# zixunh/vipe

Hardware: AMD Instinct MI355X
Metric: dense-BA+flow update iters/s, 512x384 48-KF graph (higher is better)
Workload: dtype f16 (correlation, GRU; fp32 accumulate) + f32 geometry/BA (fp64 reduced system)

## Files before the change

include/vipe_amd.h:

```cpp
#ifndef VIPE_AMD_H
#define VIPE_AMD_H

#include <stdint.h>

#ifdef __cplusplus
extern "C" {
#endif

#define VIPE_F16 0
#define VIPE_F32 1
#define VIPE_F64 2
#define VIPE_U8 3

#define VIPE_OK 0
#define VIPE_EINVAL (-1)
#define VIPE_ENOSPACE (-2)
#define VIPE_EUNSUPPORTED (-3)

#define VIPE_PYRAMID_REFERENCE 0
#define VIPE_PYRAMID_BLOCKED 1

#define VIPE_CAM_PINHOLE 0
#define VIPE_CAM_MEI 1
#define VIPE_CAM_PANORAMA 2

const char* vipe_amd_version(void);
int vipe_amd_abi_version(void);


int vipe_corr_index_forward(const void* d_volume, const float* d_coords, void* d_corr, int B, int h1, int w1,
                            int h2, int w2, int radius, int dtype, void* stream);

int vipe_corr_index_backward(const float* d_coords, const void* d_corr_grad, void* d_volume_grad, int B, int h1,
                             int w1, int h2, int w2, int radius, int dtype, void* stream);

int vipe_corr_pyramid_lookup(const void* const* h_levels, const float* d_coords, void* d_out, int B, int h1, int w1,
                             int h2, int w2, int num_levels, int radius, int dtype, void* stream);

int vipe_corr_pyramid_lookup_nhwc(const void* const* h_levels, const float* d_coords, void* d_out, int B, int h1,
                                  int w1, int h2, int w2, int num_levels, int radius, int dtype, int channel_stride,
                                  void* stream);

int vipe_corr_lookup_conv1x1(const void* const* h_levels, const float* d_coords, const void* d_w_packed,
                             const float* d_bias, void* d_out, int out_ctot, int out_coff, int B, int h1, int w1,
                             int h2, int w2, int Cout, int act, const int* d_slots, int layout, void* stream);

int vipe_corr_lookup_conv1x1_ex(const void* const* h_levels, const float* d_coords, const void* d_w_packed,
                                const float* d_bias, void* d_out, int out_ctot, int out_coff, int B, int h1, int w1,
                                int h2, int w2, int Cout, int act, const int* d_slots, int layout, void* stream,
                                int max_workgroups, int share_cu);

int vipe_corr_pyramid_build(const void* d_fmap1, const void* d_fmap2, void* const* h_levels, int B, int C, int h,
                            int w, int num_levels, void* stream);

int vipe_corr_pyramid_build_indexed(const void* d_fmaps, const int64_t* d_idx1, const int64_t* d_idx2,
                                    const int* d_slots, void* const* h_levels, int B, int C, int h, int w,
                                    int num_levels, int layout, void* stream);

int vipe_corr_blocked_dims(int h, int w, int* dims6);
int64_t vipe_corr_prep_halves(int C, int h, int w);
int vipe_corr_prep(const void* d_fmaps, void* d_prep, int n, int C, int h, int w, void* stream);
int vipe_corr_pyramid_build_prepared(const void* d_prep, int64_t frame_base, int64_t n_prepared, const int64_t* d_idx1, const int64_t* d_idx2,
                                     const int* d_slots, void* const* h_levels, int B, int C, int h, int w, int num_levels,
                                     void* stream);

int vipe_corr_volume(const void* d_fmap1, const void* d_fmap2, void* d_volume, int B, int C, int P, int dtype, void* stream);
int vipe_avg_pool2x2(const void* d_x, void* d_y, int64_t n, int h, int w, int dtype, void* stream);

int vipe_altcorr_forward(const void* d_fmap1, const void* d_fmap2, const float* d_coords, void* d_corr, int B,
                         int H1, int W1, int H2, int W2, int N, int C, int radius, int dtype, void* stream);

int vipe_altcorr_backward(const float* d_fmap1, const float* d_fmap2, const float* d_coords,
                          const float* d_corr_grad, float* d_fmap1_grad, float* d_fmap2_grad, int B, int H1, int W1,
                          int H2, int W2, int N, int C, int radius, void* stream);

int vipe_lie_expm(int group_id, const void* a, void* X, int64_t n, int dtype, int on_device, void* stream);
int vipe_lie_logm(int group_id, const void* X, void* a, int64_t n, int dtype, int on_device, void* stream);
int vipe_lie_inv(int group_id, const void* X, void* Y, int64_t n, int dtype, int on_device, void* stream);
int vipe_lie_mul(int group_id, const void* X, const void* Y, void* Z, int64_t n, int dtype, int on_device,
                 void* stream);
int vipe_lie_adj(int group_id, const void* X, const void* a, void* b, int64_t n, int dtype, int on_device,
                 void* stream);
int vipe_lie_adjT(int group_id, const void* X, const void* a, void* b, int64_t n, int dtype, int on_device,
                  void* stream);
int vipe_lie_act(int group_id, const void* X, const void* p, void* q, int64_t n, int dtype, int on_device,
                 void* stream);
int vipe_lie_act4(int group_id, const void* X, const void* p, void* q, int64_t n, int dtype, int on_device,
                  void* stream);
int vipe_lie_as_matrix(int group_id, const void* X, void* T, int64_t n, int dtype, int on_device,
                       void* stream);
int vipe_lie_projector(int group_id, const void* X, void* P, int64_t n, int dtype, int on_device,
                       void* stream);
int vipe_lie_jinv(int group_id, const void* X, const void* a, void* b, int64_t n, int dtype, int on_device,
                  void* stream);
int vipe_frontend_next_frame(float* d_poses, float* d_disps, int t1, int n_views, int P, int n_mean, int init_pose,
                             void* stream);
int vipe_lie_adjT_bcast(int group_id, const void* X, const void* a, void* b, int64_t n_elem, int64_t rows_per_elem,
                        int dtype, void* stream);
int vipe_lie_act4_bcast(int group_id, const void* X, const void* p, void* q, int64_t n_elem, int64_t rows_per_elem,
                        int dtype, void* stream);
int vipe_lie_expm_backward(int group_id, const void* grad, const void* a, void* da, int64_t n, int dtype,
                           int on_device, void* stream);
int vipe_lie_logm_backward(int group_id, const void* grad, const void* X, void* dX, int64_t n, int dtype,
                           int on_device, void* stream);
int vipe_lie_inv_backward(int group_id, const void* grad, const void* X, void* dX, int64_t n, int dtype,
                          int on_device, void* stream);
int vipe_lie_mul_backward(int group_id, const void* grad, const void* X, const void* Y, void* dX, void* dY,
                          int64_t n, int dtype, int on_device, void* stream);
int vipe_lie_adj_backward(int group_id, const void* grad, const void* X, const void* a, void* dX, void* da,
                          int64_t n, int dtype, int on_device, void* stream);
int vipe_lie_adjT_backward(int group_id, const void* grad, const void* X, const void* a, void* dX, void* da,
                           int64_t n, int dtype, int on_device, void* stream);
int vipe_lie_act_backward(int group_id, const void* grad, const void* X, const void* p, void* dX, void* dp,
                          int64_t n, int dtype, int on_device, void* stream);
int vipe_lie_act4_backward(int group_id, const void* grad, const void* X, const void* p, void* dX, void* dp,
                           int64_t n, int dtype, int on_device, void* stream);


int vipe_reproject(const float* d_poses, const float* d_disps, const float* d_intrinsics, const float* d_rig,
                   const int64_t* d_pi, const int64_t* d_qi, const int64_t* d_pj, const int64_t* d_qj,
                   const int64_t* d_di, float* d_coords, float* d_valid, int M, int ht, int wd, int n_views,
                   int camera, float intr_factor, void* stream);

int vipe_reproject_motion(const float* d_poses, const float* d_disps, const float* d_intrinsics, const float* d_rig,
                          const int64_t* d_pi, const int64_t* d_qi, const int64_t* d_pj, const int64_t* d_qj,
                          const int64_t* d_di, const float* d_target, float* d_coords, void* d_motn, int M, int ht,
                          int wd, int n_views, int camera, float intr_factor, int motn_dtype, void* stream);
int vipe_reproject_motion_nhwc(const float* d_poses, const float* d_disps, const float* d_intrinsics,
                               const float* d_rig, const int64_t* d_pi, const int64_t* d_qi, const int64_t* d_pj,
                               const int64_t* d_qj, const int64_t* d_di, const float* d_target, float* d_coords,
                               void* d_motn, int M, int ht, int wd, int n_views, int camera, float intr_factor,
                               void* stream);

typedef int (*vipe_overlap_fn)(void* user, int piece, int n_pieces, void* stream);

typedef struct {
  int n_poses;
  int n_views;
  int ht, wd;
  int M;
  int t0, t1;
  int n_iters;
  float pose_damping, pose_ep;
  int motion_only;
  int limited_disp;
  int optimize_intrinsics;
  int optimize_rig_rotation;
  int camera;
  float alpha;
  float weight_scale;
  float intr_factor;
  int reuse_plan;
  int path_hint;
  void* overlap_stream;
  vipe_overlap_fn overlap_fn;
  void* overlap_user;
  int solver_options;
  void* profile_ev0;
  void* profile_ev1;
  int profile_iter;
} vipe_ba_params;
#define VIPE_BA_OPT_ONE_CHAIN 1
#define VIPE_BA_OPT_GENERAL_ACCUMULATE 2

int64_t vipe_dense_ba_workspace_bytes(const vipe_ba_params* p);
int vipe_dense_ba(const vipe_ba_params* p, float* d_poses, float* d_disps, const float* d_disps_sens,
                  float* d_intrinsics, float* d_rig, const float* d_target, const float* d_weight,
                  const float* d_disp_damping, const int64_t* d_pi, const int64_t* d_qi, const int64_t* d_pj,
                  const int64_t* d_qj, const int64_t* d_di, void* d_workspace, int64_t workspace_bytes,
                  int* d_info, void* stream);

int vipe_dense_ba_linearize(const vipe_ba_params* p, const float* d_poses, const float* d_disps, const float* d_disps_sens,
                            const float* d_intrinsics, const float* d_rig, const float* d_target, const float* d_weight,
                            const float* d_disp_damping, const int64_t* d_pi, const int64_t* d_qi, const int64_t* d_pj,
                            const int64_t* d_qj, const int64_t* d_di, void* d_workspace, int64_t workspace_bytes,
                            double* d_S_out, int ld_out, int* d_info, void* stream);
int vipe_dense_ba_marginals(const vipe_ba_params* p, void* d_workspace, const double* d_Sinv, int ld, float* d_disp_var,
                            double* d_pose_cov, void* stream);

int64_t vipe_ba_workspace_bytes(int n_poses, int ht, int wd, int E);
int vipe_ba(float* d_poses, float* d_disps, const float* d_intrinsics, const float* d_disps_sens,
            const float* d_targets, const float* d_weights, const float* d_eta, const int64_t* d_ii,
            const int64_t* d_jj, int n_poses, int ht, int wd, int E, int n_eta, int t0, int t1, int iterations,
            float lm, float ep, int motion_only, float* d_dx, float* d_dz, void* d_workspace,
            int64_t workspace_bytes, void* stream);

int vipe_frame_distance(const float* d_poses, const float* d_disps, const float* d_intrinsics, const int64_t* d_pi,
                        const int64_t* d_pj, const int64_t* d_qi, const int64_t* d_qj, const int64_t* d_di,
                        float* d_dist, int M, int ht, int wd, float beta, void* stream);

int vipe_frame_distance_rig(const float* d_poses, const float* d_rig, const float* d_disps, const float* d_intrinsics,
                            int intr_dim, float intr_factor, const int64_t* d_pi, const int64_t* d_qi, const int64_t* d_pj,
                            const int64_t* d_qj, float* d_dist, int M, int n_views, int ht, int wd, float beta,
                            int bidirectional, void* stream);

int vipe_depth_filter(const float* d_poses, const float* d_disps, const float* d_intrinsics, const int64_t* d_inds,
                      const float* d_thresh, float* d_counter, int n, int num, int ht, int wd, void* stream);

int vipe_frame_distance_sphere(const float* d_poses, const float* d_rig, const float* d_disps, const int64_t* d_pi,
                               const int64_t* d_qi, const int64_t* d_pj, const int64_t* d_qj, float* d_dist, int M,
                               int n_views, int ht, int wd, float beta, int bidirectional, void* stream);
int vipe_depth_filter_sphere(const float* d_poses, const float* d_disps, const int64_t* d_inds, const float* d_thresh,
                             float* d_counter, int n, int num, int ht, int wd, void* stream);
int vipe_iproj_sphere(const float* d_poses, const float* d_disps, float* d_points, int n, int ht, int wd, void* stream);

int vipe_projmap(const float* d_poses, const float* d_disps, const float* d_intrinsics, const int64_t* d_ii,
                 const int64_t* d_jj, float* d_coords, float* d_valid, int E, int ht, int wd, void* stream);

int vipe_iproj(const float* d_poses, const float* d_disps, const float* d_intrinsics, float* d_points, int n, int ht,
               int wd, void* stream);

int vipe_scatter(const void* d_src, const int64_t* d_index, void* d_out, int64_t* d_arg_out, int64_t outer,
                 int64_t src_dim, int64_t inner, int64_t out_dim, int reduce, int dtype, void* stream);
int vipe_scatter_rows(const void* d_src, const int64_t* d_index, void* d_out, int64_t* d_arg_out, int64_t outer,
                      int64_t src_dim, int64_t inner, int64_t out_dim, int reduce, int dtype, void* stream);

int vipe_scatter_host(const void* h_src, const int64_t* h_index, void* h_out, int64_t* h_arg_out, int64_t outer,
                      int64_t src_dim, int64_t inner, int64_t out_dim, int reduce, int dtype);

int vipe_scatter_mean_rows_f16(const void* d_src, const int64_t* d_ix, void* d_out, int E, int n_out, int64_t inner,
                               void* stream);

int vipe_segment_mean_nhwc_f16(const void* d_src, int src_ctot, int src_coff, const int* d_order, const int* d_rowptr,
                               void* d_out, int n_out, int64_t rows_per_item, int C, void* stream);

int vipe_corr_sampler_forward(const void* d_in1, const void* d_in2, void* d_out, int B, int C, int H, int W, int kH,
                              int kW, int patchH, int patchW, int padH, int padW, int dilH, int dilW,
                              int dil_patchH, int dil_patchW, int dH, int dW, int dtype, void* stream);
int vipe_corr_sampler_backward(const void* d_in1, const void* d_in2, const void* d_grad_out, void* d_grad1,
                               void* d_grad2, int B, int C, int H, int W, int kH, int kW, int patchH, int patchW,
                               int padH, int padW, int dilH, int dilW, int dil_patchH, int dil_patchW, int dH,
                               int dW, int dtype, void* stream);

int vipe_corr_sampler_forward_host(const float* h_in1, const float* h_in2, float* h_out, int B, int C, int H, int W, int kH,
                                   int kW, int patchH, int patchW, int padH, int padW, int dilH, int dilW, int dil_patchH,
                                   int dil_patchW, int dH, int dW);
int vipe_corr_sampler_backward_host(const float* h_in1, const float* h_in2, const float* h_grad_out, float* h_grad1,
                                    float* h_grad2, int B, int C, int H, int W, int kH, int kW, int patchH, int patchW,
                                    int padH, int padW, int dilH, int dilW, int dil_patchH, int dil_patchW, int dH, int dW);

int vipe_nearest_neighbours(const float* d_query, int qdim, const float* d_tree, int tdim, int64_t M, int64_t N, int knn,
                            float* d_dist, int* d_idx, void* stream);

int vipe_ms_deform_attn_forward(const void* d_value, const int64_t* d_spatial_shapes, const int64_t* d_level_start_index,
                                const void* d_sampling_loc, const void* d_attn_weight, void* d_output, int64_t bs,
                                int64_t Lv, int heads, int C, int L, int64_t Lq, int P, int dtype, void* stream);
int vipe_ms_deform_attn_backward(const void* d_value, const int64_t* d_spatial_shapes, const int64_t* d_level_start_index,
                                 const void* d_sampling_loc, const void* d_attn_weight, const void* d_grad_output,
                                 void* d_grad_value, void* d_grad_sampling_loc, void* d_grad_attn_weight, int64_t bs,
                                 int64_t Lv, int heads, int C, int L, int64_t Lq, int P, int dtype, void* stream);

#define VIPE_ACT_NONE 0
#define VIPE_ACT_RELU 1
#define VIPE_ACT_SIGMOID 2
#define VIPE_ACT_TANH 3
int vipe_conv_pack_weights(const void* d_w_oihw, void* d_w_packed, int Cout, int Cin, int KH, int KW, int src_dtype,
                           void* stream);
int vipe_conv2d_nhwc_f16(const void* d_x, const void* d_w_packed, const float* d_bias, const float* d_extra,
                         void* d_y, int B, int H, int W, int Cin, int cin_total, int cin_off, int Cout,
                         int cout_total, int cout_off, int KH, int KW, int act, void* stream);

int vipe_conv_packed_dims(int Cout, int Cin, int KH, int KW, int* cout_pad, int* cin_pad, int* k_pad);

#define VIPE_CONV_PARTIAL 6
#define VIPE_CONV_HEADS_FUSED 7
#define VIPE_CONV_ACCINIT_F32 0x100
int vipe_conv2d_fused(const void* d_x0, int x0_ctot, int x0_coff, const void* d_x1, int x1_ctot, int x1_coff,
                      int split, const void* d_w_packed, const float* d_bias, const float* d_extra, int extra_stride,
                      int extra_off, void* d_y, int y_ctot, int y_coff, void* d_y2, int y2_ctot, int y2_coff,
                      const void* d_net, int net_ctot, int net_coff, const void* d_z, float* d_fout,
                      const void* d_accinit, int ai_ctot, int ai_coff, int B, int H, int W, int Cin, int Cout, int KH,
                      int KW, int act, int mode, void* stream);

int vipe_heads_fused_ok(int H, int W);
int vipe_heads_border_floats(int E, int H, int W, int64_t* n_floats);
int vipe_heads_finish(float* d_dw, const float* d_border, const float* d_bias, int E, int H, int W, void* stream);

typedef struct {
  const void *corr0_w, *corr2_w, *flow0_w, *flow2_w, *gw_w, *zr_w, *q_w, *zr_s_w, *q_s_w, *heads0_w, *heads2_w, *agg2_w, *eta_w;
  const void *zr_n_w, *zr_x_w;
  const float *corr0_b, *corr2_b, *flow0_b, *flow2_b, *gw_b, *zr_b, *q_b, *heads0_b, *heads2_b, *agg2_b, *eta_b;
  const float* glo_wT;
  const float* glo_b;
  const void *agg1_w, *heads_dw_w;
  const float *agg1_b, *heads_dw_b;
  const void* heads2_frag;
} vipe_update_weights;
typedef struct {
  int E, H, W, n_src;
  const void* levels[4];
  const float* coords;
  const int* slots;
  int h2, w2, pyramid_layout;
  const void* corr;
  const void* motn;
  const void* net;
  void* net_out;
  void* xbuf;
  const void* pgate;
  void *c1, *f1, *zb, *rnet;
  void* hbuf;
  float* dw;
  float *glo, *extra;
  const int *order, *rowptr;
  void *agg, *a2;
  float* eta;
  void* side_stream;
  float* pzr;
  int gate_state;
  float* hborder;
} vipe_update_buffers;
int vipe_update_operator(const vipe_update_weights* weights, const vipe_update_buffers* buffers, void* stream);

int vipe_update_gate_state(const vipe_update_weights* weights, const vipe_update_buffers* buffers, const void* d_net,
                           int parts, void* stream);
typedef struct {
  const vipe_update_weights* weights;
  const vipe_update_buffers* buffers;
  const void* net;
  const int* bounds;
  int n_bounds;
} vipe_gate_state_job;
int vipe_update_gate_state_piece(void* user, int piece, int n_pieces, void* stream);

int vipe_glo_context(const float* d_glo_sum, const float* d_wT, const float* d_bias, float* d_extra, int E, int hw,
                     void* stream);

typedef struct {
  const void* src;
  void* dst;
  const int64_t* idx;
  int64_t src_row_pitch, dst_row_pitch;
  int64_t seg_bytes, seg_pitch;
  int n_seg;
  int n_rows;
  int dst_row0;
} vipe_rows_job;
int vipe_rows_gather(const vipe_rows_job* jobs, int n_jobs, void* stream);
typedef struct {
  const void* src;
  const int64_t* frame;
  void* dst;
  int64_t dst_row_pitch;
  int dst_ctot, dst_coff;
  int dst_row0;
} vipe_nhwc_job;
int vipe_gather_nchw_to_nhwc_f16(const vipe_nhwc_job* jobs, int n_jobs, int n_rows, int C, int P, void* stream);

int vipe_flow_score(const float* d_dw, const unsigned char* d_invalid, float* d_score, int n_views, int P, void* stream);

int vipe_update_finish(const float* d_coords1, const float* d_dw, const unsigned char* d_mask, float* d_target,
                       float* d_weight, const float* d_eta, const int64_t* d_du, float* d_damping, int E, int n_src, int ht,
                       int wd, void* stream);

int vipe_enc_prep(const float* d_img, void* d_x4, int V, int H, int W, void* stream);
int vipe_enc_stem(const void* d_x4, const void* d_w, const float* d_bias, void* d_y, float* d_out_stats, int B, int H,
                  int W, int relu, void* stream);
int vipe_enc_conv(const void* d_x, const float* d_in_stats, const void* d_w, const float* d_bias, const void* d_res,
                  void* d_y, float* d_out_stats, int B, int H, int W, int Cin, int Cout, int ksize, int stride,
                  int relu, int nchw, int tanh_split, void* stream);
int vipe_enc_finish(const void* d_raw, const float* d_raw_stats, const void* d_res, const float* d_res_stats,
                    void* d_out, int B, int HW, int C, void* stream);

int vipe_frame_ingest(const void* d_rgb, int rgb_dtype, const unsigned char* d_mask, const float* d_depth, int H0, int W0,
                      int h1, int w1, int top, int left, int H, int W, float* d_images, void* d_x4,
                      unsigned char* d_mask8, float* d_disps_sens, void* stream);

int vipe_convex_upsample(const void* d_mask, int mask_dtype, const float* d_data, float* d_out, const int64_t* d_rows,
                         int N, int R, int h, int w, int C, void* stream);

int vipe_depth_export(const float* d_disp, const int64_t* d_rows, void* d_out, int out_dtype, int N, int R, int H, int W,
                      int h1, int w1, int top, int left, int H0, int W0, float depth_scale, void* stream);

int vipe_depth_consistency(const float* d_disp, const float* d_poses, const float* d_rig, const float* d_intrinsics,
                           int intr_dim, int camera, const int64_t* d_rows, const int64_t* d_nbr, unsigned char* d_out,
                           int N, int K, int R, int n_views, int H, int W, int h1, int w1, int top, int left, int H0,
                           int W0, float tol, void* stream);

int vipe_cloud_fuse(const float* d_disp, const float* d_poses, const float* d_rig, const float* d_intrinsics, int intr_dim,
                    int camera, const int64_t* d_rows, const unsigned char* d_conf, int min_agree, const void* d_rgb,
                    int rgb_dtype, int stride, float inv_voxel, int64_t* d_keys, int* d_acc, int64_t cap, int64_t* d_stats,
                    int N, int R, int n_views, int H, int W, int h1, int w1, int top, int left, int H0, int W0,
                    void* stream);

int vipe_cloud_extract(const int64_t* d_keys, const int* d_acc, int64_t cap, float voxel, int min_count, float* d_xyz,
                       unsigned char* d_rgb, int* d_count, int64_t* d_key, int64_t max_out, int64_t* d_num_out,
                       void* stream);

int vipe_cloud_render(const float* d_xyz, int64_t M, int index_base, const float* d_cams, const float* d_intrinsics,
                      int intr_dim, int camera, int B, int H, int W, int h1, int w1, int top, int left, int H0, int W0,
                      float point_size, int max_radius, int64_t* d_zbuf, int64_t* d_stats, void* stream);

int vipe_cloud_resolve(const int64_t* d_zbuf, int B, int H0, int W0, void* d_depth, int depth_dtype,
                       const unsigned char* d_rgb_points, int64_t M_total, unsigned char* d_rgb_out, int* d_index,
                       void* stream);

#define VIPE_COMPLETE_DISP 0
#define VIPE_COMPLETE_DEPTH 1

int vipe_depth_anchor_bits(const void* d_sparse, const void* d_pred, int dtype, int B, int H, int W, int64_t* d_bits,
                           void* stream);

int vipe_depth_complete(const void* d_sparse, const void* d_pred, int dtype, const unsigned char* d_mask,
                        const int64_t* d_bits, int B, int H, int W, int domain, int K, int radius, int wrap_x, void* d_out,
                        float* d_scale, float* d_shift, int* d_nbr, int64_t* d_stats, void* stream);

#define VIPE_KLT_OOB 1
#define VIPE_KLT_LOW_TEXTURE 2
#define VIPE_KLT_RESIDUAL 4
#define VIPE_KLT_FB 8
#define VIPE_KLT_MASKED 16
#define VIPE_KLT_DIVERGED 32

int vipe_klt_pyramid(const void* d_rgb, int rgb_dtype, int H, int W, int L, float* d_pyr, void* stream);

int vipe_klt_detect(const float* d_img, int H, int W, const unsigned char* d_mask, const unsigned char* d_cell_busy,
                    int cell, int border, float min_eig, float* d_out, void* stream);

int vipe_klt_track(const float* d_pyr_a, const float* d_pyr_b, int H, int W, int L, const float* d_pts, int N,
                   const float* d_fb_ref, const unsigned char* d_mask, int win_radius, int n_iters, float eps, int border,
                   float min_eig, float max_residual, float fb_thresh, float max_flow, int cell, float* d_out,
                   unsigned char* d_status, float* d_resid, unsigned char* d_cell_busy, void* stream);

#ifdef __cplusplus
}
#endif
#endif
```

vipe_amd/csrc/conv_call.cuh:

```cuda
#pragma once
#include <hip/hip_runtime_api.h>
#include <limits.h>

#include "../../include/vipe_amd.h"

enum Epi { EPI_PLAIN = 0, EPI_GLO = 1, EPI_ZR = 2, EPI_Q = 3, EPI_HEADS = 4, EPI_ETA = 5, EPI_PARTIAL = 6, EPI_HEADS_FUSED = 7 };

struct ConvView {
  const void* p = nullptr;
  int ctot = 0, coff = 0;
};

struct ConvCall {
  ConvView x0, x1;
  int split = INT_MAX;
  const void* w = nullptr;
  const float* bias = nullptr;
  const float* extra = nullptr;
  int extra_stride = 0, extra_off = 0;
  ConvView y;
  ConvView y2;
  ConvView net;
  ConvView accinit;
  bool accinit_f32 = false;
  const void* z = nullptr;
  float* fout = nullptr;
  const void* heads2_frag = nullptr;
  float* border = nullptr;
  int B = 0, H = 0, W = 0, Cin = 0, Cout = 0, KH = 1, KW = 1;
  int act = VIPE_ACT_NONE, epi = EPI_PLAIN;
};

int vipe_conv_run(const ConvCall& c, hipStream_t stream);
```

vipe_amd/csrc/conv_mfma.hip:

```cpp
#include <stdlib.h>

#include <type_traits>

#include "common.cuh"
#include "conv_call.cuh"

namespace {

typedef _Float16 half8 __attribute__((ext_vector_type(8)));
typedef _Float16 half4 __attribute__((ext_vector_type(4)));
typedef float float16v __attribute__((ext_vector_type(16)));
typedef float float4v __attribute__((ext_vector_type(4)));

struct ConvArgs {
  const half_t* x0; int x0_ctot, x0_coff;
  const half_t* x1; int x1_ctot, x1_coff;
  int split;
  const half_t* w;
  const float* bias;
  const float* extra;
  int extra_stride, extra_off;
  half_t* y; int y_ctot, y_coff;
  int B, H, W, Cin, Cin_pad, Cout, Cout_pad, KH, KW, nsteps;
  int act, epi;
  const half_t* net; int net_ctot, net_coff;
  const half_t* zbuf;
  half_t* y2; int y2_ctot, y2_coff;
  float* fout;
  const half_t* accinit; int ai_ctot, ai_coff;
  int ai_f32;
  const half_t* w2;
  float* border;
  int f_wp, f_hwp, f_tiles, f_pieces, f_xbytes, f_p1lo, f_p1hi;
  unsigned f_magic;
};

constexpr int BNP = 128;
constexpr int BK = 64;

__device__ __forceinline__ int swz(int row, int k8) { return row * 128 + ((k8 ^ ((row >> 1) & 7)) << 4); }

__device__ __forceinline__ float act_apply(float v, int act) {
  switch (act) {
    case VIPE_ACT_RELU: return fmaxf(v, 0.0f);
    case VIPE_ACT_SIGMOID: return 1.0f / (1.0f + __expf(-v));
    case VIPE_ACT_TANH: return tanhf(v);
    default: return v;
  }
}

template <int BMC, int WAVES_M, int WAVES_N, bool SMALLCIN>
__global__ __launch_bounds__(256) void conv_mfma_kernel(ConvArgs a) {
  constexpr int TM = BMC / (WAVES_M * 32);
  constexpr int TN = BNP / (WAVES_N * 32);
  static_assert(WAVES_M * WAVES_N == 4, "4 waves");
  constexpr int W_ITEMS = BMC * 8 / 256;
  constexpr int X_ITEMS = BNP * 8 / 256;

  extern __shared__ __align__(16) unsigned char lds[];
  unsigned char* ldsW = lds;
  unsigned char* ldsX = lds + 2 * BMC * 128;

  const int tid = threadIdx.x, lane = tid & 63, wave = tid >> 6;
  const int wm = wave / WAVES_N, wn = wave % WAVES_N;
  const int64_t M = (int64_t)a.B * a.H * a.W;
  const int64_t pix0 = (int64_t)blockIdx.x * BNP;
  const int cout0 = blockIdx.y * BMC;
  const int HW = a.H * a.W;

  const int k8 = tid & 7;
  int xe[X_ITEMS], xy[X_ITEMS], xx[X_ITEMS];
  bool xvalid[X_ITEMS];
#pragma unroll
  for (int j = 0; j < X_ITEMS; ++j) {
    const int64_t m = pix0 + (tid >> 3) + 32 * j;
    xvalid[j] = m < M;
    const int64_t mm = xvalid[j] ? m : 0;
    xe[j] = (int)(mm / HW);
    const int rem = (int)(mm % HW);
    xy[j] = rem / a.W;
    xx[j] = rem % a.W;
  }
  const int ph = a.KH / 2, pw = a.KW / 2;
  const int csteps = a.Cin_pad / BK;

  half8 wreg[W_ITEMS], xreg[X_ITEMS];

  auto issue_loads = [&](int s) {
    const half_t* wb = a.w + ((int64_t)s * a.Cout_pad + cout0) * BK;
#pragma unroll
    for (int j = 0; j < W_ITEMS; ++j) {
      const int row = (tid >> 3) + 32 * j;
      wreg[j] = *reinterpret_cast<const half8*>(wb + row * BK + k8 * 8);
    }
    if constexpr (!SMALLCIN) {
      const int tap = s / csteps, c0 = (s % csteps) * BK;
      const int dy = tap / a.KW - ph, dx = tap % a.KW - pw;
      const int c = c0 + k8 * 8;
      const bool cok = c < a.Cin;
      const bool s0 = c < a.split;
      const half_t* src = s0 ? a.x0 : a.x1;
      const int ctot = s0 ? a.x0_ctot : a.x1_ctot;
      const int coff = s0 ? a.x0_coff + c : a.x1_coff + (c - a.split);
#pragma unroll
      for (int j = 0; j < X_ITEMS; ++j) {
        const int yy = xy[j] + dy, xc = xx[j] + dx;
        const bool ok = cok & xvalid[j] & (yy >= 0) & (yy < a.H) & (xc >= 0) & (xc < a.W);
        half8 v = {0, 0, 0, 0, 0, 0, 0, 0};
        if (ok) v = *reinterpret_cast<const half8*>(src + ((int64_t)(xe[j] * a.H + yy) * a.W + xc) * ctot + coff);
        xreg[j] = v;
      }
    } else {
      const int q = s * 8 + k8;
#pragma unroll
      for (int j = 0; j < X_ITEMS; ++j) {
        half4 lo = {0, 0, 0, 0}, hi = {0, 0, 0, 0};
#pragma unroll
        for (int h = 0; h < 2; ++h) {
          const int tap = 2 * q + h;
          if (tap < a.KH * a.KW) {
            const int yy = xy[j] + tap / a.KW - ph, xc = xx[j] + tap % a.KW - pw;
            if (xvalid[j] & (yy >= 0) & (yy < a.H) & (xc >= 0) & (xc < a.W)) {
              const half4 v = *reinterpret_cast<const half4*>(
                  a.x0 + ((int64_t)(xe[j] * a.H + yy) * a.W + xc) * a.x0_ctot + a.x0_coff);
              if (h == 0) lo = v; else hi = v;
            }
          }
        }
        xreg[j] = half8{lo[0], lo[1], lo[2], lo[3], hi[0], hi[1], hi[2], hi[3]};
      }
    }
  };
  auto write_lds = [&](int buf) {
#pragma unroll
    for (int j = 0; j < W_ITEMS; ++j) {
      const int row = (tid >> 3) + 32 * j;
      *reinterpret_cast<half8*>(ldsW + buf * BMC * 128 + swz(row, k8)) = wreg[j];
    }
#pragma unroll
    for (int j = 0; j < X_ITEMS; ++j) {
      const int row = (tid >> 3) + 32 * j;
      *reinterpret_cast<half8*>(ldsX + buf * BNP * 128 + swz(row, k8)) = xreg[j];
    }
  };

  float16v acc[TM][TN];
#pragma unroll
  for (int i = 0; i < TM; ++i)
#pragma unroll
    for (int j = 0; j < TN; ++j)
#pragma unroll
      for (int r = 0; r < 16; ++r) acc[i][j][r] = 0.0f;

  issue_loads(0);
  write_lds(0);
  __syncthreads();
  const int lrow = lane & 31, lhalf = lane >> 5;
  for (int s = 0; s < a.nsteps; ++s) {
    const int cur = s & 1;
    if (s + 1 < a.nsteps) issue_loads(s + 1);
    const unsigned char* bw = ldsW + cur * BMC * 128;
    const unsigned char* bx = ldsX + cur * BNP * 128;
#pragma unroll
    for (int kk = 0; kk < BK / 16; ++kk) {
      half8 wf[TM], xf[TN];
#pragma unroll
      for (int i = 0; i < TM; ++i)
        wf[i] = *reinterpret_cast<const half8*>(bw + swz((wm * TM + i) * 32 + lrow, kk * 2 + lhalf));
#pragma unroll
      for (int j = 0; j < TN; ++j)
        xf[j] = *reinterpret_cast<const half8*>(bx + swz((wn * TN + j) * 32 + lrow, kk * 2 + lhalf));
#pragma unroll
      for (int i = 0; i < TM; ++i)
#pragma unroll
        for (int j = 0; j < TN; ++j)
          acc[i][j] = __builtin_amdgcn_mfma_f32_32x32x16_f16(wf[i], xf[j], acc[i][j], 0, 0, 0);
    }
    if (s + 1 < a.nsteps) write_lds(cur ^ 1);
    __syncthreads();
  }

#include "conv_epilogue.inc"
}

__device__ __attribute__((aligned(16))) unsigned char g_zero_page[64];

__device__ __forceinline__ void glds16(const void* g, unsigned lds_addr) {
#if defined(__HIP_DEVICE_COMPILE__)
  unsigned keep;
  const unsigned base = __builtin_amdgcn_readfirstlane(lds_addr);
  asm volatile(
      "s_mov_b32 %0, m0\n\ts_mov_b32 m0, %2\n\ts_nop 0\n\tglobal_load_lds_dwordx4 %1, off\n\ts_mov_b32 m0, %0"
      : "=&s"(keep)
      : "v"(g), "s"(base)
      : "memory");
#endif
}

__device__ __forceinline__ unsigned lds_address(const void* p) {
  return (unsigned)(uintptr_t)(__attribute__((address_space(3))) const unsigned char*)p;
}

template <int BMC, int WAVES_M, int WAVES_N>
__global__ __launch_bounds__(256) void conv_mfma_glds_kernel(ConvArgs a, int gy) {
  constexpr int TM = BMC / (WAVES_M * 32);
  constexpr int TN = BNP / (WAVES_N * 32);
  static_assert(WAVES_M * WAVES_N == 4, "4 waves");
  constexpr int WP = BMC / 32;
  constexpr int XP = BNP / 32;

  extern __shared__ __align__(16) unsigned char lds[];
  unsigned char* ldsW = lds;
  unsigned char* ldsX = lds + 2 * BMC * 128;

  const int tid = threadIdx.x, lane = tid & 63, wave = __builtin_amdgcn_readfirstlane(tid >> 6);
  const int wm = wave / WAVES_N, wn = wave % WAVES_N;
  const int nb = gridDim.x;
  const int L = xcd_remap(blockIdx.x, nb);
  const int64_t M = (int64_t)a.B * a.H * a.W;
  const int64_t pix0 = (int64_t)(L / gy) * BNP;
  const int cout0 = (L % gy) * BMC;
  const int HW = a.H * a.W;
  const int ph = a.KH / 2, pw = a.KW / 2;
  const int csteps = a.Cin_pad / BK;
  const int r8 = lane >> 3, sl = lane & 7;

  int woff[WP];
#pragma unroll
  for (int q = 0; q < WP; ++q) {
    const int row = (wave * WP + q) * 8 + r8;
    woff[q] = row * BK + ((sl ^ ((row >> 1) & 7)) << 3);
  }
  const half_t* xb0[XP];
  const half_t* xb1[XP];
  int xk8[XP], py[XP], px[XP];
  unsigned xmask[XP];
#pragma unroll
  for (int q = 0; q < XP; ++q) {
    const int row = (wave * XP + q) * 8 + r8;
    const int64_t m = pix0 + row;
    const bool ok = m < M;
    const int64_t mm = ok ? m : 0;
    const int rem = (int)(mm % HW);
    py[q] = ok ? rem / a.W : -100000;
    px[q] = rem % a.W;
    const int k8 = sl ^ ((row >> 1) & 7);
    xk8[q] = k8 * 8;
    xb0[q] = a.x0 + mm * a.x0_ctot + a.x0_coff + k8 * 8;
    xb1[q] = a.x1 + mm * a.x1_ctot + a.x1_coff + k8 * 8 - a.split;
    xmask[q] = 0;
  }
  for (int t = 0; t < a.KH * a.KW; ++t) {
    const int dy = t / a.KW - ph, dx = t % a.KW - pw;
#pragma unroll
    for (int q = 0; q < XP; ++q) {
      const int yy = py[q] + dy, xc = px[q] + dx;
      if (yy >= 0 && yy < a.H && xc >= 0 && xc < a.W) xmask[q] |= 1u << t;
    }
  }
  const half_t* zp = reinterpret_cast<const half_t*>(g_zero_page);

  auto issue = [&](int s, int buf) {
    const half_t* wb = a.w + ((int64_t)s * a.Cout_pad + cout0) * BK;
    unsigned char* lw = ldsW + buf * BMC * 128 + wave * WP * 1024;
#pragma unroll
    for (int q = 0; q < WP; ++q)
      glds16(wb + woff[q], lds_address(lw) + q * 1024);
    const int tap = s / csteps, c0 = (s % csteps) * BK;
    const int dy = tap / a.KW - ph, dx = tap % a.KW - pw;
    const bool s0 = c0 < a.split;
    const int64_t delta = (int64_t)(dy * a.W + dx) * (s0 ? a.x0_ctot : a.x1_ctot) + c0;
    const int crem = a.Cin - c0;
    unsigned char* lx = ldsX + buf * BNP * 128 + wave * XP * 1024;
#pragma unroll
    for (int q = 0; q < XP; ++q) {
      const bool ok = ((xmask[q] >> tap) & 1u) && (xk8[q] < crem);
      const half_t* p = (s0 ? xb0[q] : xb1[q]) + delta;
      glds16(ok ? p : zp, lds_address(lx) + q * 1024);
    }
  };

  float16v acc[TM][TN];
#pragma unroll
  for (int i = 0; i < TM; ++i)
#pragma unroll
    for (int j = 0; j < TN; ++j)
#pragma unroll
      for (int r = 0; r < 16; ++r) acc[i][j][r] = 0.0f;

  issue(0, 0);
  asm volatile("s_waitcnt vmcnt(0)" ::: "memory");
  __syncthreads();
  const int lrow = lane & 31, lhalf = lane >> 5;
  for (int s = 0; s < a.nsteps; ++s) {
    const int cur = s & 1;
    const unsigned char* bw = ldsW + cur * BMC * 128;
    const unsigned char* bx = ldsX + cur * BNP * 128;
    half8 wf[BK / 16][TM], xf[BK / 16][TN];
#pragma unroll
    for (int kk = 0; kk < BK / 16; ++kk) {
#pragma unroll
      for (int i = 0; i < TM; ++i)
        wf[kk][i] = *reinterpret_cast<const half8*>(bw + swz((wm * TM + i) * 32 + lrow, kk * 2 + lhalf));
#pragma unroll
      for (int j = 0; j < TN; ++j)
        xf[kk][j] = *reinterpret_cast<const half8*>(bx + swz((wn * TN + j) * 32 + lrow, kk * 2 + lhalf));
    }
    __builtin_amdgcn_sched_barrier(0);
    if (s + 1 < a.nsteps) issue(s + 1, cur ^ 1);
    __builtin_amdgcn_sched_barrier(0);
#pragma unroll
    for (int kk = 0; kk < BK / 16; ++kk)
#pragma unroll
      for (int i = 0; i < TM; ++i)
#pragma unroll
        for (int j = 0; j < TN; ++j)
          acc[i][j] = __builtin_amdgcn_mfma_f32_32x32x16_f16(wf[kk][i], xf[kk][j], acc[i][j], 0, 0, 0);
    asm volatile("s_waitcnt vmcnt(0)" ::: "memory");
    __syncthreads();
  }
#include "conv_epilogue.inc"
}

constexpr int HALO_TH = 4, HALO_TW = 64;
constexpr int HALO_PITCH = HALO_TW + 2;
constexpr int HALO_ROWS = (HALO_TH + 2) * HALO_PITCH;

__device__ __forceinline__ void glds16_off(const void* base, unsigned voff_bytes, unsigned lds_addr) {
#if defined(__HIP_DEVICE_COMPILE__)
  unsigned keep;
  const unsigned lb = __builtin_amdgcn_readfirstlane(lds_addr);
  const uint64_t bu = (uint64_t)base;
  const uint64_t bs = ((uint64_t)(unsigned)__builtin_amdgcn_readfirstlane((int)(bu >> 32)) << 32) |
                      (unsigned)__builtin_amdgcn_readfirstlane((int)bu);
  asm volatile(
      "s_mov_b32 %0, m0\n\ts_mov_b32 m0, %3\n\ts_nop 0\n\tglobal_load_lds_dwordx4 %1, %2\n\ts_mov_b32 m0, %0"
      : "=&s"(keep)
      : "v"(voff_bytes), "s"(bs), "s"(lb)
      : "memory");
#endif
}

__device__ __forceinline__ uint64_t uniform64(uint64_t v) {
  return ((uint64_t)(unsigned)__builtin_amdgcn_readfirstlane((int)(v >> 32)) << 32) | (unsigned)__builtin_amdgcn_readfirstlane((int)v);
}
__device__ __forceinline__ void dma16s(uint64_t sbase, unsigned voff_bytes, unsigned lds_addr) {
#if defined(__HIP_DEVICE_COMPILE__)
  unsigned keep;
  asm volatile("s_mov_b32 %0, m0\n\ts_mov_b32 m0, %3\n\ts_nop 0\n\tglobal_load_lds_dwordx4 %1, %2\n\ts_mov_b32 m0, %0"
               : "=&s"(keep)
               : "v"(voff_bytes), "s"(sbase), "s"(lds_addr)
               : "memory");
#endif
}
__device__ __forceinline__ void dma16v(uint64_t lane_ptr, unsigned lds_addr) {
#if defined(__HIP_DEVICE_COMPILE__)
  unsigned keep;
  asm volatile("s_mov_b32 %0, m0\n\ts_mov_b32 m0, %2\n\ts_nop 0\n\tglobal_load_lds_dwordx4 %1, off\n\ts_mov_b32 m0, %0"
               : "=&s"(keep)
               : "v"(lane_ptr), "s"(lds_addr)
               : "memory");
#endif
}

constexpr int H32_PIECES = (HALO_ROWS + 15) / 16;
constexpr int H32_XBYTES = H32_PIECES * 1024;
constexpr int H32_XP = (H32_PIECES + 7) / 8;
constexpr int H32_BK = 32;

__device__ __forceinline__ int swzf(int row) { return ((row >> 2) & 1) << 1; }
__device__ __forceinline__ int swz32(int row, int c) { return row * 64 + ((c ^ swzf(row)) << 4); }


__device__ __forceinline__ int flat_pixel(int q, int e, int H, int W, int wp, int hwp, unsigned magic) {
  if ((unsigned)q >= (unsigned)hwp) return -1;
  const int y = (int)__umulhi((unsigned)q, magic);
  const int x = q - y * wp;
  return x < W ? (e * H + y) * W + x : -1;
}

constexpr int HB_N = 2 * (HALO_TW + 2) + 2 * HALO_TH;
constexpr int HG_PITCH = HALO_TH * HALO_TW + 4;
__host__ __device__ __forceinline__ int hb_index(int py, int px) {
  return py < 0 ? px + 1 : py >= HALO_TH ? (HALO_TW + 2) + px + 1 : px < 0 ? 2 * (HALO_TW + 2) + py : 2 * (HALO_TW + 2) + HALO_TH + py;
}

template <int BMC, int KS, bool M16, int VAR = 0, bool FLAT = false>
__global__ __launch_bounds__(512) __attribute__((amdgpu_waves_per_eu(4, 4))) void conv_halo32_kernel(ConvArgs a, int gy) {
  static_assert(M16, "only the 16x16x32 form exists");
  constexpr int MI = BMC >= 128 ? 4 : 2, NJ = BMC == 32 ? 2 : 4;
  constexpr int BP = HALO_TH * HALO_TW;
  constexpr int WSTAGE = BMC * 64;
  extern __shared__ __align__(16) unsigned char lds[];

  const int tid = threadIdx.x, lane = tid & 63, wave = __builtin_amdgcn_readfirstlane(tid >> 6);
  const int wm = BMC == 32 ? 0 : (wave >> 2), wn = wave & 3;
  const int pxh = BMC == 32 ? (wave >> 2) * 32 : 0;
  const int L = xcd_remap(blockIdx.x, gridDim.x);
  const int tile = L / gy, cout0 = (L % gy) * BMC;
  const int xsegs = a.W / HALO_TW, tiles_per_img = FLAT ? a.f_tiles : (a.H / HALO_TH) * xsegs;
  const int e = tile / tiles_per_img, trem = tile % tiles_per_img;
  const int y0 = (trem / xsegs) * HALO_TH, x0 = (trem % xsegs) * HALO_TW;
  const int q0 = trem * BP;
  const int pitch = FLAT ? a.f_wp : HALO_PITCH;
  const int xbytes = FLAT ? a.f_xbytes : H32_XBYTES;
  const int npieces = FLAT ? a.f_pieces : H32_PIECES;
  auto pix_of = [&](int pl) -> int64_t {
    if constexpr (FLAT) return flat_pixel(q0 + pl, e, a.H, a.W, a.f_wp, a.f_hwp, a.f_magic);
    else return ((int64_t)(e * a.H + y0 + (pl >> 6))) * a.W + x0 + (pl & 63);
  };
  const int cs32 = a.Cin_pad / H32_BK, cs64 = a.Cin_pad / 64;
  const int r16 = lane >> 2, sl = lane & 3;

  const unsigned ldsW_a = lds_address(lds), ldsX_a = ldsW_a + 3 * WSTAGE;
  const unsigned sink_a = ldsX_a + 2 * xbytes;
  const unsigned char* ldsW = lds;
  const unsigned char* ldsX = lds + 3 * WSTAGE;
  const half_t* zp = reinterpret_cast<const half_t*>(g_zero_page);

  constexpr int WPIECES = BMC / 16;
  const bool wreal = wave < WPIECES;
  const int wrow = (wave % WPIECES) * 16 + r16;
  const unsigned woff = (unsigned)(wrow * 64 + ((sl ^ swzf(wrow)) << 3)) * 2u;
  const unsigned wdst = ldsW_a + (wave % WPIECES) * 1024;
  int xpix[FLAT ? 1 : H32_XP];
  const int xk = (sl ^ swzf(r16)) * 8;
  if constexpr (!FLAT) {
#pragma unroll
    for (int i = 0; i < H32_XP; ++i) {
      const int pce = wave + 8 * i;
      const int r = pce * 16 + r16;
      const int hy = r / HALO_PITCH, hx = r % HALO_PITCH;
      const int y = y0 + hy - 1, x = x0 + hx - 1;
      const bool ok = pce < H32_PIECES && r < HALO_ROWS && y >= 0 && y < a.H && x >= 0 && x < a.W;
      xpix[i] = ok ? (e * a.H + y) * a.W + x : -1;
    }
  }
  auto piece_used = [&](int i) {
    const int pce = wave + 8 * i;
    if constexpr (FLAT) return pce < npieces && (KS == 3 || (pce >= a.f_p1lo && pce <= a.f_p1hi));
    else return pce < H32_PIECES && (KS == 3 || (pce >= 4 && pce <= 20));
  };
  auto issueX = [&](int c, int i, int buf) {
    const int c0 = c * H32_BK;
    const bool s0 = c0 < a.split;
    const int ctot = s0 ? a.x0_ctot : a.x1_ctot;
    const int cb = (s0 ? a.x0_coff : a.x1_coff - a.split) + c0;
    int xp;
    if constexpr (FLAT) xp = flat_pixel(q0 - pitch - 1 + (wave + 8 * i) * 16 + r16, e, a.H, a.W, a.f_wp, a.f_hwp, a.f_magic);
    else xp = xpix[i];
    const bool ok = xp >= 0 && (c0 + xk < a.Cin);
    const uint64_t off = ((uint64_t)(unsigned)xp * (unsigned)ctot + (unsigned)(cb + xk)) * 2u;
    const char* src = reinterpret_cast<const char*>(s0 ? a.x0 : a.x1) + off;
    glds16(ok ? (const void*)src : (const void*)zp, ldsX_a + buf * xbytes + (wave + 8 * i) * 1024);
  };
  auto wsrc = [&](int tap, int c) {
    return a.w + ((int64_t)(tap * cs64 + (c >> 1)) * a.Cout_pad + cout0) * BK + (c & 1) * H32_BK;
  };
  auto issueW = [&](const half_t* wb, int slot) {
    if (wreal) glds16_off(wb, woff, wdst + slot * WSTAGE);
    else glds16(zp, sink_a);
  };
  const uint64_t zp64 = uniform64((uint64_t)zp);
  const uint64_t wbase = uniform64((uint64_t)(a.w + (int64_t)cout0 * BK));
  const unsigned tstride = (unsigned)cs64 * (unsigned)a.Cout_pad * BK * 2u;
  const unsigned sink_u = __builtin_amdgcn_readfirstlane(sink_a), wdst_u = __builtin_amdgcn_readfirstlane(wdst);
  const unsigned ldsX_u = __builtin_amdgcn_readfirstlane(ldsX_a + wave * 1024);
  auto issueW2 = [&](int tap, int c, int slot, bool more_) {
    const unsigned off = (unsigned)tap * tstride + ((unsigned)(c >> 1) * (unsigned)a.Cout_pad * BK + (unsigned)(c & 1) * H32_BK) * 2u;
    const bool on = more_ && wreal;
    dma16s(on ? wbase + off : zp64, on ? woff : 0u, on ? wdst_u + slot * WSTAGE : sink_u);
  };
  auto issueX2 = [&](int c, int i, int buf, bool on) {
    const int c0 = c * H32_BK;
    const bool s0 = c0 < a.split;
    const int ctot = s0 ? a.x0_ctot : a.x1_ctot;
    const int cb = (s0 ? a.x0_coff : a.x1_coff - a.split) + c0;
    int xp;
    if constexpr (FLAT) xp = flat_pixel(q0 - pitch - 1 + (wave + 8 * i) * 16 + r16, e, a.H, a.W, a.f_wp, a.f_hwp, a.f_magic);
    else xp = xpix[i];
    const bool ok = on && xp >= 0 && (c0 + xk < a.Cin);
    const uint64_t off = ((uint64_t)(unsigned)xp * (unsigned)ctot + (unsigned)(cb + xk)) * 2u;
    const uint64_t base = (uint64_t)(s0 ? a.x0 : a.x1);
    dma16v(ok ? base + off : zp64, on ? ldsX_u + buf * xbytes + i * 8192 : sink_u);
  };

  float4v acc16[MI][NJ];
#pragma unroll
  for (int i = 0; i < MI; ++i)
#pragma unroll
    for (int j = 0; j < NJ; ++j) acc16[i][j] = float4v{0.0f, 0.0f, 0.0f, 0.0f};
  if constexpr (BMC >= 64) {
    if (a.accinit) {
#pragma unroll
      for (int j = 0; j < NJ; ++j) {
        const int64_t m = pix_of(wn * 64 + j * 16 + (lane & 15));
        if (FLAT && m < 0) continue;
#pragma unroll
        for (int i = 0; i < MI; ++i) {
          const int cg = cout0 + wm * (MI * 16) + i * 16 + 4 * (lane >> 4);
          if constexpr (VAR == 1) {
            const float4 v = *reinterpret_cast<const float4*>(reinterpret_cast<const float*>(a.accinit) + m * a.ai_ctot +
                                                              a.ai_coff + cg);
            acc16[i][j] = float4v{v.x, v.y, v.z, v.w};
          } else {
            const half4 v = *reinterpret_cast<const half4*>(a.accinit + m * a.ai_ctot + a.ai_coff + cg);
            acc16[i][j] = float4v{(float)v[0], (float)v[1], (float)v[2], (float)v[3]};
          }
        }
      }
    }
  }

  const int l16 = lane & 15, lk = lane >> 4;
  const int wa0 = swz32(wm * MI * 16 + l16, lk);
  const int Rl0 = (FLAT ? wn * HALO_TW : wn * HALO_PITCH) + pxh + l16;
  auto mma_step = [&](const unsigned char* bw, const unsigned char* bx, int Rl, int dy, int dx) {
    const int rb = Rl + (dy + 1) * pitch + (dx + 1);
    const int xa0 = swz32(rb, lk);
    half8 wf[MI];
#pragma unroll
    for (int i = 0; i < MI; ++i) wf[i] = *reinterpret_cast<const half8*>(bw + (wa0 + i * 1024));
#pragma unroll
    for (int j = 0; j < NJ; ++j) {
      const half8 xf = *reinterpret_cast<const half8*>(bx + (xa0 + j * 1024));
#pragma unroll
      for (int i = 0; i < MI; ++i)
        acc16[i][j] = __builtin_amdgcn_mfma_f32_16x16x32_f16(wf[i], xf, acc16[i][j], 0, 0, 0);
    }
  };

  auto load_frags = [&](const unsigned char* bw, const unsigned char* bx, int Rl, int dy, int dx, half8 (&wf)[MI], half8 (&xf)[NJ]) {
    const int xa0 = swz32(Rl + (dy + 1) * pitch + (dx + 1), lk);
#pragma unroll
    for (int i = 0; i < MI; ++i) wf[i] = *reinterpret_cast<const half8*>(bw + (wa0 + i * 1024));
#pragma unroll
    for (int j = 0; j < NJ; ++j) xf[j] = *reinterpret_cast<const half8*>(bx + (xa0 + j * 1024));
  };
  auto mma_frags = [&](const half8 (&wf)[MI], const half8 (&xf)[NJ]) {
#pragma unroll
    for (int j = 0; j < NJ; ++j)
#pragma unroll
      for (int i = 0; i < MI; ++i) acc16[i][j] = __builtin_amdgcn_mfma_f32_16x16x32_f16(wf[i], xf[j], acc16[i][j], 0, 0, 0);
  };

#pragma unroll
  for (int i = 0; i < H32_XP; ++i)
    if (piece_used(i)) issueX(0, i, 0);
  issueW(wsrc(0, 0), 0);
  if constexpr (KS == 3) issueW(wsrc(1, 0), 1);
  asm volatile("s_waitcnt vmcnt(0)" ::: "memory");
  __syncthreads();

  if constexpr (KS == 3) {
    for (int c = 0; c < cs32; ++c) {
      const unsigned char* bx = ldsX + (c & 1) * xbytes;
      const bool more = c + 1 < cs32;
      int Rl = Rl0;
      asm volatile("" : "+v"(Rl));
      auto tap_step = [&](auto TAPC) {
        constexpr int TAP = decltype(TAPC)::value;
        constexpr int T2 = TAP + 2;
        half8 wf[MI], xf[NJ];
        load_frags(ldsW + (TAP % 3) * WSTAGE, bx, Rl, TAP / 3 - 1, TAP % 3 - 1, wf, xf);
        if constexpr (T2 < 9) issueW2(T2, c, T2 % 3, true);
        else issueW2(T2 - 9, c + 1, T2 % 3, more);
        if constexpr (TAP < H32_XP) issueX2(c + 1, TAP, (c + 1) & 1, more && piece_used(TAP));
        mma_frags(wf, xf);
        if constexpr (TAP == 0 || TAP == 4) asm volatile("s_waitcnt vmcnt(2)" ::: "memory");
        else if constexpr (TAP < 4) asm volatile("s_waitcnt vmcnt(3)" ::: "memory");
        else asm volatile("s_waitcnt vmcnt(1)" ::: "memory");
        __syncthreads();
      };
      tap_step(std::integral_constant<int, 0>{});
      tap_step(std::integral_constant<int, 1>{});
      tap_step(std::integral_constant<int, 2>{});
      tap_step(std::integral_constant<int, 3>{});
      tap_step(std::integral_constant<int, 4>{});
      tap_step(std::integral_constant<int, 5>{});
      tap_step(std::integral_constant<int, 6>{});
      tap_step(std::integral_constant<int, 7>{});
      tap_step(std::integral_constant<int, 8>{});
    }
  } else {
    for (int c = 0; c < cs32; ++c) {
      const unsigned char* bx = ldsX + (c & 1) * xbytes;
      if (c + 1 < cs32) {
        issueW(wsrc(0, c + 1), (c + 1) & 1);
#pragma unroll
        for (int i = 0; i < H32_XP; ++i)
          if (piece_used(i)) issueX(c + 1, i, (c + 1) & 1);
      }
      mma_step(ldsW + (c & 1) * WSTAGE, bx, Rl0, 0, 0);
      asm volatile("s_waitcnt vmcnt(0)" ::: "memory");
      __syncthreads();
    }
  }
  asm volatile("s_waitcnt vmcnt(0)" ::: "memory");
  __syncthreads();

  constexpr int CPP = BMC / 8;
  constexpr int NIT = BP * CPP / 512, PSTEP = 512 / CPP;
  const int ch = (tid % CPP) * 8, co = cout0 + ch, pl0 = tid / CPP;
  if constexpr (BMC >= 64) {
    if constexpr (VAR == 2) {
      {
#pragma unroll
        for (int j = 0; j < NJ; ++j) {
          const int64_t m = pix_of(wn * 64 + j * 16 + l16);
          if (FLAT && m < 0) continue;
#pragma unroll
          for (int i = 0; i < MI; ++i) {
            const int cg = cout0 + wm * (MI * 16) + i * 16 + 4 * lk;
            if (cg + 4 <= a.Cout)
              *reinterpret_cast<float4*>(a.fout + m * a.y_ctot + a.y_coff + cg) =
                  make_float4(acc16[i][j][0], acc16[i][j][1], acc16[i][j][2], acc16[i][j][3]);
          }
        }
        return;
      }
    }
    if constexpr (VAR == 3) {
      static_assert(BMC == 128 && KS == 3 && !FLAT, "the fused heads exist for the aligned 128-cout 3x3 tile only");
      const int slice = cout0 >> 7;
      float* G = reinterpret_cast<float*>(lds);
      float4 bq[MI];
#pragma unroll
      for (int i = 0; i < MI; ++i) bq[i] = *reinterpret_cast<const float4*>(a.bias + cout0 + wm * 64 + i * 16 + 4 * lk);
      const half8* af = reinterpret_cast<const half8*>(a.w2) + (slice * 2 + wm) * 4 * 64 + lane;
      half8 afr[2][2];
#pragma unroll
      for (int q = 0; q < 4; ++q) afr[q >> 1][q & 1] = af[q * 64];
#pragma unroll
      for (int j = 0; j < NJ; ++j) {
        half8 hb[2];
#pragma unroll
        for (int i = 0; i < MI; ++i) {
          hb[i >> 1][(i & 1) * 4 + 0] = (half_t)fmaxf(acc16[i][j][0] + bq[i].x, 0.0f);
          hb[i >> 1][(i & 1) * 4 + 1] = (half_t)fmaxf(acc16[i][j][1] + bq[i].y, 0.0f);
          hb[i >> 1][(i & 1) * 4 + 2] = (half_t)fmaxf(acc16[i][j][2] + bq[i].z, 0.0f);
          hb[i >> 1][(i & 1) * 4 + 3] = (half_t)fmaxf(acc16[i][j][3] + bq[i].w, 0.0f);
        }
        float4v g0 = float4v{0.0f, 0.0f, 0.0f, 0.0f}, g1 = g0;
        g0 = __builtin_amdgcn_mfma_f32_16x16x32_f16(afr[0][0], hb[0], g0, 0, 0, 0);
        g0 = __builtin_amdgcn_mfma_f32_16x16x32_f16(afr[0][1], hb[1], g0, 0, 0, 0);
        g1 = __builtin_amdgcn_mfma_f32_16x16x32_f16(afr[1][0], hb[0], g1, 0, 0, 0);
        g1 = __builtin_amdgcn_mfma_f32_16x16x32_f16(afr[1][1], hb[1], g1, 0, 0, 0);
        const int p = wn * 64 + j * 16 + l16;
#pragma unroll
        for (int r = 0; r < 4; ++r) G[(wm * 18 + 4 * lk + r) * HG_PITCH + p] = g0[r];
        if (lk == 0) {
          G[(wm * 18 + 16) * HG_PITCH + p] = g1[0];
          G[(wm * 18 + 17) * HG_PITCH + p] = g1[1];
        }
      }
      __syncthreads();
      for (int idx = tid; idx < 6 * 66 * 2; idx += 512) {
        const int o = idx & 1, pos = idx >> 1, py = pos / 66 - 1, px = pos % 66 - 1;
        const int yy = y0 + py, xx = x0 + px;
        if (yy < 0 || yy >= a.H || xx < 0 || xx >= a.W) continue;
        float sum = 0.0f;
#pragma unroll
        for (int tap = 0; tap < 9; ++tap) {
          const int sy = py + tap / 3 - 1, sx = px + tap % 3 - 1;
          if ((unsigned)sy < (unsigned)HALO_TH && (unsigned)sx < (unsigned)HALO_TW) {
            const float* gp = G + (tap * 2 + o) * HG_PITCH + sy * HALO_TW + sx;
            sum += gp[0] + gp[18 * HG_PITCH];
          }
        }
        if ((unsigned)py < (unsigned)HALO_TH && (unsigned)px < (unsigned)HALO_TW)
          a.fout[((int64_t)(e * a.H + yy) * a.W + xx) * 4 + slice * 2 + o] = sum;
        else
          a.border[((int64_t)tile * HB_N + hb_index(py, px)) * 4 + slice * 2 + o] = sum;
      }
      return;
    }
    constexpr int PITCH = BMC + 8;
    half_t* stage = reinterpret_cast<half_t*>(lds);
    auto stage_all = [&](auto ACTC) {
      constexpr int ACT = decltype(ACTC)::value;
      auto put = [&](int cl, int pl, float4 b, float v0, float v1, float v2, float v3) {
        half4 h;
        h[0] = (half_t)act_apply(v0 + b.x, ACT);
        h[1] = (half_t)act_apply(v1 + b.y, ACT);
        h[2] = (half_t)act_apply(v2 + b.z, ACT);
        h[3] = (half_t)act_apply(v3 + b.w, ACT);
        *reinterpret_cast<half4*>(stage + pl * PITCH + cl) = h;
      };
      auto bias4 = [&](int cl) {
        const int cg = cout0 + cl;
        float4 b = *reinterpret_cast<const float4*>(a.bias + cg);
        if (a.extra && cg + 4 <= a.Cout) {
          const float4 x = *reinterpret_cast<const float4*>(a.extra + (int64_t)e * a.extra_stride + a.extra_off + cg);
          b.x += x.x; b.y += x.y; b.z += x.z; b.w += x.w;
        }
        return b;
      };
#pragma unroll
      for (int i = 0; i < MI; ++i) {
        const int cl = wm * (MI * 16) + i * 16 + 4 * lk;
        const float4 b = bias4(cl);
#pragma unroll
        for (int j = 0; j < NJ; ++j)
          put(cl, wn * 64 + j * 16 + l16, b, acc16[i][j][0], acc16[i][j][1], acc16[i][j][2], acc16[i][j][3]);
      }
    };
    const int actsel = a.epi == EPI_PLAIN ? a.act : (a.epi == EPI_Q ? VIPE_ACT_TANH : VIPE_ACT_SIGMOID);
    if (actsel == VIPE_ACT_RELU) stage_all(std::integral_constant<int, VIPE_ACT_RELU>{});
    else if (actsel == VIPE_ACT_SIGMOID) stage_all(std::integral_constant<int, VIPE_ACT_SIGMOID>{});
    else if (actsel == VIPE_ACT_TANH) stage_all(std::integral_constant<int, VIPE_ACT_TANH>{});
    else stage_all(std::integral_constant<int, VIPE_ACT_NONE>{});
    const bool want_net = a.epi == EPI_GLO || a.epi == EPI_Q || (a.epi == EPI_ZR && co >= 128);
    const bool want_z = a.epi == EPI_Q;
    half8 nvv[NIT], zvv[NIT];
    {
      const int cn = a.epi == EPI_ZR ? co - 128 : co;
#pragma unroll
      for (int it = 0; it < NIT; ++it) {
        const int64_t m = pix_of(pl0 + PSTEP * it);
        if (FLAT && m < 0) continue;
        if (want_net) nvv[it] = *reinterpret_cast<const half8*>(a.net + m * a.net_ctot + a.net_coff + cn);
        if (want_z) zvv[it] = *reinterpret_cast<const half8*>(a.zbuf + m * 128 + co);
      }
    }
    __syncthreads();
    float gsum[8] = {0, 0, 0, 0, 0, 0, 0, 0};
#pragma unroll
    for (int it = 0; it < NIT; ++it) {
      const int pl = pl0 + PSTEP * it;
      const int64_t m = pix_of(pl);
      if (FLAT && m < 0) continue;
      const half8 sv = *reinterpret_cast<const half8*>(stage + pl * PITCH + ch);
      half8 o = sv;
      half_t* dst = nullptr;
      if (a.epi == EPI_PLAIN) {
        dst = a.y + m * a.y_ctot + a.y_coff + co;
      } else if (a.epi == EPI_GLO) {
#pragma unroll
        for (int q = 0; q < 8; ++q) gsum[q] += (float)sv[q] * (float)nvv[it][q];
      } else if (a.epi == EPI_ZR) {
        if (co < 128) {
          dst = a.y + m * a.y_ctot + a.y_coff + co;
        } else {
#pragma unroll
          for (int q = 0; q < 8; ++q) o[q] = (half_t)((float)sv[q] * (float)nvv[it][q]);
          dst = a.y2 + m * a.y2_ctot + a.y2_coff + co - 128;
        }
      } else if (a.epi == EPI_Q) {
#pragma unroll
        for (int q = 0; q < 8; ++q) {
          const float z = (float)zvv[it][q];
          o[q] = (half_t)((1.0f - z) * (float)nvv[it][q] + z * (float)sv[q]);
        }
        dst = a.y + m * a.y_ctot + a.y_coff + co;
      }
      if (dst) {
        if (co + 8 <= a.Cout) {
          *reinterpret_cast<half8*>(dst) = o;
        } else {
          for (int q = 0; q < 8 && co + q < a.Cout; ++q) dst[q] = o[q];
        }
      }
    }
    if (a.epi == EPI_GLO) {
      float* red = reinterpret_cast<float*>(lds);
      __syncthreads();
#pragma unroll
      for (int q = 0; q < 8; ++q) red[(tid / CPP) * (BMC + 1) + ch + q] = gsum[q];
      __syncthreads();
      if (tid < BMC) {
        float t = 0.0f;
        for (int r = 0; r < 512 / CPP; ++r) t += red[r * (BMC + 1) + tid];
        if (cout0 + tid < a.Cout) atomicAdd(a.fout + (int64_t)e * a.Cout + cout0 + tid, t);
      }
    }
  } else {
    constexpr int PITCH = BMC + 4;
    float* stage = reinterpret_cast<float*>(lds);
#pragma unroll
    for (int i = 0; i < MI; ++i)
#pragma unroll
      for (int j = 0; j < NJ; ++j)
        *reinterpret_cast<float4*>(stage + (wn * 64 + pxh + j * 16 + l16) * PITCH + i * 16 + 4 * lk) =
            make_float4(acc16[i][j][0], acc16[i][j][1], acc16[i][j][2], acc16[i][j][3]);
    __syncthreads();
    float bv[8];
#pragma unroll
    for (int q = 0; q < 8; ++q) {
      bv[q] = a.bias[co + q];
      if (a.extra && co + q < a.Cout) bv[q] += a.extra[(int64_t)e * a.extra_stride + a.extra_off + co + q];
    }
#pragma unroll
    for (int it = 0; it < NIT; ++it) {
      const int pl = pl0 + PSTEP * it;
      const int64_t m = pix_of(pl);
      if (FLAT && m < 0) continue;
      const float4 v0 = *reinterpret_cast<const float4*>(stage + pl * PITCH + ch);
      const float4 v1 = *reinterpret_cast<const float4*>(stage + pl * PITCH + ch + 4);
      const float v[8] = {v0.x + bv[0], v0.y + bv[1], v0.z + bv[2], v0.w + bv[3],
                          v1.x + bv[4], v1.y + bv[5], v1.z + bv[6], v1.w + bv[7]};
      if (a.epi == EPI_HEADS) {
        if (ch == 0)
          *reinterpret_cast<float4*>(a.fout + m * 4) =
              make_float4((float)(half_t)v[0], (float)(half_t)v[1], (float)(half_t)act_apply(v[2], VIPE_ACT_SIGMOID),
                          (float)(half_t)act_apply(v[3], VIPE_ACT_SIGMOID));
      } else if (a.epi == EPI_ETA) {
        if (ch == 0) {
          const float sp = v[0] > 20.0f ? v[0] : log1pf(__expf(v[0]));
          a.fout[m] = 0.01f * (float)(half_t)sp;
        }
      } else {
        half_t* dst = a.y + m * a.y_ctot + a.y_coff + co;
        half8 o;
#pragma unroll
        for (int q = 0; q < 8; ++q) o[q] = (half_t)act_apply(v[q], a.act);
        if (co + 8 <= a.Cout) {
          *reinterpret_cast<half8*>(dst) = o;
        } else {
          for (int q = 0; q < 8 && co + q < a.Cout; ++q) dst[q] = o[q];
        }
      }
    }
  }
}

constexpr int NRW_WBYTES = 9 * 1024;

template <bool FLAT>
__global__ __launch_bounds__(512) __attribute__((amdgpu_waves_per_eu(4, 4))) void conv_halo32_narrow_kernel(ConvArgs a) {
  extern __shared__ __align__(16) unsigned char lds[];
  const int tid = threadIdx.x, lane = tid & 63, wave = __builtin_amdgcn_readfirstlane(tid >> 6);
  const int wn = wave & 3, pxh = (wave >> 2) * 32;
  const int tile = xcd_remap(blockIdx.x, gridDim.x);
  const int xsegs = a.W / HALO_TW, tiles_per_img = FLAT ? a.f_tiles : (a.H / HALO_TH) * xsegs;
  const int e = tile / tiles_per_img, trem = tile % tiles_per_img;
  const int y0 = (trem / xsegs) * HALO_TH, x0 = (trem % xsegs) * HALO_TW;
  const int q0 = trem * (HALO_TH * HALO_TW);
  const int pitch = FLAT ? a.f_wp : HALO_PITCH, xbytes = FLAT ? a.f_xbytes : H32_XBYTES;
  const int npieces = FLAT ? a.f_pieces : H32_PIECES;
  auto pix_of = [&](int pl) -> int64_t {
    if constexpr (FLAT) return flat_pixel(q0 + pl, e, a.H, a.W, a.f_wp, a.f_hwp, a.f_magic);
    else return ((int64_t)(e * a.H + y0 + (pl >> 6))) * a.W + x0 + (pl & 63);
  };
  const int cs32 = a.Cin_pad / H32_BK, cs64 = a.Cin_pad / 64;
  const int r16 = lane >> 2, sl = lane & 3, l16 = lane & 15, lk = lane >> 4;
  const unsigned ldsW_a = lds_address(lds), ldsX_a = ldsW_a + 2 * NRW_WBYTES;
  const unsigned char* ldsW = lds;
  const unsigned char* ldsX = lds + 2 * NRW_WBYTES;
  const half_t* zp = reinterpret_cast<const half_t*>(g_zero_page);

  int xpix[H32_XP];
  const int xk = (sl ^ swzf(r16)) * 8;
#pragma unroll
  for (int i = 0; i < H32_XP; ++i) {
    const int pce = wave + 8 * i;
    const int r = pce * 16 + r16;
    if constexpr (FLAT) {
      xpix[i] = pce < npieces ? flat_pixel(q0 - pitch - 1 + r, e, a.H, a.W, a.f_wp, a.f_hwp, a.f_magic) : -1;
    } else {
      const int hy = r / HALO_PITCH, hx = r % HALO_PITCH;
      const int y = y0 + hy - 1, x = x0 + hx - 1;
      const bool ok = pce < H32_PIECES && r < HALO_ROWS && y >= 0 && y < a.H && x >= 0 && x < a.W;
      xpix[i] = ok ? (e * a.H + y) * a.W + x : -1;
    }
  }
  auto issue = [&](int c, int buf) {
    const int c0 = c * H32_BK;
    const bool s0 = c0 < a.split;
    const int ctot = s0 ? a.x0_ctot : a.x1_ctot;
    const int cb = (s0 ? a.x0_coff : a.x1_coff - a.split) + c0;
#pragma unroll
    for (int i = 0; i < H32_XP; ++i) {
      if (wave + 8 * i < npieces) {
        const bool ok = xpix[i] >= 0 && (c0 + xk < a.Cin);
        const uint64_t off = ((uint64_t)(unsigned)xpix[i] * (unsigned)ctot + (unsigned)(cb + xk)) * 2u;
        const char* src = reinterpret_cast<const char*>(s0 ? a.x0 : a.x1) + off;
        glds16(ok ? (const void*)src : (const void*)zp, ldsX_a + buf * xbytes + (wave + 8 * i) * 1024);
      }
    }
    const unsigned woff = (unsigned)(r16 * 64 + ((sl ^ swzf(r16)) << 3)) * 2u;
    const half_t* wb = a.w + ((int64_t)(wave * cs64 + (c >> 1)) * a.Cout_pad) * BK + (c & 1) * H32_BK;
    glds16_off(wb, woff, ldsW_a + buf * NRW_WBYTES + wave * 1024);
    if (wave == 0) {
      const half_t* w8 = a.w + ((int64_t)(8 * cs64 + (c >> 1)) * a.Cout_pad) * BK + (c & 1) * H32_BK;
      glds16_off(w8, woff, ldsW_a + buf * NRW_WBYTES + 8 * 1024);
    }
  };

  float4v acc[2] = {float4v{0.f, 0.f, 0.f, 0.f}, float4v{0.f, 0.f, 0.f, 0.f}};
  const int wa0 = swz32(l16, lk);
  const int Rl0 = (FLAT ? wn * HALO_TW : wn * HALO_PITCH) + pxh + l16;
  issue(0, 0);
  asm volatile("s_waitcnt vmcnt(0)" ::: "memory");
  __syncthreads();
  for (int c = 0; c < cs32; ++c) {
    if (c + 1 < cs32) issue(c + 1, (c + 1) & 1);
    const unsigned char* bw = ldsW + (c & 1) * NRW_WBYTES;
    const unsigned char* bx = ldsX + (c & 1) * xbytes;
#pragma unroll
    for (int tap = 0; tap < 9; ++tap) {
      const int rb = Rl0 + (tap / 3) * pitch + (tap % 3);
      const int xa0 = swz32(rb, lk);
      const half8 wf = *reinterpret_cast<const half8*>(bw + (wa0 + tap * 1024));
#pragma unroll
      for (int j = 0; j < 2; ++j) {
        const half8 xf = *reinterpret_cast<const half8*>(bx + (xa0 + j * 1024));
        acc[j] = __builtin_amdgcn_mfma_f32_16x16x32_f16(wf, xf, acc[j], 0, 0, 0);
      }
    }
    asm volatile("s_waitcnt vmcnt(0)" ::: "memory");
    __syncthreads();
  }
  constexpr int PITCH = 20;
  float* stage = reinterpret_cast<float*>(lds);
#pragma unroll
  for (int j = 0; j < 2; ++j)
    *reinterpret_cast<float4*>(stage + (wn * 64 + pxh + j * 16 + l16) * PITCH + 4 * lk) =
        make_float4(acc[j][0], acc[j][1], acc[j][2], acc[j][3]);
  __syncthreads();
  const int64_t m = tid < HALO_TH * HALO_TW ? pix_of(tid) : -1;
  if (tid < HALO_TH * HALO_TW && (!FLAT || m >= 0)) {
    float v[16];
#pragma unroll
    for (int q = 0; q < 4; ++q) {
      const float4 t4 = *reinterpret_cast<const float4*>(stage + tid * PITCH + 4 * q);
      v[4 * q] = t4.x; v[4 * q + 1] = t4.y; v[4 * q + 2] = t4.z; v[4 * q + 3] = t4.w;
    }
#pragma unroll
    for (int q = 0; q < 16; ++q) {
      v[q] += a.bias[q];
      if (a.extra && q < a.Cout) v[q] += a.extra[(int64_t)e * a.extra_stride + a.extra_off + q];
    }
    if (a.epi == EPI_HEADS) {
      *reinterpret_cast<float4*>(a.fout + m * 4) =
          make_float4((float)(half_t)v[0], (float)(half_t)v[1], (float)(half_t)act_apply(v[2], VIPE_ACT_SIGMOID),
                      (float)(half_t)act_apply(v[3], VIPE_ACT_SIGMOID));
    } else if (a.epi == EPI_ETA) {
      const float sp = v[0] > 20.0f ? v[0] : log1pf(__expf(v[0]));
      a.fout[m] = 0.01f * (float)(half_t)sp;
    } else {
      half_t* dst = a.y + m * a.y_ctot + a.y_coff;
      for (int q = 0; q < a.Cout; ++q) dst[q] = (half_t)act_apply(v[q], a.act);
    }
  }
}

constexpr int GLO_PITCH = 136;
constexpr size_t GLO_LDS = 256 * GLO_PITCH * 2 + 128 * 4;

__global__ __launch_bounds__(512) __attribute__((amdgpu_waves_per_eu(4, 4))) void conv1x1_glo_kernel(ConvArgs a) {
  extern __shared__ __align__(16) unsigned char lds[];
  half_t* xt = reinterpret_cast<half_t*>(lds);
  float* gacc = reinterpret_cast<float*>(lds + 256 * GLO_PITCH * 2);
  const int tid = threadIdx.x, lane = tid & 63, wave = tid >> 6;
  const int l16 = lane & 15, kg = lane >> 4;
  const int wq = wave & 3, wp = wave >> 2;
  const int HW = a.H * a.W;
  const int tpi = (HW + 255) / 256;
  const int e = blockIdx.x / tpi, p0 = (blockIdx.x % tpi) * 256;
  const int64_t pix0 = (int64_t)e * HW + p0;
  if (tid < 128) gacc[tid] = 0.0f;
#pragma unroll
  for (int it = 0; it < 8; ++it) {
    const int i = tid + 512 * it, px = i >> 4, ck = i & 15;
    half8 v = {0, 0, 0, 0, 0, 0, 0, 0};
    if (p0 + px < HW) v = *reinterpret_cast<const half8*>(a.x0 + (pix0 + px) * a.x0_ctot + a.x0_coff + ck * 8);
    *reinterpret_cast<half8*>(xt + px * GLO_PITCH + ck * 8) = v;
  }
  half8 af[2][4];
#pragma unroll
  for (int i = 0; i < 2; ++i)
#pragma unroll
    for (int s2 = 0; s2 < 4; ++s2) {
      const int k = 32 * s2 + 8 * kg, r = 32 * wq + 16 * i + l16;
      af[i][s2] = *reinterpret_cast<const half8*>(a.w + ((int64_t)(k >> 6) * a.Cout_pad + r) * 64 + (k & 63));
    }
  float4 bv[2];
#pragma unroll
  for (int i = 0; i < 2; ++i) bv[i] = *reinterpret_cast<const float4*>(a.bias + 32 * wq + 16 * i + 4 * kg);
  __syncthreads();
  float gs[2][4] = {{0, 0, 0, 0}, {0, 0, 0, 0}};
#pragma unroll 2
  for (int j = 0; j < 8; ++j) {
    const int pxb = wp * 128 + j * 16 + l16;
    float4v acc[2] = {float4v{0.f, 0.f, 0.f, 0.f}, float4v{0.f, 0.f, 0.f, 0.f}};
#pragma unroll
    for (int s2 = 0; s2 < 4; ++s2) {
      const half8 xf = *reinterpret_cast<const half8*>(xt + pxb * GLO_PITCH + 32 * s2 + 8 * kg);
#pragma unroll
      for (int i = 0; i < 2; ++i) acc[i] = __builtin_amdgcn_mfma_f32_16x16x32_f16(af[i][s2], xf, acc[i], 0, 0, 0);
    }
#pragma unroll
    for (int i = 0; i < 2; ++i) {
      const half4 nv = *reinterpret_cast<const half4*>(xt + pxb * GLO_PITCH + 32 * wq + 16 * i + 4 * kg);
      const float b4[4] = {bv[i].x, bv[i].y, bv[i].z, bv[i].w};
#pragma unroll
      for (int r = 0; r < 4; ++r)
        gs[i][r] += (float)(half_t)act_apply(acc[i][r] + b4[r], VIPE_ACT_SIGMOID) * (float)nv[r];
    }
  }
#pragma unroll
  for (int i = 0; i < 2; ++i)
#pragma unroll
    for (int r = 0; r < 4; ++r) {
      float v = gs[i][r];
      v += __builtin_bit_cast(float, __builtin_amdgcn_update_dpp(0, __builtin_bit_cast(int, v), 0xB1, 0xf, 0xf, true));
      v += __builtin_bit_cast(float, __builtin_amdgcn_update_dpp(0, __builtin_bit_cast(int, v), 0x4E, 0xf, 0xf, true));
      v += __builtin_bit_cast(float, __builtin_amdgcn_update_dpp(0, __builtin_bit_cast(int, v), 0x141, 0xf, 0xf, true));
      v += __builtin_bit_cast(float, __builtin_amdgcn_update_dpp(0, __builtin_bit_cast(int, v), 0x140, 0xf, 0xf, true));
      if (l16 == 0) atomicAdd(&gacc[32 * wq + 16 * i + 4 * kg + r], v);
    }
  __syncthreads();
  if (tid < a.Cout) atomicAdd(a.fout + (int64_t)e * a.Cout + tid, gacc[tid]);
}

constexpr int C7_PW = HALO_TW + 6, C7_ROWS = HALO_TH + 6;
constexpr int C7_WBYTES = 4 * 128 * 128;
constexpr int C7_XBYTES = ((C7_PW * C7_ROWS * 8 + 15) / 16) * 16;
constexpr int C7_LDS = (C7_WBYTES + C7_XBYTES) > (256 * 136 * 2) ? (C7_WBYTES + C7_XBYTES) : (256 * 136 * 2);

template <bool FLAT>
__global__ __launch_bounds__(512) __attribute__((amdgpu_waves_per_eu(4, 4))) void conv7x7_c4_kernel(ConvArgs a, int gy) {
  extern __shared__ __align__(16) unsigned char lds[];
  const int tid = threadIdx.x, lane = tid & 63, wave = __builtin_amdgcn_readfirstlane(tid >> 6);
  const int wm = wave >> 2, wn = wave & 3;
  const int L = xcd_remap(blockIdx.x, gridDim.x);
  const int tile = L / gy, cout0 = (L % gy) * 128;
  const int xsegs = a.W / HALO_TW, tiles_per_img = FLAT ? a.f_tiles : (a.H / HALO_TH) * xsegs;
  const int e = tile / tiles_per_img, trem = tile % tiles_per_img;
  const int y0 = (trem / xsegs) * HALO_TH, x0 = (trem % xsegs) * HALO_TW;
  const int q0 = trem * (HALO_TH * HALO_TW), pitch = FLAT ? a.f_wp : C7_PW;
  auto pix_of = [&](int pl) -> int64_t {
    if constexpr (FLAT) return flat_pixel(q0 + pl, e, a.H, a.W, a.f_wp, a.f_hwp, a.f_magic);
    else return ((int64_t)(e * a.H + y0 + (pl >> 6))) * a.W + x0 + (pl & 63);
  };
  const int l16 = lane & 15, lk = lane >> 4;
  const unsigned ldsW_a = lds_address(lds);
  unsigned char* ldsX = lds + C7_WBYTES;

  {
    const int r8 = lane >> 3, sl = lane & 7;
#pragma unroll
    for (int q = 0; q < 8; ++q) {
      const int pce = wave * 8 + q;
      const int blk = pce >> 4, row = (pce & 15) * 8 + r8;
      const half_t* src = a.w + ((int64_t)blk * a.Cout_pad + cout0 + row) * 64 + ((sl ^ ((row >> 1) & 7)) << 3);
      glds16(src, ldsW_a + pce * 1024);
    }
  }
  if constexpr (FLAT) {
    const int nh = HALO_TH * HALO_TW + 6 * pitch + 6;
    for (int i = tid; i < nh; i += 512) {
      const int m = flat_pixel(q0 - 3 * pitch - 3 + i, e, a.H, a.W, a.f_wp, a.f_hwp, a.f_magic);
      uint2 v = make_uint2(0u, 0u);
      if (m >= 0) v = *reinterpret_cast<const uint2*>(a.x0 + (int64_t)m * a.x0_ctot + a.x0_coff);
      *reinterpret_cast<uint2*>(ldsX + i * 8) = v;
    }
  } else {
    for (int i = tid; i < C7_PW * C7_ROWS; i += 512) {
      const int hy = i / C7_PW, hx = i % C7_PW;
      const int y = y0 + hy - 3, x = x0 + hx - 3;
      uint2 v = make_uint2(0u, 0u);
      if (y >= 0 && y < a.H && x >= 0 && x < a.W)
        v = *reinterpret_cast<const uint2*>(a.x0 + ((int64_t)(e * a.H + y) * a.W + x) * a.x0_ctot + a.x0_coff);
      *reinterpret_cast<uint2*>(ldsX + i * 8) = v;
    }
  }
  asm volatile("s_waitcnt vmcnt(0)" ::: "memory");
  __syncthreads();

  float4v acc[4][4];
#pragma unroll
  for (int i = 0; i < 4; ++i)
#pragma unroll
    for (int j = 0; j < 4; ++j) acc[i][j] = float4v{0.0f, 0.0f, 0.0f, 0.0f};
#pragma unroll
  for (int st = 0; st < 7; ++st) {
    half8 wf[4];
#pragma unroll
    for (int i = 0; i < 4; ++i)
      wf[i] = *reinterpret_cast<const half8*>(lds + (st >> 1) * 16384 + swz(wm * 64 + i * 16 + l16, (st & 1) * 4 + lk));
    const int t0 = min(st * 8 + lk * 2, 48), t1 = min(st * 8 + lk * 2 + 1, 48);
    const int wrow = FLAT ? wn * HALO_TW : wn * C7_PW;
    const int o0 = (wrow + (t0 / 7) * pitch + l16 + t0 % 7) * 8, o1 = (wrow + (t1 / 7) * pitch + l16 + t1 % 7) * 8;
#pragma unroll
    for (int j = 0; j < 4; ++j) {
      const half4 lo = *reinterpret_cast<const half4*>(ldsX + o0 + j * 128);
      const half4 hi = *reinterpret_cast<const half4*>(ldsX + o1 + j * 128);
      const half8 xf = {lo[0], lo[1], lo[2], lo[3], hi[0], hi[1], hi[2], hi[3]};
#pragma unroll
      for (int i = 0; i < 4; ++i) acc[i][j] = __builtin_amdgcn_mfma_f32_16x16x32_f16(wf[i], xf, acc[i][j], 0, 0, 0);
    }
  }
  __syncthreads();
  constexpr int PITCH = 136;
  half_t* stage = reinterpret_cast<half_t*>(lds);
#pragma unroll
  for (int i = 0; i < 4; ++i) {
    const int cl = wm * 64 + i * 16 + 4 * lk;
    const float4 b = *reinterpret_cast<const float4*>(a.bias + cout0 + cl);
#pragma unroll
    for (int j = 0; j < 4; ++j) {
      half4 h;
      h[0] = (half_t)act_apply(acc[i][j][0] + b.x, a.act);
      h[1] = (half_t)act_apply(acc[i][j][1] + b.y, a.act);
      h[2] = (half_t)act_apply(acc[i][j][2] + b.z, a.act);
      h[3] = (half_t)act_apply(acc[i][j][3] + b.w, a.act);
      *reinterpret_cast<half4*>(stage + (wn * 64 + j * 16 + l16) * PITCH + cl) = h;
    }
  }
  __syncthreads();
  const int ch = (tid & 15) * 8, co = cout0 + ch;
#pragma unroll
  for (int it = 0; it < 8; ++it) {
    const int pl = (tid >> 4) + 32 * it;
    const int64_t m = pix_of(pl);
    if (FLAT && m < 0) continue;
    const half8 o = *reinterpret_cast<const half8*>(stage + pl * PITCH + ch);
    half_t* dst = a.y + m * a.y_ctot + a.y_coff + co;
    if (co + 8 <= a.Cout) {
      *reinterpret_cast<half8*>(dst) = o;
    } else {
      for (int q = 0; q < 8 && co + q < a.Cout; ++q) dst[q] = o[q];
    }
  }
}

__global__ void pack_weights_kernel(const void* __restrict__ src, half_t* __restrict__ dst, int Cout, int Cin, int KH,
                                    int KW, int Cout_pad, int Cin_pad, int K_pad, int src_f32, int smallcin) {
  const int64_t total = (int64_t)K_pad * Cout_pad;
  for (int64_t i = (int64_t)blockIdx.x * blockDim.x + threadIdx.x; i < total; i += (int64_t)gridDim.x * blockDim.x) {
    const int kin = (int)(i % 64);
    const int co = (int)((i / 64) % Cout_pad);
    const int s = (int)(i / (64 * (int64_t)Cout_pad));
    const int k = s * 64 + kin;
    int tap, c;
    if (smallcin) { tap = k / 4; c = k % 4; }
    else { tap = k / Cin_pad; c = k % Cin_pad; }
    float v = 0.0f;
    if (co < Cout && c < Cin && tap < KH * KW) {
      const int64_t o = (((int64_t)co * Cin + c) * KH + tap / KW) * KW + tap % KW;
      v = src_f32 ? reinterpret_cast<const float*>(src)[o] : (float)reinterpret_cast<const half_t*>(src)[o];
    }
    dst[i] = (half_t)v;
  }
}

inline int round_up(int x, int m) { return (x + m - 1) / m * m; }

}


extern "C" {

VIPE_EXPORT int vipe_conv_packed_dims(int Cout, int Cin, int KH, int KW, int* cout_pad, int* cin_pad, int* k_pad) {
  if (Cout <= 0 || Cin <= 0 || KH <= 0 || KW <= 0) return VIPE_EINVAL;
  const int cp = Cout <= 32 ? 32 : (Cout <= 64 ? 64 : round_up(Cout, 128));
  int cinp, kp;
  if (Cin == 4) { cinp = 4; kp = round_up(KH * KW * 4, 64); }
  else { cinp = round_up(Cin, 64); kp = KH * KW * cinp; }
  if (cout_pad) *cout_pad = cp;
  if (cin_pad) *cin_pad = cinp;
  if (k_pad) *k_pad = kp;
  return VIPE_OK;
}

VIPE_EXPORT int vipe_conv_pack_weights(const void* d_w_oihw, void* d_w_packed, int Cout, int Cin, int KH, int KW,
                                       int src_dtype, void* stream) {
  VIPE_CHECK_ARG(d_w_oihw && d_w_packed);
  VIPE_CHECK_ARG(src_dtype == VIPE_F16 || src_dtype == VIPE_F32);
  int cp, cinp, kp;
  if (vipe_conv_packed_dims(Cout, Cin, KH, KW, &cp, &cinp, &kp) != VIPE_OK) return VIPE_EINVAL;
  VIPE_CHECK_ARG(Cin == 4 || Cin % 8 == 0);
  const int64_t total = (int64_t)kp * cp;
  pack_weights_kernel<<<(int)std::min<int64_t>((total + 255) / 256, 4096), 256, 0, as_stream(stream)>>>(
      d_w_oihw, (half_t*)d_w_packed, Cout, Cin, KH, KW, cp, cinp, kp, src_dtype == VIPE_F32, Cin == 4);
  return vipe_launch_status();
}

}

namespace {

__global__ __launch_bounds__(256) void heads_finish_kernel(float* __restrict__ dw, const float* __restrict__ border,
                                                           const float* __restrict__ bias, int64_t M, int H, int W) {
  const int64_t m = (int64_t)blockIdx.x * 256 + threadIdx.x;
  if (m >= M) return;
  const int x = (int)(m % W), y = (int)((m / W) % H), e = (int)(m / ((int64_t)W * H));
  const int xsegs = W / HALO_TW, ysegs = H / HALO_TH;
  const int ty = y / HALO_TH, tx = x / HALO_TW, py = y % HALO_TH, px = x % HALO_TW;
  const int tile = (e * ysegs + ty) * xsegs + tx;
  float4 s = reinterpret_cast<const float4*>(dw)[m];
  auto add = [&](int t, int bi) {
    const float4 v = reinterpret_cast<const float4*>(border)[(int64_t)t * HB_N + bi];
    s.x += v.x; s.y += v.y; s.z += v.z; s.w += v.w;
  };
  const bool up = py == 0 && ty > 0, down = py == HALO_TH - 1 && ty < ysegs - 1;
  const bool left = px == 0 && tx > 0, right = px == HALO_TW - 1 && tx < xsegs - 1;
  if (up) add(tile - xsegs, hb_index(HALO_TH, px));
  if (down) add(tile + xsegs, hb_index(-1, px));
  if (left) add(tile - 1, hb_index(py, HALO_TW));
  if (right) add(tile + 1, hb_index(py, -1));
  if (up && left) add(tile - xsegs - 1, hb_index(HALO_TH, HALO_TW));
  if (up && right) add(tile - xsegs + 1, hb_index(HALO_TH, -1));
  if (down && left) add(tile + xsegs - 1, hb_index(-1, HALO_TW));
  if (down && right) add(tile + xsegs + 1, hb_index(-1, -1));
  const float4 b = *reinterpret_cast<const float4*>(bias);
  const float v0 = s.x + b.x, v1 = s.y + b.y, v2 = s.z + b.z, v3 = s.w + b.w;
  reinterpret_cast<float4*>(dw)[m] = make_float4((float)(half_t)v0, (float)(half_t)v1, (float)(half_t)act_apply(v2, VIPE_ACT_SIGMOID),
                                                 (float)(half_t)act_apply(v3, VIPE_ACT_SIGMOID));
}

template <typename K>
void allow_lds(K kernel, std::atomic<uint64_t>& seen, size_t bytes) {
  vipe_once_per_device(seen, [&] { (void)hipFuncSetAttribute((const void*)kernel, hipFuncAttributeMaxDynamicSharedMemorySize, (int)bytes); });
}
constexpr size_t MAX_LDS = 160 * 1024;

bool flat_geometry(ConvArgs& a, int pad) {
  a.f_wp = a.W + pad;
  a.f_hwp = a.H * a.f_wp;
  a.f_tiles = (a.f_hwp + 255) / 256;
  a.f_magic = (unsigned)(((1ull << 32) + (unsigned)a.f_wp - 1) / (unsigned)a.f_wp);
  const int rows = 256 + 2 * a.f_wp + 2;
  a.f_pieces = (rows + 15) / 16;
  a.f_xbytes = a.f_pieces * 1024;
  a.f_p1lo = (a.f_wp + 1) / 16;
  a.f_p1hi = (a.f_wp + 256) / 16;
  return a.f_wp >= 2 && a.f_pieces <= 8 * H32_XP && a.f_hwp < (1 << 23);
}

inline bool needs_tile_kernel(const ConvArgs& a) { return a.accinit || a.epi == EPI_PARTIAL || a.ai_f32 || a.epi == EPI_HEADS_FUSED; }

template <int BMC, int KS, int VAR, bool FLAT>
int launch_halo32(const ConvArgs& a, int tiles, int gy, size_t lds, hipStream_t s) {
  static std::atomic<uint64_t> seen{0};
  allow_lds(conv_halo32_kernel<BMC, KS, true, VAR, FLAT>, seen, FLAT ? MAX_LDS : lds);
  conv_halo32_kernel<BMC, KS, true, VAR, FLAT><<<dim3(tiles * gy), 512, lds, s>>>(a, gy);
  return vipe_launch_status();
}

template <bool FLAT>
int launch_halo_family(ConvArgs& a, int cp, int64_t M, hipStream_t s) {
  const bool split_ok = a.split >= a.Cin || a.split % H32_BK == 0;
  const int tiles = FLAT ? a.B * a.f_tiles : (int)(M / (HALO_TH * HALO_TW));
  const size_t xb = FLAT ? (size_t)a.f_xbytes : (size_t)H32_XBYTES;
  if (a.epi == EPI_HEADS_FUSED) {
    if constexpr (FLAT) return VIPE_EUNSUPPORTED;
    else return launch_halo32<128, 3, 3, false>(a, tiles, 2, 3 * (size_t)128 * 64 + 2 * xb + 1024, s);
  }
  if (needs_tile_kernel(a)) {
    const bool ok = cp >= 64 && split_ok && !(a.KH == 3 && a.Cout <= 16) && !(a.epi == EPI_PARTIAL && a.Cout % 4 != 0) &&
                    !(a.ai_f32 && !a.accinit);
    if (!ok) return VIPE_EUNSUPPORTED;
  }
  if (a.KH == 3 && a.Cout <= 16 && cp == 32 && split_ok && (a.epi == EPI_HEADS || a.epi == EPI_ETA || a.epi == EPI_PLAIN)) {
    static std::atomic<uint64_t> seen{0};
    const size_t lds = 2 * NRW_WBYTES + 2 * xb + 1024;
    allow_lds(conv_halo32_narrow_kernel<FLAT>, seen, FLAT ? MAX_LDS : lds);
    conv_halo32_narrow_kernel<FLAT><<<dim3(tiles), 512, lds, s>>>(a);
    return vipe_launch_status();
  }
  if (!split_ok) return VIPE_EUNSUPPORTED;
  const int bmc = cp >= 128 ? 128 : cp;
  const int gy = cp >= 128 ? cp / 128 : 1;
  size_t lds = 3 * (size_t)bmc * 64 + 2 * xb + 1024;
  const size_t stage = bmc >= 64 ? (size_t)256 * (bmc + 8) * 2 : (size_t)256 * 36 * 4;
  if (lds < stage) lds = stage;
  if (a.ai_f32 || a.epi == EPI_PARTIAL) {
    if (!(a.KH == 3 && bmc == 128 && !(a.ai_f32 && a.epi == EPI_PARTIAL))) return VIPE_EUNSUPPORTED;
    return a.ai_f32 ? launch_halo32<128, 3, 1, FLAT>(a, tiles, gy, lds, s) : launch_halo32<128, 3, 2, FLAT>(a, tiles, gy, lds, s);
  }
  if (a.KH == 3) {
    if (bmc == 128) return launch_halo32<128, 3, 0, FLAT>(a, tiles, gy, lds, s);
    if (bmc == 64) return launch_halo32<64, 3, 0, FLAT>(a, tiles, 1, lds, s);
    return launch_halo32<32, 3, 0, FLAT>(a, tiles, 1, lds, s);
  }
  if (bmc == 128) return launch_halo32<128, 1, 0, FLAT>(a, tiles, gy, lds, s);
  if (bmc == 64) return launch_halo32<64, 1, 0, FLAT>(a, tiles, 1, lds, s);
  return launch_halo32<32, 1, 0, FLAT>(a, tiles, 1, lds, s);
}

template <int BMC, int WM, int WN>
int launch_gather(const ConvArgs& a, bool small, bool glds, int gx, int gy, hipStream_t s) {
  const size_t lds = 2 * (BMC + BNP) * 128;
  if (small) {
    if constexpr (BMC != 128) return VIPE_EUNSUPPORTED;
    else conv_mfma_kernel<BMC, WM, WN, true><<<dim3(gx, gy), 256, lds, s>>>(a);
  } else if (glds) conv_mfma_glds_kernel<BMC, WM, WN><<<dim3(gx * gy), 256, lds, s>>>(a, gy);
  else conv_mfma_kernel<BMC, WM, WN, false><<<dim3(gx, gy), 256, lds, s>>>(a);
  return vipe_launch_status();
}

int launch_conv(ConvArgs& a, hipStream_t s) {
  int cp, cinp, kp;
  if (vipe_conv_packed_dims(a.Cout, a.Cin, a.KH, a.KW, &cp, &cinp, &kp) != VIPE_OK) return VIPE_EINVAL;
  a.Cout_pad = cp;
  a.Cin_pad = cinp;
  a.nsteps = kp / 64;
  const int64_t M = (int64_t)a.B * a.H * a.W;
  if (M == 0) return VIPE_OK;
  const bool small = a.Cin == 4;
  const int gx = (int)((M + BNP - 1) / BNP);
  const bool sq13 = !small && a.KH == a.KW && (a.KH == 1 || a.KH == 3);
  const bool off32 = (int64_t)a.B * a.H * a.W < (1ll << 31);
  const bool aligned = a.W % HALO_TW == 0 && a.H % HALO_TH == 0;
  const bool halo = sq13 && aligned && off32;
  const bool flat = sq13 && !aligned && off32 && flat_geometry(a, a.KH == 3 ? 1 : 0);
  if (needs_tile_kernel(a) && !halo && !flat) return VIPE_EUNSUPPORTED;
  if (a.epi == EPI_GLO && a.KH == 1 && a.KW == 1 && a.Cin == 128 && a.Cout == 128 && cp == 128 && a.split >= a.Cin &&
      a.x0_ctot % 8 == 0 && a.x0_coff % 8 == 0 && a.net == a.x0 && a.net_ctot == a.x0_ctot && a.net_coff == a.x0_coff &&
      a.extra == nullptr) {
    static std::atomic<uint64_t> seen{0};
    allow_lds(conv1x1_glo_kernel, seen, GLO_LDS);
    conv1x1_glo_kernel<<<dim3((unsigned)(a.B * ((a.H * a.W + 255) / 256))), 512, GLO_LDS, s>>>(a);
    return vipe_launch_status();
  }
  if (halo || flat) {
    const int rc = halo ? launch_halo_family<false>(a, cp, M, s) : launch_halo_family<true>(a, cp, M, s);
    if (rc != VIPE_EUNSUPPORTED || needs_tile_kernel(a)) return rc;
  }
  if (small && a.KH == 7 && a.KW == 7 && cp % 128 == 0 && kp == 256 && a.epi == EPI_PLAIN && !a.extra && off32) {
    const int gy = cp / 128;
    if (aligned) {
      static std::atomic<uint64_t> seen{0};
      allow_lds(conv7x7_c4_kernel<false>, seen, C7_LDS);
      conv7x7_c4_kernel<false><<<dim3((int)(M / (HALO_TH * HALO_TW)) * gy), 512, C7_LDS, s>>>(a, gy);
      return vipe_launch_status();
    }
    flat_geometry(a, 3);
    const size_t need = C7_WBYTES + (size_t)(256 + 6 * a.f_wp + 6) * 8;
    if (need <= MAX_LDS && a.f_hwp < (1 << 23) && a.f_wp >= 2) {
      static std::atomic<uint64_t> seen{0};
      allow_lds(conv7x7_c4_kernel<true>, seen, MAX_LDS);
      const size_t lds = need > (size_t)(256 * 136 * 2) ? need : (size_t)(256 * 136 * 2);
      conv7x7_c4_kernel<true><<<dim3(a.B * a.f_tiles * gy), 512, lds, s>>>(a, gy);
      return vipe_launch_status();
    }
  }
  const bool glds = !small && a.KH * a.KW <= 32;
  static std::atomic<uint64_t> s1{0}, s2{0}, s3{0};
  allow_lds(conv_mfma_kernel<128, 2, 2, false>, s1, 65536);
  allow_lds(conv_mfma_kernel<128, 2, 2, true>, s2, 65536);
  allow_lds(conv_mfma_glds_kernel<128, 2, 2>, s3, 65536);
  if (cp >= 128) return launch_gather<128, 2, 2>(a, small, glds, gx, cp / 128, s);
  if (cp == 64) return launch_gather<64, 1, 4>(a, small, glds, gx, 1, s);
  return launch_gather<32, 1, 4>(a, small, glds, gx, 1, s);
}

}

int vipe_conv_run(const ConvCall& c, hipStream_t stream) {
  const int Cin = c.Cin, Cout = c.Cout;
  VIPE_CHECK_ARG(c.x0.p && c.w && c.bias);
  VIPE_CHECK_ARG(!c.accinit.p || (c.accinit.ctot % 4 == 0 && c.accinit.coff % 4 == 0 && c.accinit.coff + Cout <= c.accinit.ctot));
  VIPE_CHECK_ARG(c.B >= 0 && c.H > 0 && c.W > 0 && Cin > 0 && Cout > 0 && (c.KH & 1) && (c.KW & 1));
  if (Cin == 4) {
    VIPE_CHECK_ARG(c.split >= Cin && c.x0.ctot % 4 == 0 && c.x0.coff % 4 == 0);
  } else {
    VIPE_CHECK_ARG(Cin % 8 == 0 && c.x0.ctot % 8 == 0 && c.x0.coff % 8 == 0);
    VIPE_CHECK_ARG(c.split >= Cin || (c.split % 64 == 0 && c.x1.p && c.x1.ctot % 8 == 0 && c.x1.coff % 8 == 0));
  }
  VIPE_CHECK_ARG(c.epi >= EPI_PLAIN && c.epi <= EPI_HEADS_FUSED);
  if (c.epi == EPI_HEADS_FUSED) {
    VIPE_CHECK_ARG(c.fout && c.heads2_frag && c.border && Cin == 128 && Cout == 256 && c.KH == 3 && c.KW == 3 &&
                   c.act == VIPE_ACT_RELU && !c.extra && !c.accinit.p && !c.accinit_f32 && c.split >= Cin);
    if (c.H % HALO_TH != 0 || c.W % HALO_TW != 0) return VIPE_EUNSUPPORTED;
  }
  if (c.epi == EPI_PARTIAL) VIPE_CHECK_ARG(c.fout && c.y.ctot % 4 == 0 && c.y.coff % 4 == 0 && c.y.coff + Cout <= c.y.ctot && !c.extra);
  if (c.epi == EPI_PLAIN) VIPE_CHECK_ARG(c.y.p && c.y.ctot % 4 == 0 && c.y.coff % 4 == 0);
  if (c.epi == EPI_GLO) VIPE_CHECK_ARG(c.net.p && c.fout);
  if (c.epi == EPI_ZR) VIPE_CHECK_ARG(c.y.p && c.y2.p && c.net.p && Cout == 256);
  if (c.epi == EPI_Q) VIPE_CHECK_ARG(c.y.p && c.net.p && c.z && Cout == 128);
  if (c.epi == EPI_HEADS) VIPE_CHECK_ARG(c.fout && Cout == 4);
  if (c.epi == EPI_ETA) VIPE_CHECK_ARG(c.fout && Cout == 1);
  const ConvView& x1 = c.x1.p ? c.x1 : c.x0;
  ConvArgs a = {};
  a.x0 = (const half_t*)c.x0.p; a.x0_ctot = c.x0.ctot; a.x0_coff = c.x0.coff;
  a.x1 = (const half_t*)x1.p; a.x1_ctot = x1.ctot; a.x1_coff = x1.coff;
  a.split = c.split > Cin ? Cin : c.split;
  a.w = (const half_t*)c.w; a.bias = c.bias; a.extra = c.extra; a.extra_stride = c.extra_stride; a.extra_off = c.extra_off;
  a.y = (half_t*)c.y.p; a.y_ctot = c.y.ctot; a.y_coff = c.y.coff;
  a.y2 = (half_t*)c.y2.p; a.y2_ctot = c.y2.ctot; a.y2_coff = c.y2.coff;
  a.w2 = (const half_t*)c.heads2_frag; a.border = c.border;
  a.net = (const half_t*)c.net.p; a.net_ctot = c.net.ctot; a.net_coff = c.net.coff;
  a.zbuf = (const half_t*)c.z; a.fout = c.fout;
  a.accinit = (const half_t*)c.accinit.p; a.ai_ctot = c.accinit.ctot; a.ai_coff = c.accinit.coff; a.ai_f32 = c.accinit_f32;
  a.B = c.B; a.H = c.H; a.W = c.W; a.Cin = Cin; a.Cout = Cout; a.KH = c.KH; a.KW = c.KW;
  a.act = c.act; a.epi = c.epi;
  return launch_conv(a, stream);
}

extern "C" {

VIPE_EXPORT int vipe_conv2d_nhwc_f16(const void* d_x, const void* d_w_packed, const float* d_bias,
                                     const float* d_extra, void* d_y, int B, int H, int W, int Cin, int cin_total,
                                     int cin_off, int Cout, int cout_total, int cout_off, int KH, int KW, int act,
                                     void* stream) {
  VIPE_CHECK_ARG(act >= 0 && act <= 3);
  ConvCall c;
  c.x0 = {d_x, cin_total, cin_off}; c.y = {d_y, cout_total, cout_off};
  c.w = d_w_packed; c.bias = d_bias; c.extra = d_extra; c.extra_stride = Cout;
  c.B = B; c.H = H; c.W = W; c.Cin = Cin; c.Cout = Cout; c.KH = KH; c.KW = KW; c.act = act;
  return vipe_conv_run(c, as_stream(stream));
}

VIPE_EXPORT int vipe_conv2d_fused(const void* d_x0, int x0_ctot, int x0_coff, const void* d_x1, int x1_ctot,
                                  int x1_coff, int split, const void* d_w_packed, const float* d_bias,
                                  const float* d_extra, int extra_stride, int extra_off, void* d_y, int y_ctot,
                                  int y_coff, void* d_y2, int y2_ctot, int y2_coff, const void* d_net, int net_ctot,
                                  int net_coff, const void* d_z, float* d_fout, const void* d_accinit, int ai_ctot,
                                  int ai_coff, int B, int H, int W, int Cin, int Cout, int KH, int KW, int act, int mode,
                                  void* stream) {
  ConvCall c;
  c.x0 = {d_x0, x0_ctot, x0_coff}; c.x1 = {d_x1, x1_ctot, x1_coff}; c.split = split;
  c.w = d_w_packed; c.bias = d_bias; c.extra = d_extra; c.extra_stride = extra_stride; c.extra_off = extra_off;
  c.y = {d_y, y_ctot, y_coff}; c.y2 = {d_y2, y2_ctot, y2_coff}; c.net = {d_net, net_ctot, net_coff};
  c.z = d_z; c.fout = d_fout;
  c.accinit = {d_accinit, ai_ctot, ai_coff}; c.accinit_f32 = (mode & VIPE_CONV_ACCINIT_F32) != 0;
  c.B = B; c.H = H; c.W = W; c.Cin = Cin; c.Cout = Cout; c.KH = KH; c.KW = KW;
  c.act = act; c.epi = mode & ~VIPE_CONV_ACCINIT_F32;
  if (c.epi == EPI_HEADS_FUSED) {
    c.heads2_frag = d_net; c.border = (float*)d_y2;
    c.net.p = c.y2.p = nullptr;
  }
  return vipe_conv_run(c, as_stream(stream));
}

VIPE_EXPORT int vipe_heads_fused_ok(int H, int W) {
  const char* v = getenv("VIPE_AMD_FUSED_HEADS");
  const bool enabled = !(v && v[0] == '0');
  return enabled && H > 0 && W > 0 && H % HALO_TH == 0 && W % HALO_TW == 0;
}

VIPE_EXPORT int vipe_heads_border_floats(int E, int H, int W, int64_t* n) {
  VIPE_CHECK_ARG(n && E >= 0 && H > 0 && W > 0 && H % HALO_TH == 0 && W % HALO_TW == 0);
  *n = (int64_t)E * (H / HALO_TH) * (W / HALO_TW) * HB_N * 4;
  return VIPE_OK;
}

VIPE_EXPORT int vipe_heads_finish(float* d_dw, const float* d_border, const float* d_bias, int E, int H, int W, void* stream) {
  VIPE_CHECK_ARG(E >= 0 && H > 0 && W > 0 && H % HALO_TH == 0 && W % HALO_TW == 0);
  if (E == 0) return VIPE_OK;
  VIPE_CHECK_ARG(d_dw && d_border && d_bias);
  const int64_t M = (int64_t)E * H * W;
  heads_finish_kernel<<<(unsigned)((M + 255) / 256), 256, 0, as_stream(stream)>>>(d_dw, d_border, d_bias, M, H, W);
  return vipe_launch_status();
}

}
```

vipe_amd/csrc/update_op.hip:

```cpp
#include "common.cuh"
#include "conv_call.cuh"

namespace {

__global__ __launch_bounds__(384) void glo_gemm_kernel(const float* __restrict__ glo, const float* __restrict__ wT ,
                                                       const float* __restrict__ b, float* __restrict__ extra, float inv_hw) {
  __shared__ float g[128];
  const int e = blockIdx.x, t = threadIdx.x;
  if (t < 128) g[t] = glo[(int64_t)e * 128 + t] * inv_hw;
  __syncthreads();
  float acc = b[t];
#pragma unroll 8
  for (int k = 0; k < 128; ++k) acc = __builtin_fmaf(g[k], wT[k * 384 + t], acc);
  extra[(int64_t)e * 384 + t] = acc;
}

__global__ __launch_bounds__(256) void update_finish_kernel(const float* __restrict__ coords1, const float* __restrict__ dw,
                                                            const unsigned char* __restrict__ mask, float* __restrict__ target,
                                                            float* __restrict__ weight, const float* __restrict__ eta,
                                                            const int64_t* __restrict__ du, float* __restrict__ damping,
                                                            int64_t n_px, int64_t n_eta, int P) {
  const int64_t i = (int64_t)blockIdx.x * 256 + threadIdx.x;
  if (i < n_px) {
    const float2 c = reinterpret_cast<const float2*>(coords1)[i];
    const float4 d = reinterpret_cast<const float4*>(dw)[i];
    const bool m = mask && mask[i];
    reinterpret_cast<float2*>(target)[i] = make_float2(c.x + d.x, c.y + d.y);
    reinterpret_cast<float2*>(weight)[i] = m ? make_float2(0.f, 0.f) : make_float2(d.z, d.w);
  }
  if (i < n_eta) damping[du[i / P] * P + i % P] = eta[i];
}

hipEvent_t* operator_events() {
  static thread_local hipEvent_t ev[64][4] = {};
  int d = 0;
  (void)hipGetDevice(&d);
  hipEvent_t* e = ev[d & 63];
  for (int i = 0; i < 4; ++i)
    if (!e[i] && hipEventCreateWithFlags(&e[i], hipEventDisableTiming) != hipSuccess) return nullptr;
  return e;
}

struct Grid { int B, H, W; };
#define RUN(call) \
  do { const int rc_ = (call); if (rc_ != VIPE_OK) return rc_; } while (0)

ConvCall conv(Grid g, ConvView x0, int Cin, const void* w, const float* bias, int Cout, int k) {
  ConvCall c;
  c.x0 = x0; c.w = w; c.bias = bias;
  c.B = g.B; c.H = g.H; c.W = g.W; c.Cin = Cin; c.Cout = Cout; c.KH = c.KW = k;
  return c;
}

int relu_conv(Grid g, ConvView x0, int Cin, const void* w, const float* bias, int Cout, int k, ConvView y, hipStream_t st) {
  ConvCall c = conv(g, x0, Cin, w, bias, Cout, k);
  c.y = y; c.act = VIPE_ACT_RELU;
  return vipe_conv_run(c, st);
}

int global_context(const vipe_update_weights* wt, const vipe_update_buffers* b, const void* net, hipStream_t s) {
  if (hipMemsetAsync(b->glo, 0, sizeof(float) * 128 * (size_t)b->E, s) != hipSuccess) return VIPE_EINVAL;
  ConvCall c = conv({b->E, b->H, b->W}, {net, 128, 0}, 128, wt->gw_w, wt->gw_b, 128, 1);
  c.epi = EPI_GLO; c.net = c.x0; c.fout = b->glo;
  RUN(vipe_conv_run(c, s));
  glo_gemm_kernel<<<b->E, 384, 0, s>>>(b->glo, wt->glo_wT, wt->glo_b, b->extra, 1.0f / (float)(b->H * b->W));
  return VIPE_OK;
}
}

extern "C" {

VIPE_EXPORT int vipe_update_operator(const vipe_update_weights* wt, const vipe_update_buffers* b, void* stream) {
  VIPE_CHECK_ARG(wt && b && b->E >= 0 && b->H > 0 && b->W > 0);
  if (b->E == 0) return VIPE_OK;
  const int E = b->E, H = b->H, W = b->W;
  const Grid g = {E, H, W};
  hipStream_t s = as_stream(stream);
  hipStream_t s2 = (hipStream_t)b->side_stream;
  hipEvent_t* ev = s2 ? operator_events() : nullptr;
  if (s2 && !ev) return VIPE_EINVAL;
  hipStream_t side = s2 ? s2 : s;
  auto fork = [&](int i) { return !s2 || (hipEventRecord(ev[i], s) == hipSuccess && hipStreamWaitEvent(s2, ev[i], 0) == hipSuccess); };
  auto join = [&](int i) { return !s2 || (hipEventRecord(ev[i], s2) == hipSuccess && hipStreamWaitEvent(s, ev[i], 0) == hipSuccess); };
  VIPE_CHECK_ARG(fork(0));
  if (b->levels[0]) {
    RUN(vipe_corr_lookup_conv1x1_ex(b->levels, b->coords, wt->corr0_w, wt->corr0_b, b->c1, 128, 0, E, H, W, b->h2, b->w2, 128,
                                    VIPE_ACT_RELU, b->slots, b->pyramid_layout, stream, 0, s2 ? 1 : 0));
  } else {
    VIPE_CHECK_ARG(b->corr);
    RUN(relu_conv(g, {b->corr, 200, 0}, 200, wt->corr0_w, wt->corr0_b, 128, 1, {b->c1, 128, 0}, s));
  }
  RUN(relu_conv(g, {b->c1, 128, 0}, 128, wt->corr2_w, wt->corr2_b, 128, 3, {b->xbuf, 320, 128}, s));
  RUN(relu_conv(g, {b->motn, 4, 0}, 4, wt->flow0_w, wt->flow0_b, 128, 7, {b->f1, 128, 0}, side));
  RUN(relu_conv(g, {b->f1, 128, 0}, 128, wt->flow2_w, wt->flow2_b, 64, 3, {b->xbuf, 320, 256}, side));
  VIPE_CHECK_ARG(join(1));
  const int Es = b->gate_state;
  if (Es != 0) VIPE_CHECK_ARG(Es > 0 && Es <= E && b->pgate && b->pzr && wt->zr_x_w);
  else RUN(global_context(wt, b, b->net, s));
  const bool ctx = b->pgate != nullptr;
  const int gate_cin = ctx ? 320 : 448, rest_coff = ctx ? 128 : 0;
  auto zr = [&](int e0, int n, bool staged) -> int {
    auto at = [&](const void* p, int ctot, int coff) { return ConvView{(const char*)p + (int64_t)e0 * H * W * ctot * 2, ctot, coff}; };
    ConvCall c;
    if (staged) {
      c = conv({n, H, W}, at(b->xbuf, 320, 128), 192, wt->zr_x_w, wt->zr_b, 256, 3);
      c.accinit = {b->pzr + (int64_t)e0 * H * W * 256, 256, 0}; c.accinit_f32 = true;
    } else {
      c = conv({n, H, W}, at(b->net, 128, 0), gate_cin, ctx ? wt->zr_s_w : wt->zr_w, wt->zr_b, 256, 3);
      c.x1 = at(b->xbuf, 320, rest_coff); c.split = 128;
      if (ctx) c.accinit = at(b->pgate, 384, 0);
    }
    c.epi = EPI_ZR; c.extra = b->extra + (int64_t)e0 * 384; c.extra_stride = 384;
    c.y = at(b->zb, 128, 0); c.y2 = at(b->rnet, 128, 0); c.net = at(b->net, 128, 0);
    return vipe_conv_run(c, s);
  };
  if (Es != 0) RUN(zr(0, Es, true));
  if (Es < E) RUN(zr(Es, E - Es, false));
  ConvCall q = conv(g, {b->rnet, 128, 0}, gate_cin, ctx ? wt->q_s_w : wt->q_w, wt->q_b, 128, 3);
  q.x1 = {b->xbuf, 320, rest_coff}; q.split = 128;
  if (ctx) q.accinit = {b->pgate, 384, 256};
  q.epi = EPI_Q; q.extra = b->extra; q.extra_stride = 384; q.extra_off = 256;
  q.y = {b->net_out, 128, 0}; q.net = {b->net, 128, 0}; q.z = b->zb;
  RUN(vipe_conv_run(q, s));
  const bool two_tails = s2 && b->n_src > 0;
  const bool by_consumer = wt->agg1_w && wt->agg1_b && wt->heads_dw_w && wt->heads_dw_b;
  auto heads0 = [&](const void* w, const float* bias, int coff, int cout) -> int {
    return relu_conv(g, {b->net_out, 128, 0}, 128, w, bias, cout, 3, {b->hbuf, 384, coff}, s);
  };
  auto agg_chain = [&](hipStream_t st) -> int {
    if (b->n_src <= 0) return VIPE_OK;
    VIPE_CHECK_ARG(b->order && b->rowptr && b->agg && b->a2 && b->eta);
    const Grid gs = {b->n_src, H, W};
    RUN(vipe_segment_mean_nhwc_f16(b->hbuf, 384, 256, b->order, b->rowptr, b->agg, b->n_src, (int64_t)H * W, 128, st));
    RUN(relu_conv(gs, {b->agg, 128, 0}, 128, wt->agg2_w, wt->agg2_b, 128, 3, {b->a2, 128, 0}, st));
    ConvCall c = conv(gs, {b->a2, 128, 0}, 128, wt->eta_w, wt->eta_b, 1, 3);
    c.epi = EPI_ETA; c.fout = b->eta;
    return vipe_conv_run(c, st);
  };
  auto heads2 = [&](hipStream_t st) -> int {
    ConvCall c = conv(g, {b->hbuf, 384, 0}, 256, wt->heads2_w, wt->heads2_b, 4, 3);
    c.epi = EPI_HEADS; c.fout = b->dw;
    return vipe_conv_run(c, st);
  };
  if (by_consumer && two_tails) {
    RUN(heads0(wt->agg1_w, wt->agg1_b, 256, 128));
    VIPE_CHECK_ARG(fork(2));
    RUN(agg_chain(side));
    if (wt->heads2_frag && b->hborder && vipe_heads_fused_ok(H, W)) {
      ConvCall c = conv(g, {b->net_out, 128, 0}, 128, wt->heads_dw_w, wt->heads_dw_b, 256, 3);
      c.act = VIPE_ACT_RELU; c.epi = EPI_HEADS_FUSED; c.heads2_frag = wt->heads2_frag; c.border = b->hborder; c.fout = b->dw;
      RUN(vipe_conv_run(c, s));
      RUN(vipe_heads_finish(b->dw, b->hborder, wt->heads2_b, E, H, W, stream));
    } else {
      RUN(heads0(wt->heads_dw_w, wt->heads_dw_b, 0, 256));
      RUN(heads2(s));
    }
  } else {
    RUN(heads0(wt->heads0_w, wt->heads0_b, 0, 384));
    if (two_tails) VIPE_CHECK_ARG(fork(2));
    RUN(heads2(two_tails ? s2 : s));
    RUN(agg_chain(s));
  }
  if (two_tails) VIPE_CHECK_ARG(join(3));
  return vipe_launch_status();
}

VIPE_EXPORT int vipe_update_gate_state(const vipe_update_weights* wt, const vipe_update_buffers* b, const void* d_net,
                                       int parts, void* stream) {
  VIPE_CHECK_ARG(wt && b && b->E >= 0 && b->H > 0 && b->W > 0 && parts >= 1 && parts <= 3);
  if (b->E == 0) return VIPE_OK;
  VIPE_CHECK_ARG(d_net && (!(parts & 1) || (b->glo && b->extra)) && (!(parts & 2) || (b->pgate && b->pzr && wt->zr_n_w)));
  if (parts & 1) RUN(global_context(wt, b, d_net, as_stream(stream)));
  if (parts & 2) {
    ConvCall c = conv({b->E, b->H, b->W}, {d_net, 128, 0}, 128, wt->zr_n_w, wt->zr_b, 256, 3);
    c.epi = EPI_PARTIAL; c.accinit = {b->pgate, 384, 0};
    c.fout = b->pzr; c.y = {nullptr, 256, 0};
    RUN(vipe_conv_run(c, as_stream(stream)));
  }
  return vipe_launch_status();
}
#undef RUN

VIPE_EXPORT int vipe_update_gate_state_piece(void* user, int piece, int n_pieces, void* stream) {
  const vipe_gate_state_job* j = (const vipe_gate_state_job*)user;
  VIPE_CHECK_ARG(j && j->weights && j->buffers && j->net && n_pieces > 0 && piece >= 0 && piece < n_pieces);
  const vipe_update_buffers* b = j->buffers;
  VIPE_CHECK_ARG(b->E >= 0 && b->H > 0 && b->W > 0 && b->pgate && b->pzr);
  int64_t e0 = (int64_t)b->E * piece / n_pieces, e1 = (int64_t)b->E * (piece + 1) / n_pieces;
  if (j->bounds && j->n_bounds == n_pieces + 1) {
    e0 = j->bounds[piece];
    e1 = j->bounds[piece + 1];
    VIPE_CHECK_ARG(j->bounds[0] == 0 && j->bounds[n_pieces] == b->E && e0 >= 0 && e0 <= e1 && e1 <= b->E);
  }
  if (e1 <= e0) return VIPE_OK;
  const int64_t px = (int64_t)b->H * b->W;
  vipe_update_buffers sub = *b;
  sub.E = (int)(e1 - e0);
  sub.pgate = (const char*)b->pgate + e0 * px * 384 * 2;
  sub.pzr = b->pzr + e0 * px * 256;
  return vipe_update_gate_state(j->weights, &sub, (const char*)j->net + e0 * px * 128 * 2, 2, stream);
}

VIPE_EXPORT int vipe_glo_context(const float* d_glo_sum, const float* d_wT, const float* d_bias, float* d_extra, int E, int hw,
                                 void* stream) {
  VIPE_CHECK_ARG(E >= 0 && hw > 0);
  if (E == 0) return VIPE_OK;
  VIPE_CHECK_ARG(d_glo_sum && d_wT && d_bias && d_extra);
  glo_gemm_kernel<<<E, 384, 0, as_stream(stream)>>>(d_glo_sum, d_wT, d_bias, d_extra, 1.0f / (float)hw);
  return vipe_launch_status();
}

VIPE_EXPORT int vipe_update_finish(const float* d_coords1, const float* d_dw, const unsigned char* d_mask, float* d_target,
                                   float* d_weight, const float* d_eta, const int64_t* d_du, float* d_damping, int E,
                                   int n_src, int ht, int wd, void* stream) {
  VIPE_CHECK_ARG(E >= 0 && n_src >= 0 && ht > 0 && wd > 0);
  if (E == 0) return VIPE_OK;
  VIPE_CHECK_ARG(d_coords1 && d_dw && d_target && d_weight && (n_src == 0 || (d_eta && d_du && d_damping)));
  const int P = ht * wd;
  const int64_t n_px = (int64_t)E * P, n_eta = (int64_t)n_src * P;
  const int64_t n = n_px > n_eta ? n_px : n_eta;
  update_finish_kernel<<<(unsigned)((n + 255) / 256), 256, 0, as_stream(stream)>>>(d_coords1, d_dw, d_mask, d_target, d_weight,
                                                                                  d_eta, d_du, d_damping, n_px, n_eta, P);
  return vipe_launch_status();
}

}
```

vipe_amd/slam/factor_graph.py:

```python

import ctypes
import dataclasses
import os

import numpy as np
import torch

from .._lib import check, check_gpu_contig, lib, parse_struct, require, stream_ptr, upload, upload_many
from ..ext import slam_ext
from .edge_index import NAMES, EdgeIndex, as_host
from .networks import AltCorrBlock, CorrBlock, CorrPool

WORK = {"edge_updates": 0, "pyramids_built": 0}
BACKEND_VOLUME_GB = 160


def warm_volume_pool(device, gigabytes=None):
    if torch.device(device).type != "cuda":
        return 0
    want = float(gigabytes if gigabytes is not None else os.environ.get("VIPE_AMD_BACKEND_VOLUME_GB", BACKEND_VOLUME_GB)) * 2**30
    free, _ = torch.cuda.mem_get_info(device)
    n = int(min(want, 0.85 * free))
    if n <= 0:
        return 0
    x = torch.empty(n, dtype=torch.uint8, device=device)
    x[::1 << 21].zero_()
    del x
    return n


RowsJob = parse_struct("vipe_rows_job")
NhwcJob = parse_struct("vipe_nhwc_job")


def per_view(x, V):
    if V == 1:
        return x
    views = torch.arange(V, device=x.device) if torch.is_tensor(x) else np.arange(V)
    return (x[:, None] * V + views).reshape(-1)


def host_csr(dix, n_src):
    order = np.argsort(dix, kind="stable").astype(np.int32)
    rowptr = np.concatenate([[0], np.cumsum(np.bincount(dix, minlength=n_src))]).astype(np.int32)
    return order, rowptr


def chunk_groups(cnt, max_edges):
    groups, size = [], 0
    for g0 in range(0, len(cnt), 8):
        n8 = int(cnt[g0:g0 + 8].sum())
        if n8 == 0:
            continue
        if not groups or size + n8 > max_edges:
            groups.append([])
            size = 0
        groups[-1].append(g0)
        size += n8
    return groups


BackendChunkPlan = dataclasses.make_dataclass("BackendChunkPlan", frozen=True, fields=[
    ("groups", list), ("rows", list), ("max_rows", int), ("max_edges", int), ("budget_rows", int), ("keep_all", bool), ("keep_some", bool)])
_BackendChunk = dataclasses.make_dataclass("_BackendChunk", ["idx_x", "edges", "du", "dixs", "csr", "mask", "xb", "pgate"])


def plan_backend_chunks(cnt, n_views, bytes_per_pyramid, steps, use_volume, budget_bytes, chunk_edges):
    keep_all = bool(use_volume and steps > 1 and int(cnt.sum()) * n_views * bytes_per_pyramid <= budget_bytes)
    keep_some = bool(use_volume and steps > 1 and not keep_all)
    budget_rows = int(budget_bytes / bytes_per_pyramid)
    max_edges = max(8, min(chunk_edges, budget_rows // n_views))
    if keep_some:
        max_edges = max(8, min(max_edges, max(256, budget_rows // (8 * n_views))))
    groups = chunk_groups(cnt, max_edges)
    rows = [int(sum(cnt[g0:g0 + 8].sum() for g0 in grp)) * n_views for grp in groups]
    return BackendChunkPlan(groups, rows, max(rows, default=0), max_edges, budget_rows, keep_all, keep_some)


class _PyramidResidency:

    def __init__(self, plan):
        self.plan, self._vols, self.kept_rows = plan, {}, 0
        self.get = self._vols.get

    def offer(self, gi, vol):
        p, n = self.plan, self.plan.rows[gi]
        if p.keep_all or (p.keep_some and self.kept_rows + n + p.max_rows <= p.budget_rows):
            self._vols[gi] = vol
            self.kept_rows += n


def rows_gather(jobs):
    arr = (RowsJob * len(jobs))()
    for j, job in zip(arr, jobs):
        src, dst, idx, n_rows, row_bytes, dst_row0, seg = (*job, None)[:7]
        check_gpu_contig(src, dst, idx)
        require(idx.dtype == torch.int64, "row indices must be int64")
        j.src, j.dst, j.idx = src.data_ptr(), dst.data_ptr(), idx.data_ptr()
        j.src_row_pitch = j.dst_row_pitch = row_bytes
        j.seg_bytes, j.seg_pitch, j.n_seg = seg or (row_bytes, row_bytes, 1)
        j.n_rows, j.dst_row0 = int(n_rows), int(dst_row0)
    if jobs:
        check(lib().vipe_rows_gather(ctypes.addressof(arr), len(jobs), stream_ptr(jobs[0][2])), "rows_gather")


class _EdgeStores:

    def __init__(self, ht, wd, device, with_pgate):
        self.ht, self.wd, self.device, self.with_pgate = ht, wd, device, with_pgate
        self.cap = 0
        self.net, self.xb, self.pg = [None, None], [None, None], [None, None]
        self.cur = 0

    def _alloc(self, cap):
        f16 = dict(dtype=torch.float16, device=self.device)
        shp = (cap, self.ht, self.wd)
        return ([torch.empty(shp + (128,), **f16) for _ in range(2)], [torch.empty(shp + (320,), **f16) for _ in range(2)],
                [torch.empty(shp + (384,), **f16) if self.with_pgate else None for _ in range(2)])

    def bank_of(self, net_n):
        if net_n is not None and self.net[0] is not None:
            for k in (0, 1):
                if net_n.data_ptr() == self.net[k].data_ptr():
                    return k
        return None

    def reserve(self, rows, net_n, n_live):
        grow = rows > self.cap
        if grow:
            cap = max(rows + rows // 4, 64)
            net, xb, pg = self._alloc(cap)
            if n_live and self.cap:
                xb[0][:n_live, ..., :128] = self.xb[self.cur][:n_live, ..., :128]
                if self.with_pgate:
                    pg[0][:n_live] = self.pg[self.cur][:n_live]
            old = net_n
            self.net, self.xb, self.pg, self.cur, self.cap = net, xb, pg, 0, cap
            if n_live and old is not None:
                self.net[0][:n_live] = old
                return self.net[0][:n_live]
            return None
        if n_live and self.bank_of(net_n) is None:
            self.net[0][:n_live] = net_n
            return self.net[0][:n_live]
        return net_n

    def net_spare(self, net_n):
        k = self.bank_of(net_n)
        return None if k is None else self.net[1 - k][:net_n.shape[0]]

    def append(self, buffer_nets, buffer_inps, frames, net_n, n_live):
        k = int(frames.shape[0])
        if n_live == 0:
            net_n = None
        net_n = self.reserve(n_live + k, net_n, n_live)
        nb = 0 if net_n is None else self.bank_of(net_n)
        P = self.ht * self.wd
        require(frames.dtype == torch.int64, "frame indices must be int64")
        jobs = (NhwcJob * 2)()
        for j, (src, dst, ctot) in enumerate(((buffer_nets, self.net[nb], 128), (buffer_inps, self.xb[self.cur], 320))):
            check_gpu_contig(src, frames, dst)
            jobs[j].src, jobs[j].frame, jobs[j].dst = src.data_ptr(), frames.data_ptr(), dst.data_ptr()
            jobs[j].dst_row_pitch, jobs[j].dst_ctot, jobs[j].dst_coff, jobs[j].dst_row0 = P * ctot, ctot, 0, n_live
        check(lib().vipe_gather_nchw_to_nhwc_f16(ctypes.addressof(jobs), 2, k, 128, P, stream_ptr(frames)), "gather_nchw_to_nhwc")
        n = n_live + k
        return self.net[nb][:n], self.xb[self.cur][:n], self.xb[self.cur][n_live:n]

    def compact(self, keep, n_keep, net_n, extra_jobs=()):
        P = self.ht * self.wd
        nb = self.bank_of(net_n)
        jobs = []
        if n_keep:
            jobs.append((self.net[nb], self.net[1 - nb], keep, n_keep, P * 128 * 2, 0))
            jobs.append((self.xb[self.cur], self.xb[1 - self.cur], keep, n_keep, P * 320 * 2, 0, (256, 640, P)))
            if self.with_pgate:
                jobs.append((self.pg[self.cur], self.pg[1 - self.cur], keep, n_keep, P * 384 * 2, 0))
        rows_gather(jobs + list(extra_jobs))
        self.cur ^= 1
        return (self.net[1 - nb][:n_keep], self.xb[self.cur][:n_keep], self.pg[self.cur][:n_keep] if self.with_pgate else None)


def _index_property(name):
    def put(self, tensor):
        self._index.assign(name, tensor)
        if name != "age":
            self._edges_changed()

    return property(lambda self: self._index.device(name), put)


class FactorGraph:
    upsample = False
    upsample_from_row = None
    _last_ba = None

    def __init__(self, update_module, buffer, device, max_factors=48, incremental=True, cross_view=False):
        self.update_op = update_module
        self.buffer = buffer
        self.device = device
        self.max_factors = max_factors
        self.incremental = incremental
        self.cross_view = cross_view and buffer.n_views > 1
        ht, wd = buffer.height // 8, buffer.width // 8
        self.ht, self.wd = ht, wd
        self.damping = 1e-6 * torch.ones_like(buffer.flattened_disps)
        self.target = torch.zeros([1, 0, ht, wd, 2], device=device, dtype=torch.float)
        self.weight = torch.zeros([1, 0, ht, wd, 2], device=device, dtype=torch.float)
        self.corr, self.net_n, self.xbuf = None, None, None
        self.pgate = None
        self._stores = None
        self._gate_state = None
        self._side = None
        self.gate_overlap_min_edges = int(os.environ.get("VIPE_AMD_GATE_OVERLAP_MIN_EDGES", "64"))
        self.gate_overlap_mode = "gated"
        self.gate_overlap_share = 0.5
        self.gate_overlap_fractions = [0.4, 0.4, 0.2]
        self.target_inac = torch.zeros([1, 0, ht, wd, 2], device=device, dtype=torch.float)
        self.weight_inac = torch.zeros([1, 0, ht, wd, 2], device=device, dtype=torch.float)
        self._plan = None
        self._plan_serial = 0
        self._ba_state = {}
        self._spare = None
        self._inac_cap = None

    ii, jj, age, ii_inac, jj_inac = (_index_property(n) for n in NAMES)

    @property
    def _index(self):
        index = self.__dict__.get("_edge_index")
        if index is None:
            index = self.__dict__["_edge_index"] = EdgeIndex(self.device)
        return index

    def host_edges(self):
        return dict(self._index.host)

    def _edges_changed(self):
        self._plan = None
        self._gate_state = None

    @torch.no_grad()
    def add_factors(self, ii, jj, remove=False):
        ii_h, jj_h = self._index.absent(as_host(ii), as_host(jj))
        if ii_h.shape[0] == 0:
            return
        if (self.max_factors > 0 and self._index.host["ii"].shape[0] + ii_h.shape[0] > self.max_factors and self.corr is not None
                and remove):
            ix = np.argsort(self._index.host["age"], kind="stable")
            self.rm_factors(ix >= self.max_factors - ii_h.shape[0], store=True)
        ii, jj = upload_many([ii_h, jj_h], self.device)
        pi, qi, _, pj, qj, _ = self.buffer.expand_edge_multiview(ii, jj)
        V = self.buffer.n_views
        n_live = 0 if self.net_n is None else int(self.net_n.shape[0])
        f1, f2 = (pi, pj) if V == 1 else (pi * V + qi, pj * V + qj)
        if self.incremental:
            if self.corr is None:
                self.corr = CorrPool(capacity=max(64, self.max_factors + 16))
            lo, hi = int(min(ii_h.min(), jj_h.min())), int(max(ii_h.max(), jj_h.max()))
            rng = (0, self.buffer.n_frames * V) if (self.cross_view and V > 1) else (lo * V, (hi + 1) * V)
            self.corr.add_edges(self.buffer.flattened_fmaps, f1, f2, frame_range=rng)
            WORK["pyramids_built"] += int(pi.shape[0])
            eng = self.update_op.engine(self.device)
            if self._stores is None:
                self._stores = _EdgeStores(self.ht, self.wd, self.device, eng.supports_gate_split(self.ht, self.wd))
            self.net_n, self.xbuf, xb_new = self._stores.append(self.buffer.flattened_nets, self.buffer.flattened_inps,
                                                                f1.contiguous(), self.net_n, n_live)
            if self._stores.with_pgate:
                pg = self._stores.pg[self._stores.cur]
                eng.gate_context(xb_new, out=pg[n_live:n_live + xb_new.shape[0]])
                self.pgate = pg[:n_live + xb_new.shape[0]]
        else:
            net = self.buffer.nets[pi, qi].permute(0, 2, 3, 1).contiguous()
            self.net_n = net if self.net_n is None else torch.cat([self.net_n, net], 0)
        target, _ = self.buffer.reproject_dense_disp(ii, jj)
        target = target[None]
        self._index.append(ii_h, jj_h)
        self._edges_changed()
        self.target = torch.cat([self.target, target], 1)
        self.weight = torch.cat([self.weight, torch.zeros_like(target)], 1)

    @torch.no_grad()
    def rm_factors(self, mask, store=False):
        m = as_host(mask, bool)
        if not m.any():
            return
        self._index.remove(m, store)
        self._edges_changed()
        V = self.buffer.n_views
        keep_x_np, drop_x_np = per_view(np.flatnonzero(~m), V), per_view(np.flatnonzero(m), V)
        keep_x, drop_x = upload_many([keep_x_np, drop_x_np], self.device)
        nk, nd = int(keep_x_np.shape[0]), int(drop_x_np.shape[0])
        if self.corr is not None:
            self.corr = self.corr[keep_x_np]
        self._contiguous_targets()
        row = int(self.target.shape[2] * self.target.shape[3] * 2 * 4)
        new_t = torch.empty((1, nk) + tuple(self.target.shape[2:]), dtype=self.target.dtype, device=self.device)
        new_w = torch.empty_like(new_t)
        extra = [(self.target, new_t, keep_x, nk, row, 0), (self.weight, new_w, keep_x, nk, row, 0)] if nk else []
        if store and nd:
            ti, wi, n0 = self._inactive_room(nd)
            extra += [(self.target, ti, drop_x, nd, row, n0), (self.weight, wi, drop_x, nd, row, n0)]
        st = self._stores
        if st is not None and self.net_n is not None and st.bank_of(self.net_n) is None and self.net_n.shape[0]:
            self.net_n = st.reserve(self.net_n.shape[0], self.net_n, self.net_n.shape[0])
        if st is not None and self.net_n is not None and st.bank_of(self.net_n) is not None:
            self.net_n, self.xbuf, pg = st.compact(keep_x, nk, self.net_n, extra)
            if self.pgate is not None:
                self.pgate = pg
        else:
            if self.net_n is not None:
                self.net_n = self.net_n[keep_x]
            rows_gather(extra)
        self.target, self.weight = new_t, new_w

    def add_neighborhood_factors(self, t0, t1, r=3):
        ii, jj = torch.meshgrid(torch.arange(t0, t1), torch.arange(t0, t1), indexing="ij")
        ii, jj = ii.reshape(-1), jj.reshape(-1)
        keep = ((ii - jj).abs() > 0) & ((ii - jj).abs() <= r)
        self.add_factors(ii[keep], jj[keep])

    @torch.no_grad()
    def add_proximity_factors(self, t0=0, t1=0, rad=2, nms=2, beta=0.25, thresh=16.0, remove=False, dist=None):
        assert t0 >= t1, "t0 should be a subset of t1"
        t = self.buffer.n_frames
        iin, jjn = np.meshgrid(np.arange(t0, t, dtype=np.int64), np.arange(t1, t, dtype=np.int64), indexing="ij")
        iin, jjn = iin.reshape(-1), jjn.reshape(-1)
        if iin.size == 0:
            return
        if dist is not None:
            d = np.array(dist, dtype=np.float32).reshape(-1)
            assert d.shape[0] == iin.shape[0]
        else:
            ii, jj = upload_many([iin, jjn], self.device)
            d = self.buffer.frame_distance_dense_disp(ii, jj, beta=beta)
            d = (d[:, 0] if d.shape[1] == 1 else d.mean(-1)).cpu().numpy().astype(np.float32)
        nj = t - t1

        def suppress(i, j):
            if (t0 <= i < t) and (t1 <= j < t):
                d[(i - t0) * nj + (j - t1)] = np.inf

        D = d.reshape(t - t0, nj)
        h = self.host_edges()
        I = np.concatenate([h["ii"], h["ii_inac"]])
        J = np.concatenate([h["jj"], h["jj_inac"]])
        if I.size:
            lim = np.maximum(np.minimum(np.abs(I - J) - 2, nms), 0)
            for di in range(-nms, nms + 1):
                for dj in range(-nms, nms + 1):
                    sel = (abs(di) + abs(dj)) <= lim
                    a, b = I[sel] + di, J[sel] + dj
                    ok = (a >= t0) & (a < t) & (b >= t1) & (b < t)
                    D[a[ok] - t0, b[ok] - t1] = np.inf
        d[(iin - rad < jjn) | (d > thresh)] = np.inf
        es = []
        for i in range(t0, t):
            if self.cross_view:
                es.append((i, i))
                suppress(i, i)
            for j in range(max(i - rad - 1, 0), i):
                es.append((i, j))
                es.append((j, i))
                suppress(i, j)
        order = np.argsort(d, kind="stable")
        order = order[d[order] <= thresh]
        nt = t - t0
        diamonds = []
        for lim_k in range(nms + 1):
            dd = [(di, dj) for di in range(-nms, nms + 1) for dj in range(-nms, nms + 1) if abs(di) + abs(dj) <= lim_k]
            diamonds.append((np.array([x[0] for x in dd]), np.array([x[1] for x in dd])))
        for k in order.tolist():
            if d[k] > thresh:
                continue
            if len(es) > self.max_factors:
                break
            i, j = int(iin[k]), int(jjn[k])
            es.append((i, j))
            es.append((j, i))
            ddi, ddj = diamonds[max(min(abs(i - j) - 2, nms), 0)]
            a, b = i - t0 + ddi, j - t1 + ddj
            ok = (a >= 0) & (a < nt) & (b >= 0) & (b < nj)
            d[a[ok] * nj + b[ok]] = np.inf
        if len(es) == 0:
            return
        e = np.asarray(es, dtype=np.int64)
        self.add_factors(e[:, 0], e[:, 1], remove)

    @torch.no_grad()
    def rm_second_newest_keyframe(self, ix):
        self.buffer.remove_second_newest(ix)
        active, inactive = self._index.drop_keyframe(ix)
        self._edges_changed()
        if inactive.any():
            keep_x = per_view(upload(np.flatnonzero(~inactive), self.device), self.buffer.n_views)
            self.target_inac = self.target_inac[:, keep_x]
            self.weight_inac = self.weight_inac[:, keep_x]
        self.rm_factors(active, store=False)

    def get_edges_np(self):
        ii, jj = self.ii.cpu().numpy(), self.jj.cpu().numpy()
        w = torch.mean(self.weight, dim=[0, 2, 3, 4]).cpu().numpy()
        ix = np.argsort(ii)
        return np.stack([ii[ix], jj[ix]], axis=1), w[ix]

    @property
    def f_net(self):
        return None if self.net_n is None else self.net_n.permute(0, 3, 1, 2)[None]

    @property
    def inp(self):
        return None if self.xbuf is None else self.xbuf[..., 0:128].permute(0, 3, 1, 2)[None]

    def _net_spare(self):
        sp = self._stores.net_spare(self.net_n) if self._stores is not None else None
        if sp is not None:
            return sp
        sp = self._spare
        if sp is None or sp.shape != self.net_n.shape or sp.data_ptr() == self.net_n.data_ptr():
            sp = torch.empty_like(self.net_n)
        self._spare = self.net_n
        return sp

    def _edge_plan(self):
        if self._plan is None:
            pi, qi, di, pj, qj, _ = self.buffer.expand_edge_multiview(self.ii, self.jj)
            ii_h, jj_h = self._index.host["ii"], self._index.host["jj"]
            self._plan_serial += 1
            if self.cross_view or self.buffer.n_views > 1:
                from .update_engine import segment_csr
                du, dix = torch.unique(di, return_inverse=True)
                n_src = int(du.numel())
                csr = segment_csr(dix, n_src)
            else:
                du_h, dix_h = np.unique(ii_h, return_inverse=True)
                du, dix = upload_many([du_h, dix_h], self.device)
                n_src = int(du_h.shape[0])
                csr = tuple(upload_many(host_csr(dix_h, n_src), self.device, torch.int32))
            self._plan = dict(pi=pi, qi=qi, di=di, pj=pj, qj=qj, du=du, dix=dix, n_src=n_src, csr=csr,
                              t0=int(max(1, ii_h.min() + 1)), t1=int(max(ii_h.max(), jj_h.max()) + 1), base=int(min(ii_h.min(), jj_h.min())))
        return self._plan

    def _inactive_room(self, k):
        n = self.target_inac.shape[1]
        cap = self._inac_cap
        if cap is None or cap[0].shape[1] < n + k or cap[0].data_ptr() != self.target_inac.data_ptr():
            size = max(2 * (n + k), 256)
            cap = tuple(torch.empty((1, size) + tuple(x.shape[2:]), dtype=x.dtype, device=x.device)
                        for x in (self.target_inac, self.weight_inac))
            cap[0][:, :n] = self.target_inac
            cap[1][:, :n] = self.weight_inac
            self._inac_cap = cap
        self.target_inac, self.weight_inac = cap[0][:, :n + k], cap[1][:, :n + k]
        return cap[0], cap[1], n

    def _upsample_disps(self, mask, du, own=None):
        from ..ext import droid_net_ext
        buf = self.buffer
        require(buf.disps_up is not None, "FactorGraph.upsample needs GraphBuffer(upsample_disps=True)")
        droid_net_ext.cvx_upsample(buf.flattened_disps[..., None], mask, rows=du if own is None else own[0],
                                   out=buf.flattened_disps_up[..., None])
        flags = buf.disps_up_valid.view(-1)
        if own is None:
            flags[du] = True
        else:
            flags[du] = flags[du] | own[1]

    def _own_rows(self, P):
        key = ("own_rows", int(self.upsample_from_row))
        if key not in P:
            keep = P["du"] >= key[1]
            P[key] = (torch.where(keep, P["du"], torch.full_like(P["du"], -1)), keep)
        return P[key]

    def _shift_plan(self, plan5, base):
        pi, qi, di, pj, qj = plan5
        if self.cross_view or base <= 0:
            return (pi, qi, di, pj, qj, 0)
        V = self.buffer.n_views
        return (pi - base, qi, di - base * V, pj - base, qj, base)

    def _ba_plan(self, P):
        if "ba_plan" not in P:
            P["ba_plan"] = self._shift_plan((P["pi"], P["qi"], P["di"], P["pj"], P["qj"]), P["base"])
        return P["ba_plan"]

    @staticmethod
    def _ba_flags(t0, t1, **flags):
        return dict(dict(t0=t0, t1=t1, pose_damping=1e-3, pose_ep=0.1, motion_only=False, limited_disp=False,
                         optimize_intrinsics=False, optimize_rig_rotation=False), **flags)

    def _contiguous_targets(self):
        self.weight, self.target = self.weight.contiguous(), self.target.contiguous()

    @torch.no_grad()
    def update(self, t0=None, t1=None, itrs=3, use_inactive=False, motion_only=False, fixed_motion=False,
               limited_disp=False):
        assert self.incremental and self.corr is not None and self.xbuf is not None and self.net_n is not None
        assert not (motion_only and fixed_motion)
        P = self._edge_plan()
        t0 = P["t0"] if t0 is None else t0
        t1 = P["t1"] if t1 is None else t1
        buf = self.buffer
        E_act = int(P["pi"].shape[0])
        WORK["edge_updates"] += E_act
        if "io" not in P:
            P["io"] = (torch.empty((E_act, self.ht, self.wd, 2), dtype=torch.float32, device=self.device),
                       torch.empty((E_act, self.ht, self.wd, 4), dtype=torch.float16, device=self.device))
            P["mask"] = buf.masks[P["pi"], P["qi"]].contiguous()
        self._contiguous_targets()
        coords1, motn = slam_ext.reproject_motion_nhwc(buf.poses, buf.flattened_disps, buf.intrinsics, buf.rig,
                                                       P["pi"], P["qi"], P["pj"], P["qj"], P["di"],
                                                       self.target[0], camera=buf.camera_type, out=P["io"])
        eng = self.update_op.engine(self.device)
        corr = self.corr.lookup_deferred(coords1)
        up = {"want_upmask": True} if self.upsample else {}
        self.net_n, dw, eta, upmask = eng.forward_nhwc(self.net_n, self.xbuf, corr, motn, ix=P["dix"], n_src=P["n_src"],
                                                       net_out=self._net_spare(), csr=P["csr"], pgate=self.pgate,
                                                       gate_state=self._gate_state, **up)
        self._gate_state = None
        overlap = self.pgate is not None and E_act >= self.gate_overlap_min_edges
        ba_overlap = None
        if overlap:
            main = torch.cuda.current_stream(self.device)
            if self._side is None:
                self._side = torch.cuda.Stream(device=self.device)
            self._side.wait_stream(main)
            n_staged = max(1, int(round(self.gate_overlap_share * E_act)))
            if self.gate_overlap_mode == "gated":
                with torch.cuda.stream(self._side):
                    eng.hidden_gate_state(self.net_n, self.pgate, parts=1)
                fr = self.gate_overlap_fractions if len(self.gate_overlap_fractions) == itrs else None
                gate_state, ov = eng.gate_state_job(self.net_n, self.pgate, fractions=fr, n_staged=n_staged)
                ba_overlap = ov(self._side)
            else:
                with torch.cuda.stream(self._side):
                    gate_state = eng.hidden_gate_state(self.net_n, self.pgate, n_staged=n_staged)
        slam_ext.update_finish(coords1, dw, P["mask"], self.target, self.weight, eta, P["du"], self.damping)
        if use_inactive:
            key = ("inac", t0)
            if key not in P:
                h = self._index.host
                sel_h = np.flatnonzero((h["ii_inac"] >= t0 - 3) & (h["jj_inac"] >= t0 - 3))
                ii, jj, sel_exp = upload_many([np.concatenate([h["ii_inac"][sel_h], h["ii"]]),
                                               np.concatenate([h["jj_inac"][sel_h], h["jj"]]),
                                               per_view(sel_h, buf.n_views)], self.device)
                base = int(min(h["ii"].min(), h["jj"].min(), *(h[k][sel_h].min() for k in ("ii_inac", "jj_inac") if sel_h.size)))
                plan = self._shift_plan(buf.expand_edge_multiview(ii, jj)[:5], base)
                n_sel = int(sel_exp.shape[0])
                comb = tuple(torch.empty((1, n_sel + E_act) + tuple(x.shape[2:]), dtype=x.dtype, device=x.device)
                             for x in (self.target, self.weight))
                comb[0][:, :n_sel] = self.target_inac.index_select(1, sel_exp)
                comb[1][:, :n_sel] = self.weight_inac.index_select(1, sel_exp)
                P[key] = (ii, jj, plan, comb, n_sel)
            ii, jj, plan, comb, n_sel = P[key]
            plan_key = (self._plan_serial, "inac", t0)
            if self.target.data_ptr() != comb[0][:, n_sel:].data_ptr():
                comb[0][:, n_sel:] = self.target
                comb[1][:, n_sel:] = self.weight
                self.target, self.weight = comb[0][:, n_sel:], comb[1][:, n_sel:]
            target, weight = comb
        else:
            ii, jj, target, weight = self.ii, self.jj, self.target, self.weight
            plan = self._ba_plan(P)
            plan_key = (self._plan_serial, "act")
        E = target.shape[1]
        self._last_ba = self._ba_flags(t0, t1 if not fixed_motion else t0, motion_only=motion_only, limited_disp=limited_disp)
        buf.bundle_adjustment(target.view(E, -1, 2), weight.view(E, -1, 2), self.damping, ii, jj, n_iters=itrs,
                              **self._last_ba, plan=plan, ba_state=self._ba_state, plan_key=plan_key, overlap=ba_overlap)
        if self.upsample:
            self._upsample_disps(upmask, P["du"], own=None if self.upsample_from_row is None else self._own_rows(P))
        if overlap:
            main.wait_stream(self._side)
            self._gate_state = gate_state
        self._index.tick()

    @torch.no_grad()
    def marginals(self, t0=None, t1=None, **flags):
        P = self._edge_plan() if int(self.ii.shape[0]) else None
        ba = dict(self._last_ba or self._ba_flags(P["t0"] if P else 0, P["t1"] if P else 0))
        ba.update(flags)
        ba.update({k: v for k, v in (("t0", t0), ("t1", t1)) if v is not None})
        E = self.target.shape[1]
        return self.buffer.ba_marginals(self.target.contiguous().view(E, -1, 2), self.weight.contiguous().view(E, -1, 2),
                                        self.damping, self.ii, self.jj, **ba, plan=self._ba_plan(P) if P else None)

    def _backend_chunk(self, plan, gi, eng):
        buf, V, ii_np = self.buffer, self.buffer.n_views, self._index.host["ii"]
        sel = np.flatnonzero(np.isin(ii_np // 8 * 8, plan.groups[gi]))
        if sel.shape[0] == ii_np.shape[0]:
            idx_x, iis, jjs = None, self.ii, self.jj
        else:
            idx = upload(sel, self.device)
            idx_x, iis, jjs = per_view(idx, V), self.ii[idx], self.jj[idx]
        edges = buf.expand_edge_multiview(iis, jjs)
        pis, qis = edges[:2]
        du_np, dixs_np = np.unique(per_view(ii_np[sel], V), return_inverse=True)
        du, dixs = upload_many([du_np, dixs_np], self.device)
        mask = buf.masks[pis, qis].contiguous()
        csr = tuple(upload_many(host_csr(dixs_np, du_np.shape[0]), self.device, torch.int32))
        xb = torch.empty((plan.rows[gi], self.ht, self.wd, 320), dtype=torch.half, device=self.device)
        xb[..., 0:128] = buf.inps[pis, qis].permute(0, 2, 3, 1)
        pgate = eng.gate_context(xb) if eng.supports_gate_split(self.ht, self.wd) else None
        return _BackendChunk(idx_x=idx_x, edges=edges, du=du, dixs=dixs, csr=csr, mask=mask, xb=xb, pgate=pgate)

    @torch.no_grad()
    def update_batch(self, itrs, steps, optimize_intrinsics, optimize_rig_rotation, solver_verbose=False):
        assert self.net_n is not None
        buf, eng = self.buffer, self.update_op.engine(self.device)
        from ..ext import droid_net_ext
        use_volume = (droid_net_ext.fused_build_covers(buf.flattened_fmaps.shape[1], self.ht, self.wd, 4, buf.flattened_fmaps.dtype)
                      and os.environ.get("VIPE_AMD_BACKEND_ALTCORR") is None)
        corr_op = None if use_volume else AltCorrBlock(buf.flattened_fmaps[None])
        P, V = self._edge_plan(), buf.n_views
        ii_np = self._index.host["ii"]
        assert self._index.host["jj"].max() >= ii_np.max()
        G_, S_, R_ = droid_net_ext.blocked_dims(self.ht, self.wd)[:3]
        plan = plan_backend_chunks(np.bincount(ii_np), V, (G_ * 64) * (R_ * 4 * S_ * 32) * 2 * (1 + 1 / 4 + 1 / 16 + 1 / 64), steps,
                                   use_volume, float(os.environ.get("VIPE_AMD_BACKEND_VOLUME_GB", BACKEND_VOLUME_GB)) * 2**30,
                                   int(os.environ.get("VIPE_AMD_BACKEND_CHUNK_EDGES", "4096")))
        chunks, kept = {}, _PyramidResidency(plan)
        for step in range(steps):
            up = {"want_upmask": True} if self.upsample and step == steps - 1 else {}
            upmasks = []
            coords1, motn = slam_ext.reproject_motion_nhwc(buf.poses, buf.flattened_disps, buf.intrinsics, buf.rig,
                                                           P["pi"], P["qi"], P["pj"], P["qj"], P["di"],
                                                           self.target[0].contiguous(), camera=buf.camera_type)
            for gi in range(len(plan.groups)):
                if gi not in chunks:
                    chunks[gi] = self._backend_chunk(plan, gi, eng)
                c, n = chunks[gi], plan.rows[gi]
                take = (lambda x: x) if c.idx_x is None else (lambda x: x.index_select(0, c.idx_x))
                c1 = take(coords1)
                pis, qis, dis, pjs, qjs, djs = c.edges
                if use_volume:
                    vol = kept.get(gi)
                    if vol is None:
                        corr_n = None
                        lo, hi = (0, buf.n_frames) if (self.cross_view and V > 1) else (P["base"], P["t1"])
                        vol = CorrBlock.from_buffer(buf.flattened_fmaps, pis * V + qis, pjs * V + qjs, frame_range=(lo * V, hi * V))
                        WORK["pyramids_built"] += n
                        kept.offer(gi, vol)
                    corr_n = vol.lookup_deferred(c1)
                else:
                    corr1 = corr_op(c1[None], dis, djs)
                    corr_n = torch.zeros((n, self.ht, self.wd, 200), dtype=torch.half, device=self.device)
                    corr_n[..., :196] = corr1[0].permute(0, 2, 3, 1)
                net, dw, eta, upmask = eng.forward_nhwc(take(self.net_n).contiguous(), c.xb, corr_n, take(motn).contiguous(),
                                                        ix=c.dixs, n_src=int(c.du.shape[0]), csr=c.csr, pgate=c.pgate, **up)
                if up:
                    upmasks.append((upmask, c.du))
                WORK["edge_updates"] += n
                self._gate_state = None
                if c.idx_x is None:
                    self.net_n = net if net.data_ptr() != self.net_n.data_ptr() else net.clone()
                    self._contiguous_targets()
                    slam_ext.update_finish(c1, dw, c.mask, self.target, self.weight, eta, c.du, self.damping)
                else:
                    weight = dw[..., 2:4].masked_fill(c.mask.unsqueeze(-1), 0.0)
                    self.net_n[c.idx_x] = net
                    self.target[0, c.idx_x] = c1 + dw[..., 0:2]
                    self.weight[0, c.idx_x] = weight
                    self.damping[c.du] = eta
            E = self.target.shape[1]
            self._last_ba = self._ba_flags(1, buf.n_frames, pose_damping=1e-5, pose_ep=1e-2, optimize_intrinsics=optimize_intrinsics,
                                           optimize_rig_rotation=optimize_rig_rotation)
            buf.bundle_adjustment(self.target.view(E, -1, 2), self.weight.view(E, -1, 2), self.damping, self.ii, self.jj,
                                  n_iters=itrs, **self._last_ba, verbose=solver_verbose)
            for upmask, du in upmasks:
                self._upsample_disps(upmask, du)
```

vipe_amd/slam/update_engine.py:

```python

import ctypes
import os

import torch

from .._lib import check, lib, parse_struct, ptr, stream_ptr

UpdateWeights = parse_struct("vipe_update_weights")
UpdateBuffers = parse_struct("vipe_update_buffers")
GateStateJob = parse_struct("vipe_gate_state_job")

ACT = {"none": 0, "relu": 1, "sigmoid": 2, "tanh": 3}
EPI = {"plain": 0, "glo": 1, "zr": 2, "q": 3, "heads": 4, "eta": 5, "partial": 6, "heads_fused": 7}
ACCINIT_F32 = 0x100
CORR_CH = 200


class _Packed:

    def __init__(self, w_oihw, bias, device):
        w = w_oihw.detach().to(device=device, dtype=torch.float16).contiguous()
        self.cout, self.cin, self.kh, self.kw = w.shape
        cp, cinp, kp = ctypes.c_int(), ctypes.c_int(), ctypes.c_int()
        check(lib().vipe_conv_packed_dims(self.cout, self.cin, self.kh, self.kw, ctypes.addressof(cp),
                                          ctypes.addressof(cinp), ctypes.addressof(kp)), "conv_packed_dims")
        self.packed = torch.empty(kp.value * cp.value, dtype=torch.float16, device=device)
        check(lib().vipe_conv_pack_weights(ptr(w), ptr(self.packed), self.cout, self.cin, self.kh, self.kw, 0,
                                           stream_ptr(w)), "conv_pack_weights")
        assert bias.numel() == self.cout, (tuple(bias.shape), self.cout)
        self.bias = torch.zeros(cp.value, dtype=torch.float32, device=device)
        self.bias[:self.cout] = bias.detach().to(device=device, dtype=torch.float32).reshape(-1)
        self.flops_per_pixel = 2.0 * self.cout * self.cin * self.kh * self.kw


def heads2_fragment_index():
    import numpy as np
    s, h, rb, ip, lane, e = np.meshgrid(*[np.arange(n) for n in (2, 2, 2, 2, 64, 8)], indexing="ij")
    row = 16 * rb + lane % 16
    tap, o = row // 2, row % 2
    ch = 128 * s + 64 * h + 16 * (2 * ip + e // 4) + 4 * (lane // 16) + e % 4
    valid = row < 18
    return np.where(valid, 2 * s + o, 0), ch, np.where(valid, tap, 0), valid


def pack_heads2_fragments(h2_oihw):
    out, ch, tap, valid = (torch.from_numpy(a).to(h2_oihw.device) for a in heads2_fragment_index())
    w = h2_oihw.reshape(4, 256, 9)[out, ch, tap]
    return torch.where(valid, w, torch.zeros_like(w)).to(torch.float16).contiguous().reshape(-1)


def segment_csr(ix, n_src):
    order = torch.argsort(ix, stable=True).to(torch.int32).contiguous()
    counts = torch.bincount(ix, minlength=n_src)
    rowptr = torch.zeros(n_src + 1, dtype=torch.int32, device=ix.device)
    rowptr[1:] = torch.cumsum(counts, 0).to(torch.int32)
    return order, rowptr


class UpdateEngine:
    def __init__(self, module, device):
        self.device = device
        self.m = module
        self._bufs = {}
        self._op_side = None
        self.op_side_min_edges = int(os.environ.get("VIPE_AMD_OP_SIDE_MIN_EDGES", "64"))
        self._gate_gen = 0
        self._pack_all()

    def _pack_all(self):
        m, d = self.m, self.device
        f16 = torch.float16

        def wb(conv):
            return conv.weight.detach().to(d, f16), conv.bias.detach().to(d, torch.float32)

        w, b = wb(m.corr_encoder[0])
        w = torch.cat([w, torch.zeros(128, CORR_CH - 196, 1, 1, device=d, dtype=f16)], 1)
        self.corr0 = _Packed(w, b, d)
        self.corr2 = _Packed(*wb(m.corr_encoder[2]), d)
        self.flow0 = _Packed(*wb(m.flow_encoder[0]), d)
        self.flow2 = _Packed(*wb(m.flow_encoder[2]), d)
        self.gw = _Packed(*wb(m.gru.w), d)
        wz, bz = wb(m.gru.convz)
        wr, br = wb(m.gru.convr)
        self.zr = _Packed(torch.cat([wz, wr], 0), torch.cat([bz, br], 0), d)
        wq, bq = wb(m.gru.convq)
        self.q = _Packed(wq, bq, d)
        rest = list(range(0, 128)) + list(range(256, 448))
        self.zr_s = _Packed(torch.cat([wz, wr], 0)[:, rest].contiguous(), torch.cat([bz, br], 0), d)
        self.q_s = _Packed(wq[:, rest].contiguous(), bq, d)
        self.gates_inp = _Packed(torch.cat([wz, wr, wq], 0)[:, 128:256].contiguous(), torch.zeros(384, device=d), d)
        self.zr_n = _Packed(torch.cat([wz, wr], 0)[:, 0:128].contiguous(), torch.cat([bz, br], 0), d)
        self.zr_x = _Packed(torch.cat([wz, wr], 0)[:, 256:448].contiguous(), torch.cat([bz, br], 0), d)
        wd0, bd0 = wb(m.delta[0])
        ww0, bw0 = wb(m.weight[0])
        wa1, ba1 = wb(m.agg.conv1)
        self.heads0 = _Packed(torch.cat([wd0, ww0, wa1], 0), torch.cat([bd0, bw0, ba1], 0), d)
        self.heads_by_consumer = os.environ.get("VIPE_AMD_HEADS_BY_CONSUMER", "1") != "0"
        self.agg1 = _Packed(wa1, ba1, d)
        self.heads_dw = _Packed(torch.cat([wd0, ww0], 0), torch.cat([bd0, bw0], 0), d)
        wd2, bd2 = wb(m.delta[2])
        ww2, bw2 = wb(m.weight[2])
        h2 = torch.zeros(4, 256, 3, 3, device=d, dtype=f16)
        h2[0:2, 0:128] = wd2[:2]
        h2[2:4, 128:256] = ww2[:2]
        self.heads2 = _Packed(h2, torch.cat([bd2[:2], bw2[:2]], 0), d)
        self.heads2_frag = pack_heads2_fragments(h2)
        self.fused_heads_on = self.heads_by_consumer and os.environ.get("VIPE_AMD_FUSED_HEADS", "1") != "0"
        self.agg2 = _Packed(*wb(m.agg.conv2), d)
        self.eta = _Packed(*wb(m.agg.eta[0]), d)
        self.upmask = _Packed(*wb(m.agg.upmask[0]), d)
        g = m.gru
        self.glo_w = torch.cat([g.convz_glo.weight, g.convr_glo.weight, g.convq_glo.weight], 0).detach().to(d).float() \
            .reshape(384, 128).t().contiguous()
        self.glo_b = torch.cat([g.convz_glo.bias, g.convr_glo.bias, g.convq_glo.bias], 0).detach().to(d).float()
        wd_ = UpdateWeights()
        for name, pk in dict(corr0=self.corr0, corr2=self.corr2, flow0=self.flow0, flow2=self.flow2, gw=self.gw, zr=self.zr,
                             q=self.q, heads0=self.heads0, heads2=self.heads2, agg2=self.agg2, eta=self.eta).items():
            setattr(wd_, name + "_w", pk.packed.data_ptr())
            setattr(wd_, name + "_b", pk.bias.data_ptr())
        wd_.zr_s_w, wd_.q_s_w = self.zr_s.packed.data_ptr(), self.q_s.packed.data_ptr()
        wd_.zr_n_w, wd_.zr_x_w = self.zr_n.packed.data_ptr(), self.zr_x.packed.data_ptr()
        wd_.glo_wT, wd_.glo_b = self.glo_w.data_ptr(), self.glo_b.data_ptr()
        if self.heads_by_consumer:
            wd_.agg1_w, wd_.agg1_b = self.agg1.packed.data_ptr(), self.agg1.bias.data_ptr()
            wd_.heads_dw_w, wd_.heads_dw_b = self.heads_dw.packed.data_ptr(), self.heads_dw.bias.data_ptr()
            if self.fused_heads_on:
                wd_.heads2_frag = self.heads2_frag.data_ptr()
        self._wdesc = wd_
        self._bdesc = {}

    def _conv(self, pk, x0, x0_coff, B, H, W, y=None, y_coff=0, act="none", mode="plain", x1=None, x1_coff=0,
              split=None, extra=None, extra_off=0, y2=None, y2_coff=0, net=None, net_coff=0, z=None, fout=None,
              cin=None, accinit=None, ai_coff=0, w2=None, border=None):
        cin = pk.cin if cin is None else cin
        split = cin if split is None else split
        if mode == "heads_fused":
            assert net is None and y2 is None and w2 is not None and border is not None
            net, y2 = w2, border
        check(lib().vipe_conv2d_fused(
            ptr(x0), x0.shape[-1], x0_coff, ptr(x1), x1.shape[-1] if x1 is not None else 0, x1_coff, split,
            ptr(pk.packed), ptr(pk.bias), ptr(extra), extra.shape[-1] if extra is not None else 0, extra_off,
            ptr(y), (y if y is not None else fout).shape[-1] if (y is not None or mode == "partial") else 0, y_coff,
            ptr(y2), y2.shape[-1] if y2 is not None else 0, y2_coff,
            ptr(net), net.shape[-1] if net is not None else 0, net_coff, ptr(z), ptr(fout), ptr(accinit),
            accinit.shape[-1] if accinit is not None else 0, ai_coff, B, H, W, cin, pk.cout,
            pk.kh, pk.kw, ACT[act],
            EPI[mode] | (ACCINIT_F32 if accinit is not None and accinit.dtype == torch.float32 else 0),
            stream_ptr(x0)), "conv2d_fused")

    @staticmethod
    def supports_gate_split(ht, wd):
        return (wd % 64 == 0 and ht % 4 == 0) or wd <= 126

    def gate_context(self, xbuf, out=None):
        E, H, W, _ = xbuf.shape
        pg = out if out is not None else torch.empty((E, H, W, 384), dtype=torch.float16, device=xbuf.device)
        self._conv(self.gates_inp, xbuf, 0, E, H, W, y=pg, act="none", cin=128)
        return pg

    @torch.no_grad()
    def hidden_gate_state(self, net, pgate, native=True, parts=3, n_staged=None):
        E, H, W, _ = net.shape
        gs, b, glo = self._gate_state(net, pgate, n_staged)
        Es, pzr, extra = gs["n_staged"], gs["pzr"], gs["extra"]
        if native:
            for part, n in ((1, E), (2, Es)):
                if parts & part:
                    b.E = n
                    check(lib().vipe_update_gate_state(ctypes.addressof(self._wdesc), ctypes.addressof(b), ptr(net), part,
                                                       stream_ptr(net)), "update_gate_state")
        else:
            if parts & 1:
                glo.zero_()
                self._conv(self.gw, net, 0, E, H, W, mode="glo", net=net, fout=glo)
                check(lib().vipe_glo_context(ptr(glo), ptr(self.glo_w), ptr(self.glo_b), ptr(extra), E, H * W,
                                             stream_ptr(glo)), "glo_context")
            if parts & 2:
                self._conv(self.zr_n, net, 0, Es, H, W, mode="partial", fout=pzr, accinit=pgate, ai_coff=0)
        return gs

    def _gate_state(self, net, pgate, n_staged):
        E, H, W, _ = net.shape
        Es = E if n_staged is None else max(1, min(E, int(n_staged)))
        self._gate_gen += 1
        glo = self._buf("glo", (E, 128), torch.float32)
        extra = self._buf("extra", (E, 384), torch.float32)
        pzr = self._buf("pzr", (Es, H, W, 256), torch.float32)
        b = UpdateBuffers()
        b.E, b.H, b.W = Es, H, W
        b.pgate, b.pzr, b.glo, b.extra = pgate.data_ptr(), pzr.data_ptr(), glo.data_ptr(), extra.data_ptr()
        gs = dict(net_ptr=net.data_ptr(), pgate_ptr=pgate.data_ptr(), shape=tuple(net.shape), pzr=pzr, extra=extra,
                  n_staged=Es, keep=(b,), gen=self._gate_gen)
        return gs, b, glo

    def gate_state_job(self, net, pgate, fractions=None, n_staged=None):
        gs, b, _ = self._gate_state(net, pgate, n_staged)
        E = gs["n_staged"]
        job = GateStateJob()
        job.weights, job.buffers, job.net = ctypes.addressof(self._wdesc), ctypes.addressof(b), net.data_ptr()
        bounds = None
        if fractions:
            cum, acc = [0], 0.0
            for f in fractions[:-1]:
                acc += f
                cum.append(min(E, int(round(E * acc / sum(fractions)))))
            cum.append(E)
            bounds = (ctypes.c_int * len(cum))(*cum)
            job.bounds, job.n_bounds = ctypes.addressof(bounds), len(cum)
        fn = ctypes.cast(lib().vipe_update_gate_state_piece, ctypes.c_void_p).value
        gs["keep"] = (b, job, bounds)
        return gs, (lambda stream: (stream.cuda_stream, fn, ctypes.addressof(job)))

    def gate_state_matches(self, gs, net, pgate):
        return (gs is not None and pgate is not None and gs["net_ptr"] == net.data_ptr() and
                gs["pgate_ptr"] == pgate.data_ptr() and gs["shape"] == tuple(net.shape) and gs.get("gen") == self._gate_gen)

    def fused_heads(self, H, W):
        return self.fused_heads_on and bool(lib().vipe_heads_fused_ok(H, W))

    def _hborder(self, E, H, W):
        n = ctypes.c_int64()
        check(lib().vipe_heads_border_floats(E, H, W, ctypes.addressof(n)), "heads_border_floats")
        return self._buf("hborder", (n.value,), torch.float32)

    def _buf(self, name, shape, dtype=torch.float16):
        t = self._bufs.get(name)
        if t is None or tuple(t.shape) != tuple(shape) or t.dtype != dtype:
            t = torch.empty(shape, dtype=dtype, device=self.device)
            self._bufs[name] = t
        return t

    @torch.no_grad()
    def forward_nhwc(self, net, xbuf, corr, motn, ix=None, n_src=None, net_out=None, want_upmask=False, csr=None,
                     pgate=None, native=True, gate_state=None):
        E, H, W, _ = net.shape
        if not self.gate_state_matches(gate_state, net, pgate):
            gate_state = None
        if gate_state is None:
            self._gate_gen += 1
        c1 = self._buf("c1", (E, H, W, 128))
        f1 = self._buf("f1", (E, H, W, 128))
        zb = self._buf("z", (E, H, W, 128))
        rnet = self._buf("rnet", (E, H, W, 128))
        hbuf = self._buf("h", (E, H, W, 384))
        dw = self._buf("dw", (E, H, W, 4), torch.float32)
        glo = self._buf("glo", (E, 128), torch.float32)
        if net_out is None:
            net_out = torch.empty_like(net)
        if native:
            return self._forward_native(net, xbuf, corr, motn, ix, n_src, net_out, want_upmask, csr, pgate,
                                        (c1, f1, zb, rnet, hbuf, dw, glo), gate_state)
        if isinstance(corr, tuple):
            from ..ext import droid_net_ext
            droid_net_ext.corr_lookup_conv1x1(corr[1], corr[2], self.corr0.packed, self.corr0.bias, c1, act="relu",
                                              slots=corr[3] if len(corr) > 3 else None,
                                              grid=corr[4] if len(corr) > 4 else None)
        else:
            self._conv(self.corr0, corr, 0, E, H, W, y=c1, act="relu", cin=CORR_CH)
        self._conv(self.corr2, c1, 0, E, H, W, y=xbuf, y_coff=128, act="relu")
        self._conv(self.flow0, motn, 0, E, H, W, y=f1, act="relu")
        self._conv(self.flow2, f1, 0, E, H, W, y=xbuf, y_coff=256, act="relu")
        extra = self._buf("extra", (E, 384), torch.float32)
        if gate_state is None:
            glo.zero_()
            self._conv(self.gw, net, 0, E, H, W, mode="glo", net=net, fout=glo)
            check(lib().vipe_glo_context(ptr(glo), ptr(self.glo_w), ptr(self.glo_b), ptr(extra), E, H * W, stream_ptr(glo)),
                  "glo_context")
        if gate_state is not None:
            Es = gate_state["n_staged"]
            self._conv(self.zr_x, xbuf, 128, Es, H, W, y=zb, y2=rnet, net=net, mode="zr", extra=extra,
                       accinit=gate_state["pzr"], ai_coff=0, cin=192)
            if Es < E:
                self._conv(self.zr_s, net[Es:], 0, E - Es, H, W, x1=xbuf[Es:], x1_coff=128, split=128, y=zb[Es:], y2=rnet[Es:],
                           net=net[Es:], mode="zr", extra=extra[Es:], accinit=pgate[Es:], ai_coff=0)
            self._conv(self.q_s, rnet, 0, E, H, W, x1=xbuf, x1_coff=128, split=128, y=net_out, net=net, z=zb, mode="q",
                       extra=extra, extra_off=256, accinit=pgate, ai_coff=256)
        elif pgate is not None:
            self._conv(self.zr_s, net, 0, E, H, W, x1=xbuf, x1_coff=128, split=128, y=zb, y2=rnet, net=net, mode="zr",
                       extra=extra, accinit=pgate, ai_coff=0)
            self._conv(self.q_s, rnet, 0, E, H, W, x1=xbuf, x1_coff=128, split=128, y=net_out, net=net, z=zb, mode="q",
                       extra=extra, extra_off=256, accinit=pgate, ai_coff=256)
        else:
            self._conv(self.zr, net, 0, E, H, W, x1=xbuf, split=128, y=zb, y2=rnet, net=net, mode="zr", extra=extra)
            self._conv(self.q, rnet, 0, E, H, W, x1=xbuf, split=128, y=net_out, net=net, z=zb, mode="q", extra=extra,
                       extra_off=256)
        if n_src is None and ix is not None:
            n_src = int(ix.max().item()) + 1 if ix.numel() else 0
        eta = upmask = a2 = None

        def agg_chain():
            order, rowptr = csr if csr is not None else segment_csr(ix, n_src)
            agg = self._buf("agg", (n_src, H, W, 128))
            check(lib().vipe_segment_mean_nhwc_f16(ptr(hbuf), 384, 256, ptr(order), ptr(rowptr), ptr(agg), n_src, H * W,
                                                   128, stream_ptr(hbuf)), "segment_mean")
            a2 = self._buf("a2", (n_src, H, W, 128))
            eta = self._buf("eta", (n_src, H, W), torch.float32)
            self._conv(self.agg2, agg, 0, n_src, H, W, y=a2, act="relu")
            self._conv(self.eta, a2, 0, n_src, H, W, mode="eta", fout=eta)
            return a2, eta

        chain = ix is not None and n_src > 0
        if self.heads_by_consumer and chain and E >= self.op_side_min_edges:
            self._conv(self.agg1, net_out, 0, E, H, W, y=hbuf, y_coff=256, act="relu")
            a2, eta = agg_chain()
            if self.fused_heads(H, W):
                hborder = self._hborder(E, H, W)
                self._conv(self.heads_dw, net_out, 0, E, H, W, act="relu", mode="heads_fused", w2=self.heads2_frag,
                           border=hborder, fout=dw)
                check(lib().vipe_heads_finish(ptr(dw), ptr(hborder), ptr(self.heads2.bias), E, H, W, stream_ptr(dw)),
                      "heads_finish")
            else:
                self._conv(self.heads_dw, net_out, 0, E, H, W, y=hbuf, act="relu")
                self._conv(self.heads2, hbuf, 0, E, H, W, mode="heads", fout=dw, cin=256)
        else:
            self._conv(self.heads0, net_out, 0, E, H, W, y=hbuf, act="relu")
            self._conv(self.heads2, hbuf, 0, E, H, W, mode="heads", fout=dw, cin=256)
            if ix is not None:
                a2, eta = agg_chain()
        if ix is not None and want_upmask:
            upmask = torch.empty((n_src, H, W, 576), dtype=torch.float16, device=self.device)
            self._conv(self.upmask, a2, 0, n_src, H, W, y=upmask)
        return net_out, dw, eta, upmask

    def _forward_native(self, net, xbuf, corr, motn, ix, n_src, net_out, want_upmask, csr, pgate, scratch,
                        gate_state=None):
        c1, f1, zb, rnet, hbuf, dw, glo = scratch
        E, H, W, _ = net.shape
        extra = self._buf("extra", (E, 384), torch.float32)
        eta = agg = a2 = order = rowptr = None
        if ix is not None:
            if n_src is None:
                n_src = int(ix.max().item()) + 1 if ix.numel() else 0
            if csr is None:
                csr = segment_csr(ix, n_src)
            order, rowptr = csr
            agg = self._buf("agg", (n_src, H, W, 128))
            a2 = self._buf("a2", (n_src, H, W, 128))
            eta = self._buf("eta", (n_src, H, W), torch.float32)
        lookup = isinstance(corr, tuple)
        hborder = self._hborder(E, H, W) if self.fused_heads(H, W) else None
        tensors = (net, net_out, xbuf, motn, pgate, c1, f1, zb, rnet, hbuf, dw, glo, extra, order, rowptr, agg, a2, eta,
                   hborder) + \
            ((tuple(corr[1]) + (corr[2],) + ((corr[3],) if len(corr) > 3 and corr[3] is not None else ())) if lookup else (corr,))
        pzr = gate_state["pzr"] if gate_state is not None else None
        two_streams = E >= self.op_side_min_edges
        if two_streams and self._op_side is None:
            self._op_side = torch.cuda.Stream(device=self.device)
        key = tuple(0 if t is None else t.data_ptr() for t in tensors) + (E, H, W, n_src or 0, two_streams,
                                                                         0 if pzr is None else pzr.data_ptr(),
                                                                         0 if pzr is None else int(gate_state["n_staged"]))
        b = self._bdesc.get(key)
        if b is None:
            if len(self._bdesc) > 16:
                self._bdesc.clear()
            b = UpdateBuffers()
            b.E, b.H, b.W, b.n_src = E, H, W, int(n_src or 0) if ix is not None else 0
            if lookup:
                lv = corr[1]
                for i in range(4):
                    b.levels[i] = lv[i].data_ptr()
                b.coords = corr[2].data_ptr()
                b.slots = corr[3].data_ptr() if len(corr) > 3 and corr[3] is not None else None
                if len(corr) > 4 and corr[4] is not None:
                    b.h2, b.w2 = int(corr[4][0]), int(corr[4][1])
                else:
                    b.h2, b.w2 = int(lv[2].shape[3]) << 2, int(lv[2].shape[4]) << 2
                b.pyramid_layout = 1 if lv[0].dim() == 7 else 0
            else:
                b.corr = corr.data_ptr()
            for name, t in dict(motn=motn, net=net, net_out=net_out, xbuf=xbuf, pgate=pgate, c1=c1, f1=f1, zb=zb, rnet=rnet,
                                hbuf=hbuf, dw=dw, glo=glo, extra=extra, order=order, rowptr=rowptr, agg=agg, a2=a2,
                                eta=eta, hborder=hborder).items():
                setattr(b, name, None if t is None else t.data_ptr())
            if pzr is not None:
                b.pzr, b.gate_state = pzr.data_ptr(), int(gate_state["n_staged"])
            if two_streams:
                b.side_stream = self._op_side.cuda_stream
            self._bdesc[key] = b
        check(lib().vipe_update_operator(ctypes.addressof(self._wdesc), ctypes.addressof(b), stream_ptr(net)),
              "update_operator")
        upmask = None
        if want_upmask and ix is not None:
            upmask = torch.empty((n_src, H, W, 576), dtype=torch.float16, device=self.device)
            self._conv(self.upmask, a2, 0, n_src, H, W, y=upmask)
        return net_out, dw, eta, upmask

    @torch.no_grad()
    def forward(self, net, inp, corr, flow=None, ix=None, skip_upmask=False, n_src=None):
        batch, num, ch, ht, wd = net.shape
        E = batch * num
        dev = net.device
        f16 = torch.float16
        net_n = net.reshape(E, 128, ht, wd).to(f16).permute(0, 2, 3, 1).contiguous()
        xbuf = torch.empty((E, ht, wd, 320), dtype=f16, device=dev)
        xbuf[..., 0:128] = inp.reshape(E, 128, ht, wd).permute(0, 2, 3, 1)
        corr_n = torch.zeros((E, ht, wd, CORR_CH), dtype=f16, device=dev)
        corr_n[..., :196] = corr.reshape(E, 196, ht, wd).permute(0, 2, 3, 1)
        if flow is None:
            motn_n = torch.zeros((E, ht, wd, 4), dtype=f16, device=dev)
        else:
            motn_n = flow.reshape(E, 4, ht, wd).to(f16).permute(0, 2, 3, 1).contiguous()
        ixd = ix.to(dev) if ix is not None else None
        pgate = self.gate_context(xbuf) if self.supports_gate_split(ht, wd) else None
        net_o, dw, eta, upmask = self.forward_nhwc(net_n, xbuf, corr_n, motn_n, ixd, n_src, want_upmask=not skip_upmask,
                                                   pgate=pgate)
        net_out = net_o.permute(0, 3, 1, 2).reshape(batch, num, 128, ht, wd)
        dwv = dw.view(batch, num, ht, wd, 4).to(f16)
        delta, weight = dwv[..., 0:2].contiguous(), dwv[..., 2:4].contiguous()
        if ix is None:
            return net_out, delta, weight
        n_src = eta.shape[0]
        if upmask is not None:
            upmask = upmask.permute(0, 3, 1, 2).reshape(batch, n_src, 576, ht, wd)
        return net_out, delta, weight, eta.clone().view(batch, n_src, ht, wd), upmask
```

Measured before the change: 276.9.

## Share per-source gate context rows across edges via row indirection

Adds a GateContextPool that stores the precomputed gate context (pgate) once per unique key, presumably the source frame, instead of once per edge. Edges refer to their pool row through an int32 index array. The conv kernels gain an accinit_rows indirection so the accumulator-init load reads the shared row. This avoids recomputing and storing duplicate per-edge gate context, cutting memory traffic and gate_context compute when edges share sources. In exchange it adds host-side refcount bookkeeping, an index upload, and scattered accinit reads.

```diff
diff --git a/include/vipe_amd.h b/include/vipe_amd.h
--- a/include/vipe_amd.h
+++ b/include/vipe_amd.h
@@ -271,6 +271,12 @@
                       const void* d_net, int net_ctot, int net_coff, const void* d_z, float* d_fout,
                       const void* d_accinit, int ai_ctot, int ai_coff, int B, int H, int W, int Cin, int Cout, int KH,
                       int KW, int act, int mode, void* stream);
+int vipe_conv2d_fused_rows(const void* d_x0, int x0_ctot, int x0_coff, const void* d_x1, int x1_ctot, int x1_coff,
+                           int split, const void* d_w_packed, const float* d_bias, const float* d_extra, int extra_stride,
+                           int extra_off, void* d_y, int y_ctot, int y_coff, void* d_y2, int y2_ctot, int y2_coff,
+                           const void* d_net, int net_ctot, int net_coff, const void* d_z, float* d_fout,
+                           const void* d_accinit, int ai_ctot, int ai_coff, int B, int H, int W, int Cin, int Cout, int KH,
+                           int KW, int act, int mode, void* stream, const int* d_accinit_rows);
 
 int vipe_heads_fused_ok(int H, int W);
 int vipe_heads_border_floats(int E, int H, int W, int64_t* n_floats);
@@ -309,6 +315,7 @@
   float* pzr;
   int gate_state;
   float* hborder;
+  const int* pgate_rows;
 } vipe_update_buffers;
 int vipe_update_operator(const vipe_update_weights* weights, const vipe_update_buffers* buffers, void* stream);
 
diff --git a/vipe_amd/csrc/conv_call.cuh b/vipe_amd/csrc/conv_call.cuh
--- a/vipe_amd/csrc/conv_call.cuh
+++ b/vipe_amd/csrc/conv_call.cuh
@@ -23,6 +23,7 @@
   ConvView net;
   ConvView accinit;
   bool accinit_f32 = false;
+  const int* accinit_rows = nullptr;
   const void* z = nullptr;
   float* fout = nullptr;
   const void* heads2_frag = nullptr;
diff --git a/vipe_amd/csrc/conv_mfma.hip b/vipe_amd/csrc/conv_mfma.hip
--- a/vipe_amd/csrc/conv_mfma.hip
+++ b/vipe_amd/csrc/conv_mfma.hip
@@ -29,6 +29,7 @@
   float* fout;
   const half_t* accinit; int ai_ctot, ai_coff;
   int ai_f32;
+  const int* ai_rows;
   const half_t* w2;
   float* border;
   int f_wp, f_hwp, f_tiles, f_pieces, f_xbytes, f_p1lo, f_p1hi;
@@ -405,10 +406,11 @@
   const int pitch = FLAT ? a.f_wp : HALO_PITCH;
   const int xbytes = FLAT ? a.f_xbytes : H32_XBYTES;
   const int npieces = FLAT ? a.f_pieces : H32_PIECES;
-  auto pix_of = [&](int pl) -> int64_t {
-    if constexpr (FLAT) return flat_pixel(q0 + pl, e, a.H, a.W, a.f_wp, a.f_hwp, a.f_magic);
-    else return ((int64_t)(e * a.H + y0 + (pl >> 6))) * a.W + x0 + (pl & 63);
-  };
+  auto pix_in = [&](int pl, int img) -> int64_t {
+    if constexpr (FLAT) return flat_pixel(q0 + pl, img, a.H, a.W, a.f_wp, a.f_hwp, a.f_magic);
+    else return ((int64_t)(img * a.H + y0 + (pl >> 6))) * a.W + x0 + (pl & 63);
+  };
+  auto pix_of = [&](int pl) -> int64_t { return pix_in(pl, e); };
   const int cs32 = a.Cin_pad / H32_BK, cs64 = a.Cin_pad / 64;
   const int r16 = lane >> 2, sl = lane & 3;
 
@@ -492,23 +494,32 @@
     for (int j = 0; j < NJ; ++j) acc16[i][j] = float4v{0.0f, 0.0f, 0.0f, 0.0f};
   if constexpr (BMC >= 64) {
     if (a.accinit) {
-#pragma unroll
-      for (int j = 0; j < NJ; ++j) {
-        const int64_t m = pix_of(wn * 64 + j * 16 + (lane & 15));
-        if (FLAT && m < 0) continue;
-#pragma unroll
-        for (int i = 0; i < MI; ++i) {
-          const int cg = cout0 + wm * (MI * 16) + i * 16 + 4 * (lane >> 4);
-          if constexpr (VAR == 1) {
-            const float4 v = *reinterpret_cast<const float4*>(reinterpret_cast<const float*>(a.accinit) + m * a.ai_ctot +
-                                                              a.ai_coff + cg);
-            acc16[i][j] = float4v{v.x, v.y, v.z, v.w};
-          } else {
-            const half4 v = *reinterpret_cast<const half4*>(a.accinit + m * a.ai_ctot + a.ai_coff + cg);
-            acc16[i][j] = float4v{(float)v[0], (float)v[1], (float)v[2], (float)v[3]};
-          }
-        }
+#define LOAD_INIT(IMG)                                                                                                        \
+  _Pragma("unroll") for (int j = 0; j < NJ; ++j) {                                                                            \
+    const int64_t m = pix_in(wn * 64 + j * 16 + (lane & 15), IMG);                                                            \
+    if (FLAT && m < 0) continue;                                                                                              \
+    _Pragma("unroll") for (int i = 0; i < MI; ++i) {                                                                          \
+      const int cg = cout0 + wm * (MI * 16) + i * 16 + 4 * (lane >> 4);                                                       \
+      if constexpr (VAR == 1) {                                                                                               \
+        const float4 v =                                                                                                      \
+            *reinterpret_cast<const float4*>(reinterpret_cast<const float*>(a.accinit) + m * a.ai_ctot + a.ai_coff + cg);     \
+        acc16[i][j] = float4v{v.x, v.y, v.z, v.w};                                                                            \
+      } else {                                                                                                                \
+        const half4 v = *reinterpret_cast<const half4*>(a.accinit + m * a.ai_ctot + a.ai_coff + cg);                          \
+        acc16[i][j] = float4v{(float)v[0], (float)v[1], (float)v[2], (float)v[3]};                                            \
+      }                                                                                                                       \
+    }                                                                                                                         \
+  }
+      if constexpr (FLAT) {
+        const int er = a.ai_rows ? a.ai_rows[e] : e;
+        LOAD_INIT(er)
+      } else if (a.ai_rows) {
+        const int er = a.ai_rows[e];
+        LOAD_INIT(er)
+      } else {
+        LOAD_INIT(e)
       }
+#undef LOAD_INIT
     }
   }
 
@@ -1354,6 +1365,7 @@
   const int Cin = c.Cin, Cout = c.Cout;
   VIPE_CHECK_ARG(c.x0.p && c.w && c.bias);
   VIPE_CHECK_ARG(!c.accinit.p || (c.accinit.ctot % 4 == 0 && c.accinit.coff % 4 == 0 && c.accinit.coff + Cout <= c.accinit.ctot));
+  VIPE_CHECK_ARG(!c.accinit_rows || c.accinit.p);
   VIPE_CHECK_ARG(c.B >= 0 && c.H > 0 && c.W > 0 && Cin > 0 && Cout > 0 && (c.KH & 1) && (c.KW & 1));
   if (Cin == 4) {
     VIPE_CHECK_ARG(c.split >= Cin && c.x0.ctot % 4 == 0 && c.x0.coff % 4 == 0);
@@ -1386,6 +1398,7 @@
   a.net = (const half_t*)c.net.p; a.net_ctot = c.net.ctot; a.net_coff = c.net.coff;
   a.zbuf = (const half_t*)c.z; a.fout = c.fout;
   a.accinit = (const half_t*)c.accinit.p; a.ai_ctot = c.accinit.ctot; a.ai_coff = c.accinit.coff; a.ai_f32 = c.accinit_f32;
+  a.ai_rows = c.accinit_rows;
   a.B = c.B; a.H = c.H; a.W = c.W; a.Cin = Cin; a.Cout = Cout; a.KH = c.KH; a.KW = c.KW;
   a.act = c.act; a.epi = c.epi;
   return launch_conv(a, stream);
@@ -1405,6 +1418,29 @@
   return vipe_conv_run(c, as_stream(stream));
 }
 
+VIPE_EXPORT int vipe_conv2d_fused_rows(const void* d_x0, int x0_ctot, int x0_coff, const void* d_x1, int x1_ctot,
+                                  int x1_coff, int split, const void* d_w_packed, const float* d_bias,
+                                  const float* d_extra, int extra_stride, int extra_off, void* d_y, int y_ctot,
+                                  int y_coff, void* d_y2, int y2_ctot, int y2_coff, const void* d_net, int net_ctot,
+                                  int net_coff, const void* d_z, float* d_fout, const void* d_accinit, int ai_ctot,
+                                  int ai_coff, int B, int H, int W, int Cin, int Cout, int KH, int KW, int act, int mode,
+                                  void* stream, const int* d_accinit_rows) {
+  ConvCall c;
+  c.x0 = {d_x0, x0_ctot, x0_coff}; c.x1 = {d_x1, x1_ctot, x1_coff}; c.split = split;
+  c.w = d_w_packed; c.bias = d_bias; c.extra = d_extra; c.extra_stride = extra_stride; c.extra_off = extra_off;
+  c.y = {d_y, y_ctot, y_coff}; c.y2 = {d_y2, y2_ctot, y2_coff}; c.net = {d_net, net_ctot, net_coff};
+  c.z = d_z; c.fout = d_fout;
+  c.accinit = {d_accinit, ai_ctot, ai_coff}; c.accinit_f32 = (mode & VIPE_CONV_ACCINIT_F32) != 0;
+  c.accinit_rows = d_accinit_rows;
+  c.B = B; c.H = H; c.W = W; c.Cin = Cin; c.Cout = Cout; c.KH = KH; c.KW = KW;
+  c.act = act; c.epi = mode & ~VIPE_CONV_ACCINIT_F32;
+  if (c.epi == EPI_HEADS_FUSED) {
+    c.heads2_frag = d_net; c.border = (float*)d_y2;
+    c.net.p = c.y2.p = nullptr;
+  }
+  return vipe_conv_run(c, as_stream(stream));
+}
+
 VIPE_EXPORT int vipe_conv2d_fused(const void* d_x0, int x0_ctot, int x0_coff, const void* d_x1, int x1_ctot,
                                   int x1_coff, int split, const void* d_w_packed, const float* d_bias,
                                   const float* d_extra, int extra_stride, int extra_off, void* d_y, int y_ctot,
@@ -1412,19 +1448,9 @@
                                   int net_coff, const void* d_z, float* d_fout, const void* d_accinit, int ai_ctot,
                                   int ai_coff, int B, int H, int W, int Cin, int Cout, int KH, int KW, int act, int mode,
                                   void* stream) {
-  ConvCall c;
-  c.x0 = {d_x0, x0_ctot, x0_coff}; c.x1 = {d_x1, x1_ctot, x1_coff}; c.split = split;
-  c.w = d_w_packed; c.bias = d_bias; c.extra = d_extra; c.extra_stride = extra_stride; c.extra_off = extra_off;
-  c.y = {d_y, y_ctot, y_coff}; c.y2 = {d_y2, y2_ctot, y2_coff}; c.net = {d_net, net_ctot, net_coff};
-  c.z = d_z; c.fout = d_fout;
-  c.accinit = {d_accinit, ai_ctot, ai_coff}; c.accinit_f32 = (mode & VIPE_CONV_ACCINIT_F32) != 0;
-  c.B = B; c.H = H; c.W = W; c.Cin = Cin; c.Cout = Cout; c.KH = KH; c.KW = KW;
-  c.act = act; c.epi = mode & ~VIPE_CONV_ACCINIT_F32;
-  if (c.epi == EPI_HEADS_FUSED) {
-    c.heads2_frag = d_net; c.border = (float*)d_y2;
-    c.net.p = c.y2.p = nullptr;
-  }
-  return vipe_conv_run(c, as_stream(stream));
+  return vipe_conv2d_fused_rows(d_x0, x0_ctot, x0_coff, d_x1, x1_ctot, x1_coff, split, d_w_packed, d_bias, d_extra, extra_stride,
+                                extra_off, d_y, y_ctot, y_coff, d_y2, y2_ctot, y2_coff, d_net, net_ctot, net_coff, d_z, d_fout,
+                                d_accinit, ai_ctot, ai_coff, B, H, W, Cin, Cout, KH, KW, act, mode, stream, nullptr);
 }
 
 VIPE_EXPORT int vipe_heads_fused_ok(int H, int W) {
diff --git a/vipe_amd/csrc/update_op.hip b/vipe_amd/csrc/update_op.hip
--- a/vipe_amd/csrc/update_op.hip
+++ b/vipe_amd/csrc/update_op.hip
@@ -108,7 +108,11 @@
     } else {
       c = conv({n, H, W}, at(b->net, 128, 0), gate_cin, ctx ? wt->zr_s_w : wt->zr_w, wt->zr_b, 256, 3);
       c.x1 = at(b->xbuf, 320, rest_coff); c.split = 128;
-      if (ctx) c.accinit = at(b->pgate, 384, 0);
+      if (ctx && b->pgate_rows) {
+        c.accinit = {b->pgate, 384, 0}; c.accinit_rows = b->pgate_rows + e0;
+      } else if (ctx) {
+        c.accinit = at(b->pgate, 384, 0);
+      }
     }
     c.epi = EPI_ZR; c.extra = b->extra + (int64_t)e0 * 384; c.extra_stride = 384;
     c.y = at(b->zb, 128, 0); c.y2 = at(b->rnet, 128, 0); c.net = at(b->net, 128, 0);
@@ -118,7 +122,7 @@
   if (Es < E) RUN(zr(Es, E - Es, false));
   ConvCall q = conv(g, {b->rnet, 128, 0}, gate_cin, ctx ? wt->q_s_w : wt->q_w, wt->q_b, 128, 3);
   q.x1 = {b->xbuf, 320, rest_coff}; q.split = 128;
-  if (ctx) q.accinit = {b->pgate, 384, 256};
+  if (ctx) { q.accinit = {b->pgate, 384, 256}; q.accinit_rows = b->pgate_rows; }
   q.epi = EPI_Q; q.extra = b->extra; q.extra_stride = 384; q.extra_off = 256;
   q.y = {b->net_out, 128, 0}; q.net = {b->net, 128, 0}; q.z = b->zb;
   RUN(vipe_conv_run(q, s));
@@ -173,7 +177,7 @@
   if (parts & 1) RUN(global_context(wt, b, d_net, as_stream(stream)));
   if (parts & 2) {
     ConvCall c = conv({b->E, b->H, b->W}, {d_net, 128, 0}, 128, wt->zr_n_w, wt->zr_b, 256, 3);
-    c.epi = EPI_PARTIAL; c.accinit = {b->pgate, 384, 0};
+    c.epi = EPI_PARTIAL; c.accinit = {b->pgate, 384, 0}; c.accinit_rows = b->pgate_rows;
     c.fout = b->pzr; c.y = {nullptr, 256, 0};
     RUN(vipe_conv_run(c, as_stream(stream)));
   }
@@ -196,7 +200,8 @@
   const int64_t px = (int64_t)b->H * b->W;
   vipe_update_buffers sub = *b;
   sub.E = (int)(e1 - e0);
-  sub.pgate = (const char*)b->pgate + e0 * px * 384 * 2;
+  if (b->pgate_rows) sub.pgate_rows = b->pgate_rows + e0;
+  else sub.pgate = (const char*)b->pgate + e0 * px * 384 * 2;
   sub.pzr = b->pzr + e0 * px * 256;
   return vipe_update_gate_state(j->weights, &sub, (const char*)j->net + e0 * px * 128 * 2, 2, stream);
 }
diff --git a/vipe_amd/slam/factor_graph.py b/vipe_amd/slam/factor_graph.py
--- a/vipe_amd/slam/factor_graph.py
+++ b/vipe_amd/slam/factor_graph.py
@@ -62,7 +62,7 @@
 
 BackendChunkPlan = dataclasses.make_dataclass("BackendChunkPlan", frozen=True, fields=[
     ("groups", list), ("rows", list), ("max_rows", int), ("max_edges", int), ("budget_rows", int), ("keep_all", bool), ("keep_some", bool)])
-_BackendChunk = dataclasses.make_dataclass("_BackendChunk", ["idx_x", "edges", "du", "dixs", "csr", "mask", "xb", "pgate"])
+_BackendChunk = dataclasses.make_dataclass("_BackendChunk", ["idx_x", "edges", "du", "dixs", "csr", "mask", "xb", "pgate", "pgate_rows"])
 
 
 def plan_backend_chunks(cnt, n_views, bytes_per_pyramid, steps, use_volume, budget_bytes, chunk_edges):
@@ -180,6 +180,60 @@
         return (self.net[1 - nb][:n_keep], self.xb[self.cur][:n_keep], self.pg[self.cur][:n_keep] if self.with_pgate else None)
 
 
+class GateContextPool:
+
+    def __init__(self, ht, wd, device):
+        self.ht, self.wd, self.device = ht, wd, device
+        self.rows = None
+        self.refs = np.zeros(0, dtype=np.int64)
+        self.edge_rows = np.zeros(0, dtype=np.int32)
+        self._dev = None
+
+    @property
+    def n_rows(self):
+        return int(np.count_nonzero(self.refs))
+
+    def _reserve(self, n_free):
+        free = np.flatnonzero(self.refs == 0)
+        if free.shape[0] < n_free:
+            cap0 = self.refs.shape[0]
+            cap = max(cap0 + (n_free - free.shape[0]), cap0 + cap0 // 4, 16)
+            rows = torch.empty((cap, self.ht, self.wd, 384), dtype=torch.float16, device=self.device)
+            if cap0:
+                rows[:cap0] = self.rows
+            self.rows, self.refs = rows, np.concatenate([self.refs, np.zeros(cap - cap0, dtype=np.int64)])
+            free = np.flatnonzero(self.refs == 0)
+        return free[:n_free]
+
+    def add(self, keys):
+        keys = np.asarray(keys, dtype=np.int64).reshape(-1)
+        _, first, inv = np.unique(keys, return_index=True, return_inverse=True)
+        fresh = self._reserve(first.shape[0])
+        self.refs[fresh] = np.bincount(inv.reshape(-1), minlength=first.shape[0])
+        self.edge_rows = np.concatenate([self.edge_rows, fresh[inv.reshape(-1)].astype(np.int32)])
+        self._dev = None
+        return fresh, first.astype(np.int64)
+
+    def remove(self, keep):
+        keep = np.asarray(keep, dtype=np.int64).reshape(-1)
+        self.refs = self.refs - np.bincount(self.edge_rows, minlength=self.refs.shape[0])
+        self.edge_rows = self.edge_rows[keep]
+        self.refs = self.refs + np.bincount(self.edge_rows, minlength=self.refs.shape[0])
+        self._dev = None
+
+    def fill(self, fresh, inp, gate_context):
+        m = int(fresh.shape[0])
+        if m and int(fresh[-1]) - int(fresh[0]) == m - 1:
+            gate_context(inp, out=self.rows[int(fresh[0]):int(fresh[0]) + m])
+        elif m:
+            self.rows.index_copy_(0, upload(fresh, self.device), gate_context(inp))
+
+    def device_rows(self):
+        if self._dev is None:
+            self._dev = upload(self.edge_rows, self.device, torch.int32)
+        return self._dev
+
+
 def _index_property(name):
     def put(self, tensor):
         self._index.assign(name, tensor)
@@ -193,6 +247,8 @@
     upsample = False
     upsample_from_row = None
     _last_ba = None
+    pgate_rows = None
+    _gate_pool = None
 
     def __init__(self, update_module, buffer, device, max_factors=48, incremental=True, cross_view=False):
         self.update_op = update_module
@@ -262,13 +318,22 @@
             WORK["pyramids_built"] += int(pi.shape[0])
             eng = self.update_op.engine(self.device)
             if self._stores is None:
-                self._stores = _EdgeStores(self.ht, self.wd, self.device, eng.supports_gate_split(self.ht, self.wd))
+                split = eng.supports_gate_split(self.ht, self.wd)
+                by_source = split and os.environ.get("VIPE_AMD_GATE_ROWS", "1") != "0"
+                self._stores = _EdgeStores(self.ht, self.wd, self.device, split and not by_source)
+                self._gate_pool = GateContextPool(self.ht, self.wd, self.device) if by_source else None
             self.net_n, self.xbuf, xb_new = self._stores.append(self.buffer.flattened_nets, self.buffer.flattened_inps,
                                                                 f1.contiguous(), self.net_n, n_live)
             if self._stores.with_pgate:
                 pg = self._stores.pg[self._stores.cur]
                 eng.gate_context(xb_new, out=pg[n_live:n_live + xb_new.shape[0]])
                 self.pgate = pg[:n_live + xb_new.shape[0]]
+            elif self._gate_pool is not None:
+                pool = self._gate_pool
+                fresh, first = pool.add(per_view(ii_h, V))
+                inp = xb_new if first.shape[0] == xb_new.shape[0] else xb_new.index_select(0, upload(first, self.device))
+                pool.fill(fresh, inp, eng.gate_context)
+                self.pgate, self.pgate_rows = pool.rows, pool.device_rows()
         else:
             net = self.buffer.nets[pi, qi].permute(0, 2, 3, 1).contiguous()
             self.net_n = net if self.net_n is None else torch.cat([self.net_n, net], 0)
@@ -305,12 +370,15 @@
             self.net_n = st.reserve(self.net_n.shape[0], self.net_n, self.net_n.shape[0])
         if st is not None and self.net_n is not None and st.bank_of(self.net_n) is not None:
             self.net_n, self.xbuf, pg = st.compact(keep_x, nk, self.net_n, extra)
-            if self.pgate is not None:
+            if self.pgate is not None and st.with_pgate:
                 self.pgate = pg
         else:
             if self.net_n is not None:
                 self.net_n = self.net_n[keep_x]
             rows_gather(extra)
+        if self._gate_pool is not None:
+            self._gate_pool.remove(keep_x_np)
+            self.pgate_rows = self._gate_pool.device_rows()
         self.target, self.weight = new_t, new_w
 
     def add_neighborhood_factors(self, t0, t1, r=3):
@@ -516,7 +584,7 @@
         up = {"want_upmask": True} if self.upsample else {}
         self.net_n, dw, eta, upmask = eng.forward_nhwc(self.net_n, self.xbuf, corr, motn, ix=P["dix"], n_src=P["n_src"],
                                                        net_out=self._net_spare(), csr=P["csr"], pgate=self.pgate,
-                                                       gate_state=self._gate_state, **up)
+                                                       pgate_rows=self.pgate_rows, gate_state=self._gate_state, **up)
         self._gate_state = None
         overlap = self.pgate is not None and E_act >= self.gate_overlap_min_edges
         ba_overlap = None
@@ -528,13 +596,14 @@
             n_staged = max(1, int(round(self.gate_overlap_share * E_act)))
             if self.gate_overlap_mode == "gated":
                 with torch.cuda.stream(self._side):
-                    eng.hidden_gate_state(self.net_n, self.pgate, parts=1)
+                    eng.hidden_gate_state(self.net_n, self.pgate, parts=1, pgate_rows=self.pgate_rows)
                 fr = self.gate_overlap_fractions if len(self.gate_overlap_fractions) == itrs else None
-                gate_state, ov = eng.gate_state_job(self.net_n, self.pgate, fractions=fr, n_staged=n_staged)
+                gate_state, ov = eng.gate_state_job(self.net_n, self.pgate, fractions=fr, n_staged=n_staged,
+                                                    pgate_rows=self.pgate_rows)
                 ba_overlap = ov(self._side)
             else:
                 with torch.cuda.stream(self._side):
-                    gate_state = eng.hidden_gate_state(self.net_n, self.pgate, n_staged=n_staged)
+                    gate_state = eng.hidden_gate_state(self.net_n, self.pgate, n_staged=n_staged, pgate_rows=self.pgate_rows)
         slam_ext.update_finish(coords1, dw, P["mask"], self.target, self.weight, eta, P["du"], self.damping)
         if use_inactive:
             key = ("inac", t0)
@@ -600,8 +669,14 @@
         csr = tuple(upload_many(host_csr(dixs_np, du_np.shape[0]), self.device, torch.int32))
         xb = torch.empty((plan.rows[gi], self.ht, self.wd, 320), dtype=torch.half, device=self.device)
         xb[..., 0:128] = buf.inps[pis, qis].permute(0, 2, 3, 1)
-        pgate = eng.gate_context(xb) if eng.supports_gate_split(self.ht, self.wd) else None
-        return _BackendChunk(idx_x=idx_x, edges=edges, du=du, dixs=dixs, csr=csr, mask=mask, xb=xb, pgate=pgate)
+        pgate = pgate_rows = None
+        if eng.supports_gate_split(self.ht, self.wd) and os.environ.get("VIPE_AMD_GATE_ROWS", "1") != "0":
+            inp = buf.flattened_inps[du].view(-1, 128, self.ht, self.wd).permute(0, 2, 3, 1).contiguous()
+            pgate, pgate_rows = eng.gate_context(inp), dixs.to(torch.int32)
+        elif eng.supports_gate_split(self.ht, self.wd):
+            pgate = eng.gate_context(xb)
+        return _BackendChunk(idx_x=idx_x, edges=edges, du=du, dixs=dixs, csr=csr, mask=mask, xb=xb, pgate=pgate,
+                             pgate_rows=pgate_rows)
 
     @torch.no_grad()
     def update_batch(self, itrs, steps, optimize_intrinsics, optimize_rig_rotation, solver_verbose=False):
@@ -646,7 +721,8 @@
                     corr_n = torch.zeros((n, self.ht, self.wd, 200), dtype=torch.half, device=self.device)
                     corr_n[..., :196] = corr1[0].permute(0, 2, 3, 1)
                 net, dw, eta, upmask = eng.forward_nhwc(take(self.net_n).contiguous(), c.xb, corr_n, take(motn).contiguous(),
-                                                        ix=c.dixs, n_src=int(c.du.shape[0]), csr=c.csr, pgate=c.pgate, **up)
+                                                        ix=c.dixs, n_src=int(c.du.shape[0]), csr=c.csr, pgate=c.pgate,
+                                                        pgate_rows=c.pgate_rows, **up)
                 if up:
                     upmasks.append((upmask, c.du))
                 WORK["edge_updates"] += n
diff --git a/vipe_amd/slam/update_engine.py b/vipe_amd/slam/update_engine.py
--- a/vipe_amd/slam/update_engine.py
+++ b/vipe_amd/slam/update_engine.py
@@ -4,7 +4,7 @@
 
 import torch
 
-from .._lib import check, lib, parse_struct, ptr, stream_ptr
+from .._lib import check, lib, parse_struct, ptr, require, stream_ptr
 
 UpdateWeights = parse_struct("vipe_update_weights")
 UpdateBuffers = parse_struct("vipe_update_buffers")
@@ -132,13 +132,18 @@
 
     def _conv(self, pk, x0, x0_coff, B, H, W, y=None, y_coff=0, act="none", mode="plain", x1=None, x1_coff=0,
               split=None, extra=None, extra_off=0, y2=None, y2_coff=0, net=None, net_coff=0, z=None, fout=None,
-              cin=None, accinit=None, ai_coff=0, w2=None, border=None):
+              cin=None, accinit=None, ai_coff=0, w2=None, border=None, accinit_rows=None):
         cin = pk.cin if cin is None else cin
         split = cin if split is None else split
         if mode == "heads_fused":
             assert net is None and y2 is None and w2 is not None and border is not None
             net, y2 = w2, border
-        check(lib().vipe_conv2d_fused(
+        rows = ()
+        if accinit_rows is not None:
+            require(accinit is not None and accinit_rows.dtype == torch.int32 and accinit_rows.shape[0] >= B,
+                    "accinit_rows: int32 [B], with accinit")
+            rows = (ptr(accinit_rows),)
+        check((lib().vipe_conv2d_fused_rows if rows else lib().vipe_conv2d_fused)(
             ptr(x0), x0.shape[-1], x0_coff, ptr(x1), x1.shape[-1] if x1 is not None else 0, x1_coff, split,
             ptr(pk.packed), ptr(pk.bias), ptr(extra), extra.shape[-1] if extra is not None else 0, extra_off,
             ptr(y), (y if y is not None else fout).shape[-1] if (y is not None or mode == "partial") else 0, y_coff,
@@ -147,7 +152,7 @@
             accinit.shape[-1] if accinit is not None else 0, ai_coff, B, H, W, cin, pk.cout,
             pk.kh, pk.kw, ACT[act],
             EPI[mode] | (ACCINIT_F32 if accinit is not None and accinit.dtype == torch.float32 else 0),
-            stream_ptr(x0)), "conv2d_fused")
+            stream_ptr(x0), *rows), "conv2d_fused")
 
     @staticmethod
     def supports_gate_split(ht, wd):
@@ -160,9 +165,9 @@
         return pg
 
     @torch.no_grad()
-    def hidden_gate_state(self, net, pgate, native=True, parts=3, n_staged=None):
+    def hidden_gate_state(self, net, pgate, native=True, parts=3, n_staged=None, pgate_rows=None):
         E, H, W, _ = net.shape
-        gs, b, glo = self._gate_state(net, pgate, n_staged)
+        gs, b, glo = self._gate_state(net, pgate, n_staged, pgate_rows)
         Es, pzr, extra = gs["n_staged"], gs["pzr"], gs["extra"]
         if native:
             for part, n in ((1, E), (2, Es)):
@@ -177,10 +182,11 @@
                 check(lib().vipe_glo_context(ptr(glo), ptr(self.glo_w), ptr(self.glo_b), ptr(extra), E, H * W,
                                              stream_ptr(glo)), "glo_context")
             if parts & 2:
-                self._conv(self.zr_n, net, 0, Es, H, W, mode="partial", fout=pzr, accinit=pgate, ai_coff=0)
+                self._conv(self.zr_n, net, 0, Es, H, W, mode="partial", fout=pzr, accinit=pgate, ai_coff=0,
+                           **({} if pgate_rows is None else {"accinit_rows": pgate_rows}))
         return gs
 
-    def _gate_state(self, net, pgate, n_staged):
+    def _gate_state(self, net, pgate, n_staged, pgate_rows=None):
         E, H, W, _ = net.shape
         Es = E if n_staged is None else max(1, min(E, int(n_staged)))
         self._gate_gen += 1
@@ -190,12 +196,21 @@
         b = UpdateBuffers()
         b.E, b.H, b.W = Es, H, W
         b.pgate, b.pzr, b.glo, b.extra = pgate.data_ptr(), pzr.data_ptr(), glo.data_ptr(), extra.data_ptr()
-        gs = dict(net_ptr=net.data_ptr(), pgate_ptr=pgate.data_ptr(), shape=tuple(net.shape), pzr=pzr, extra=extra,
-                  n_staged=Es, keep=(b,), gen=self._gate_gen)
+        b.pgate_rows = self._rows_ptr(pgate_rows, E) or None
+        gs = dict(net_ptr=net.data_ptr(), pgate_ptr=pgate.data_ptr(), rows_ptr=self._rows_ptr(pgate_rows, E), shape=tuple(net.shape),
+                  pzr=pzr, extra=extra, n_staged=Es, keep=(b,), gen=self._gate_gen)
         return gs, b, glo
 
-    def gate_state_job(self, net, pgate, fractions=None, n_staged=None):
-        gs, b, _ = self._gate_state(net, pgate, n_staged)
+    @staticmethod
+    def _rows_ptr(pgate_rows, E):
+        if pgate_rows is None:
+            return 0
+        require(pgate_rows.dtype == torch.int32 and pgate_rows.is_contiguous() and pgate_rows.shape[0] == E,
+                "pgate_rows: contiguous int32 [E]")
+        return pgate_rows.data_ptr()
+
+    def gate_state_job(self, net, pgate, fractions=None, n_staged=None, pgate_rows=None):
+        gs, b, _ = self._gate_state(net, pgate, n_staged, pgate_rows)
         E = gs["n_staged"]
         job = GateStateJob()
         job.weights, job.buffers, job.net = ctypes.addressof(self._wdesc), ctypes.addressof(b), net.data_ptr()
@@ -212,9 +227,10 @@
         gs["keep"] = (b, job, bounds)
         return gs, (lambda stream: (stream.cuda_stream, fn, ctypes.addressof(job)))
 
-    def gate_state_matches(self, gs, net, pgate):
+    def gate_state_matches(self, gs, net, pgate, pgate_rows=...):
         return (gs is not None and pgate is not None and gs["net_ptr"] == net.data_ptr() and
-                gs["pgate_ptr"] == pgate.data_ptr() and gs["shape"] == tuple(net.shape) and gs.get("gen") == self._gate_gen)
+                gs["pgate_ptr"] == pgate.data_ptr() and gs["shape"] == tuple(net.shape) and gs.get("gen") == self._gate_gen and
+                (pgate_rows is ... or gs.get("rows_ptr", 0) == (0 if pgate_rows is None else pgate_rows.data_ptr())))
 
     def fused_heads(self, H, W):
         return self.fused_heads_on and bool(lib().vipe_heads_fused_ok(H, W))
@@ -233,9 +249,12 @@
 
     @torch.no_grad()
     def forward_nhwc(self, net, xbuf, corr, motn, ix=None, n_src=None, net_out=None, want_upmask=False, csr=None,
-                     pgate=None, native=True, gate_state=None):
+                     pgate=None, native=True, gate_state=None, pgate_rows=None):
         E, H, W, _ = net.shape
-        if not self.gate_state_matches(gate_state, net, pgate):
+        if pgate is None:
+            pgate_rows = None
+        self._rows_ptr(pgate_rows, E)
+        if not self.gate_state_matches(gate_state, net, pgate, pgate_rows):
             gate_state = None
         if gate_state is None:
             self._gate_gen += 1
@@ -250,7 +269,9 @@
             net_out = torch.empty_like(net)
         if native:
             return self._forward_native(net, xbuf, corr, motn, ix, n_src, net_out, want_upmask, csr, pgate,
-                                        (c1, f1, zb, rnet, hbuf, dw, glo), gate_state)
+                                        (c1, f1, zb, rnet, hbuf, dw, glo), gate_state, pgate_rows)
+        shared = pgate_rows is not None
+        rows = {"accinit_rows": pgate_rows} if shared else {}
         if isinstance(corr, tuple):
             from ..ext import droid_net_ext
             droid_net_ext.corr_lookup_conv1x1(corr[1], corr[2], self.corr0.packed, self.corr0.bias, c1, act="relu",
@@ -273,14 +294,15 @@
                        accinit=gate_state["pzr"], ai_coff=0, cin=192)
             if Es < E:
                 self._conv(self.zr_s, net[Es:], 0, E - Es, H, W, x1=xbuf[Es:], x1_coff=128, split=128, y=zb[Es:], y2=rnet[Es:],
-                           net=net[Es:], mode="zr", extra=extra[Es:], accinit=pgate[Es:], ai_coff=0)
+                           net=net[Es:], mode="zr", extra=extra[Es:], ai_coff=0,
+                           **(dict(accinit=pgate, accinit_rows=pgate_rows[Es:]) if shared else dict(accinit=pgate[Es:])))
             self._conv(self.q_s, rnet, 0, E, H, W, x1=xbuf, x1_coff=128, split=128, y=net_out, net=net, z=zb, mode="q",
-                       extra=extra, extra_off=256, accinit=pgate, ai_coff=256)
+                       extra=extra, extra_off=256, accinit=pgate, ai_coff=256, **rows)
         elif pgate is not None:
             self._conv(self.zr_s, net, 0, E, H, W, x1=xbuf, x1_coff=128, split=128, y=zb, y2=rnet, net=net, mode="zr",
-                       extra=extra, accinit=pgate, ai_coff=0)
+                       extra=extra, accinit=pgate, ai_coff=0, **rows)
             self._conv(self.q_s, rnet, 0, E, H, W, x1=xbuf, x1_coff=128, split=128, y=net_out, net=net, z=zb, mode="q",
-                       extra=extra, extra_off=256, accinit=pgate, ai_coff=256)
+                       extra=extra, extra_off=256, accinit=pgate, ai_coff=256, **rows)
         else:
             self._conv(self.zr, net, 0, E, H, W, x1=xbuf, split=128, y=zb, y2=rnet, net=net, mode="zr", extra=extra)
             self._conv(self.q, rnet, 0, E, H, W, x1=xbuf, split=128, y=net_out, net=net, z=zb, mode="q", extra=extra,
@@ -324,7 +346,7 @@
         return net_out, dw, eta, upmask
 
     def _forward_native(self, net, xbuf, corr, motn, ix, n_src, net_out, want_upmask, csr, pgate, scratch,
-                        gate_state=None):
+                        gate_state=None, pgate_rows=None):
         c1, f1, zb, rnet, hbuf, dw, glo = scratch
         E, H, W, _ = net.shape
         extra = self._buf("extra", (E, 384), torch.float32)
@@ -340,7 +362,7 @@
             eta = self._buf("eta", (n_src, H, W), torch.float32)
         lookup = isinstance(corr, tuple)
         hborder = self._hborder(E, H, W) if self.fused_heads(H, W) else None
-        tensors = (net, net_out, xbuf, motn, pgate, c1, f1, zb, rnet, hbuf, dw, glo, extra, order, rowptr, agg, a2, eta,
+        tensors = (net, net_out, xbuf, motn, pgate, pgate_rows, c1, f1, zb, rnet, hbuf, dw, glo, extra, order, rowptr, agg, a2, eta,
                    hborder) + \
             ((tuple(corr[1]) + (corr[2],) + ((corr[3],) if len(corr) > 3 and corr[3] is not None else ())) if lookup else (corr,))
         pzr = gate_state["pzr"] if gate_state is not None else None
@@ -369,7 +391,7 @@
                 b.pyramid_layout = 1 if lv[0].dim() == 7 else 0
             else:
                 b.corr = corr.data_ptr()
-            for name, t in dict(motn=motn, net=net, net_out=net_out, xbuf=xbuf, pgate=pgate, c1=c1, f1=f1, zb=zb, rnet=rnet,
+            for name, t in dict(motn=motn, net=net, net_out=net_out, xbuf=xbuf, pgate=pgate, pgate_rows=pgate_rows, c1=c1, f1=f1, zb=zb, rnet=rnet,
                                 hbuf=hbuf, dw=dw, glo=glo, extra=extra, order=order, rowptr=rowptr, agg=agg, a2=a2,
                                 eta=eta, hborder=hborder).items():
                 setattr(b, name, None if t is None else t.data_ptr())
```

Measured after the change: 278.6 (median of 6 runs). About the same (+0.6%).
